# MiRaCLeXeoN/sduss

Hardware: AMD Instinct MI355X
Metric: images/sec (node), SDXL 1024^2 50-step, fixed prompt, CFG (higher is better)
Workload: dtype bf16; 1 GPU; SDXL-base-1.0 UNet 1024x1024 50-step Euler, CFG 5.0, 4 requests/step (denoiser batch 8) per GPU, is_sliced=False, random-init weights of the real architecture (2.57 B params), one data-parallel replica per GPU, no collective; resolution=1024, steps_per_image=50

## Files before the change

### include/mxdenoise.h

```cpp
#ifndef MXDENOISE_H
#define MXDENOISE_H

#include <stddef.h>
#include <stdint.h>

#ifdef __cplusplus
extern "C" {
#endif

enum { MX_F32 = 0, MX_F16 = 1, MX_BF16 = 2 };

const char* mx_last_error(void);
int mx_version(void);
#define MX_PROF_KINDS 12
int mx_profile_enable(int on);
int mx_profile_collect(double* out);
int mx_profile_records(double* out, int max_records);

size_t mx_groupnorm_halo_workspace_bytes(int N, int C, int cpg);
int mx_groupnorm_halo(void* stream, const void* x, const void* gamma, const void* beta, void* y,
                      int N, int C, int H, int W, int cpg, double eps, int padding,
                      const int32_t* latent_offset, int n_latents, const int32_t* patch_map,
                      const int32_t* padding_idx, int dtype, void* workspace);
int mx_halo_only(void* stream, const void* x, void* y, int N, int C, int H, int W,
                 const int32_t* padding_idx, int dtype);


enum {
  MX_EPI_SILU     = 1 << 0,
  MX_EPI_GEGLU    = 1 << 1,
  MX_EPI_OUT_F32  = 1 << 2,
  MX_EPI_QKV      = 1 << 3,
  MX_EPI_GELU_TANH = 1 << 4,
  MX_EPI_RES_BCAST = 1 << 5,
  MX_EPI_RMSNORM  = 1 << 6,
  MX_EPI_GELU     = 1 << 7,
  MX_EPI_QUICK_GELU = 1 << 8,
  MX_EPI_GEGLU_TANH = 1 << 9
};

#define MX_MAX_SEGS 4
typedef struct mx_gemm_seg {
  const void* a;
  const void* a2;
  void* c;
  const void* residual;
  void* vt;
  const float* rowbias;
  const float* gate;
  const float* ln_stats;
  float* stats_out;
  int M;
  int rows_per_batch;
  int ldvt;
  int B, Hin, Win, Hout, Wout;
  int a_batch_rows, a_row_off, c_batch_rows, c_row_off;
} mx_gemm_seg;

typedef struct mx_gemm_desc {
  const void* a;
  const void* w;
  void* c;
  const float* bias;
  const float* rowbias;
  const void* residual;
  void* vt;
  int M, N, K;
  int lda, ldc, ldr, ldrb;
  int rows_per_batch;
  int flags;
  int seg, period, ldvt;
  int B, Hin, Win, Cin;
  int Hout, Wout;
  int stride;
  int up;
  int corner_patch;
  int a_batch_rows, a_row_off, c_batch_rows, c_row_off;
  const float* gate;
  int ldg;
  float out_scale;
  const float* rms_wq;
  const float* rms_wk;
  float rms_eps;
  int vhalo;
  const void* a2;
  int lda2, k_split;
  const float* ln_stats;
  const float* ln_colsum;
  int ln_slabs;
  float ln_eps;
  float* stats_out;
  const mx_gemm_seg* segs;
  int n_segs;
  int splitk;
  const float* ln_final;
  float* ln_final_out;
  unsigned* ln_final_cnt;
  float* gn_part_out;
  int cin_valid;
} mx_gemm_desc;

int mx_gemm(void* stream, const mx_gemm_desc* d);
int mx_gemm_launches(const mx_gemm_desc* d);
int mx_gemm_stats_slabs(const mx_gemm_desc* d);
int mx_gemm_ln_prefers_pass(const mx_gemm_desc* d);
int mx_gemm_ln_final_supported(const mx_gemm_desc* d);
int mx_gemm_gn_partials_supported(const mx_gemm_desc* d, int conv);
enum { MX_FORM_TILE_GENERIC = 0, MX_FORM_TILE_256 = 1, MX_FORM_TILE_128 = 2, MX_FORM_PERSISTENT_256 = 3, MX_FORM_SMALL_M = 4, MX_FORM_CONV_SMALL_N = 5, MX_FORM_CONV_SMALL_CIN = 6 };
int mx_gemm_form(const mx_gemm_desc* d, int conv);
int mx_gemm_kernel_name(const mx_gemm_desc* d, int conv, int launch, char* buf, int cap);
int mx_gemm_kernel_names(char* buf, int cap);
int mx_attention_kernel_name(int B, int H, int Lq, int Lk, int ldo, int prescaled, int causal, int bias, int key_chunk, int force_cross, char* buf, int cap);
int mx_attention_kernel_names(char* buf, int cap);
#define MX_STATS_PITCH(slabs) (((slabs) + 3) & ~3)
int mx_row_stats(void* stream, const void* x, int ldx, float* stats, int M, int C);
int mx_conv3x3(void* stream, const mx_gemm_desc* d);
int mx_gemm_splitk(const mx_gemm_desc* d, int conv);
void mx_gemm_release_scratch(void* stream, int all);

typedef struct mx_attn_tail_desc {
  mx_gemm_desc out1, to_q, out2;
  const void* k; int ldk;
  const void* vt; int ldvt; int64_t vt_batch_stride;
  int B, heads, L, ctx_len;
  unsigned* sync;
} mx_attn_tail_desc;
size_t mx_attn_tail_sync_bytes(int M);
int mx_attn_tail_supported(const mx_attn_tail_desc* d);
int mx_attn_tail_preferred(void);
int mx_attn_tail(void* stream, const mx_attn_tail_desc* d);
int mx_attn_tail_status(void* stream, const unsigned* sync, unsigned* word);

#define MX_VT_POS(key) (((key) & ~12) | (((key) & 4) << 1) | (((key) & 8) >> 1))
#define MX_VT_LD(Lk) (((Lk) + 15) / 16 * 16)

int mx_attention(void* stream, const void* q, int ldq, const void* k, int ldk, const void* vt, int ldvt,
                 int64_t vt_batch_stride, void* o, int ldo, int B, int H, int Lq, int Lk, float scale);
#define MX_ATTN_QSCALE(scale) ((scale) * 1.4426950408889634f)
int mx_attention_prescaled(void* stream, const void* q, int ldq, const void* k, int ldk, const void* vt, int ldvt,
                           int64_t vt_batch_stride, void* o, int ldo, int B, int H, int Lq, int Lk);
int mx_attention_cross_prescaled(void* stream, const void* q, int ldq, const void* k, int ldk, const void* vt, int ldvt,
                                 int64_t vt_batch_stride, void* o, int ldo, int B, int H, int Lq, int Lk);
typedef struct mx_attn_problem {
  const void* q; const void* k; const void* vt; void* o;
  int64_t vt_batch_stride;
  int B, Lq, Lk, ldvt;
} mx_attn_problem;
int mx_attention_prescaled_grouped(void* stream, const mx_attn_problem* probs, int n, int ldq, int ldk, int ldo, int H);
int mx_attention_prescaled_bias(void* stream, const void* q, int ldq, const void* k, int ldk, const void* vt, int ldvt,
                                int64_t vt_batch_stride, void* o, int ldo, int B, int H, int Lq, int Lk, const float* bias, int ldb);
int mx_attention_prescaled_causal(void* stream, const void* q, int ldq, const void* k, int ldk, const void* vt, int ldvt,
                                  int64_t vt_batch_stride, void* o, int ldo, int B, int H, int L);

int mx_layernorm(void* stream, const void* x, void* y, const float* gamma, const float* beta,
                 int M, int C, float eps);

int mx_rmsnorm(void* stream, const void* x, void* y, const float* w, int M, int C, float eps);

int mx_layernorm_mod(void* stream, const void* x, void* y, void* y2, const float* scale, const float* shift,
                     const float* scale2, const float* shift2, int ldmod, int M, int C, int rows_per_batch, float eps);
int mx_layernorm_mod_grouped(void* stream, const void* x, void* y, void* y2, const float* scale, const float* shift, const float* scale2,
                             const float* shift2, int ldmod, int C, float eps, const int* batches, const int* rows_per_batch, int n);
int mx_rmsnorm_heads(void* stream, void* x, int ld, int nbatch, int rows_per_batch, int batch_rows, int row_off,
                     int heads_total, int heads_q, const float* wq, const float* wk, float eps, float q_scale);

size_t mx_groupnorm_nhwc_workspace_bytes(int B, int H, int W, int C);
int mx_groupnorm_nhwc(void* stream, const void* x, void* y, const float* gamma, const float* beta,
                      int B, int H, int W, int C, int groups, float eps, int silu, int patch,
                      void* workspace);

int mx_groupnorm_nhwc_cat(void* stream, const void* x, int C1, const void* x2, void* y, const float* gamma, const float* beta,
                          int B, int H, int W, int C, int groups, float eps, int silu, int patch, void* workspace);
int mx_groupnorm_nhwc_from_partials(void* stream, const void* x, void* y, const float* gamma, const float* beta, int B, int H, int W, int C, int groups, float eps,
                                    int silu, const float* part, int chunk, const float* add_bias, const float* add_rowbias, int ldrb, void* workspace);

typedef struct mx_gn_problem { const void* x; const void* x2; void* y; int B, H, W; } mx_gn_problem;
size_t mx_groupnorm_nhwc_grouped_workspace_bytes(const mx_gn_problem* probs, int n, int C);
int mx_groupnorm_nhwc_grouped(void* stream, const mx_gn_problem* probs, int n, int C1, const float* gamma, const float* beta, int C, int groups,
                              float eps, int silu, int patch, void* workspace);

typedef struct mx_unet_config {
  int in_channels, out_channels;
// ... 199 lines not shown
```

### sduss_amd/csrc/gemm_args.h

```cpp
#pragma once
#include "common.h"
#include "../../include/mxdenoise.h"

namespace mx {

constexpr int kMaxSegs = MX_MAX_SEGS;
struct GemmSeg {
  const bf16_t* a; const bf16_t* a2; void* c; const bf16_t* residual; bf16_t* vt; const float* rowbias; const float* gate;
  const float* ln_stats; float* stats_out;
  int M, tile0, rows_per_batch, ldvt;
  int B, Hin, Win, Hout, Wout;
  int a_batch_rows, a_row_off, c_batch_rows, c_row_off;
};

struct GemmArgs {
  const bf16_t* a;
  const bf16_t* w;
  void* c;
  const float* bias;
  const float* rowbias;
  const bf16_t* residual;
  bf16_t* vt;
  int M, N, K;
  int lda, ldc, ldr, ldrb;
  int rows_per_batch;
  int flags;
  int seg, period, ldvt;
  int B, Hin, Win, Cin, Hout, Wout, stride, up, corner_patch;
  int a_batch_rows, a_row_off, c_batch_rows, c_row_off;
  const float* gate;
  int ldg;
  int xcd_map;
  float out_scale;
  const float* rms_wq;
  const float* rms_wk;
  float rms_eps;
  int stagger_ticks;
  int vhalo;
  const bf16_t* a2;
  int lda2, k_split;
  const float* ln_stats;
  const float* ln_colsum;
  int ln_slabs;
  float ln_eps;
  float* stats_out;
  const float* ln_final;
  float* ln_final_out;
  unsigned* ln_final_cnt;
  int ln_final_slabs;
  float* gn_part;
  int splitk;
  float* sk_ws;
  unsigned* sk_cnt;
  int nseg, mt_total;
  GemmSeg prob[kMaxSegs];
};

__device__ __forceinline__ int gemm_select_seg(GemmArgs& q, const GemmArgs& p, int& tm) {
  if (p.nseg <= 0) return 0;
  int s = 0;
#pragma unroll
  for (int i = 1; i < kMaxSegs; ++i) if (i < p.nseg && tm >= p.prob[i].tile0) s = i;
  const GemmSeg& g = p.prob[s];
  tm -= g.tile0;
  q.a = g.a; q.a2 = g.a2; q.c = g.c; q.residual = g.residual; q.vt = g.vt; q.rowbias = g.rowbias; q.gate = g.gate;
  q.ln_stats = g.ln_stats; q.stats_out = g.stats_out;
  q.M = g.M; q.rows_per_batch = g.rows_per_batch; q.ldvt = g.ldvt;
  q.B = g.B; q.Hin = g.Hin; q.Win = g.Win; q.Hout = g.Hout; q.Wout = g.Wout;
  q.a_batch_rows = g.a_batch_rows; q.a_row_off = g.a_row_off; q.c_batch_rows = g.c_batch_rows; q.c_row_off = g.c_row_off;
  return s;
}
__device__ __forceinline__ int gemm_m_tiles(const GemmArgs& p, int rows) { return p.nseg > 0 ? p.mt_total : (p.M + rows - 1) / rows; }

__device__ __forceinline__ f32x4 fma4(const f32x4 a, const float s, const f32x4 c) {
  return f32x4{fmaf(a[0], s, c[0]), fmaf(a[1], s, c[1]), fmaf(a[2], s, c[2]), fmaf(a[3], s, c[3])};
}

__device__ __forceinline__ float sum_over_fq(float x) {
  float a = x, b = x;
  asm volatile("s_nop 1\n\tv_permlane16_swap_b32 %0, %1" : "+v"(a), "+v"(b));
  a += b; b = a;
  asm volatile("s_nop 1\n\tv_permlane32_swap_b32 %0, %1" : "+v"(a), "+v"(b));
  return a + b;
}

template <int NI, int MI>
__device__ __forceinline__ void gemm_ln_init(const GemmArgs& p, f32x4 (&acc)[NI][MI], const int m_wave0, const int wave_n0, const int fr,
                                             const int fq, float (&rstd)[MI]) {
#pragma clang fp contract(off)
  const int slabs = p.ln_slabs;
  const int pitch = (slabs + 3) & ~3;
  float s1[MI], s2[MI];
#pragma unroll
  for (int j = 0; j < MI; ++j) { s1[j] = 0.f; s2[j] = 0.f; }
  for (int g = 4 * fq; g < slabs; g += 16) {
    constexpr int JC = MI > 4 ? 4 : MI;
#pragma unroll
    for (int j0 = 0; j0 < MI; j0 += JC) {
      f32x4 va[JC], vb[JC];
#pragma unroll
      for (int j = 0; j < JC; ++j) {
        const int m = m_wave0 + (j0 + j) * 16 + fr;
        const float* src = p.ln_stats + ((long)(m < p.M ? m : p.M - 1) * pitch + g) * 2;
        va[j] = *reinterpret_cast<const f32x4*>(src);
        vb[j] = *reinterpret_cast<const f32x4*>(src + 4);
      }
#pragma unroll
      for (int j = 0; j < JC; ++j) {
        s1[j0 + j] += va[j][0] + (g + 1 < slabs ? va[j][2] : 0.f) + (g + 2 < slabs ? vb[j][0] : 0.f) + (g + 3 < slabs ? vb[j][2] : 0.f);
        s2[j0 + j] += va[j][1] + (g + 1 < slabs ? va[j][3] : 0.f) + (g + 2 < slabs ? vb[j][1] : 0.f) + (g + 3 < slabs ? vb[j][3] : 0.f);
      }
    }
  }
  const float inv = 1.0f / (float)p.K;
  float nmean[MI];
#pragma unroll
  for (int j = 0; j < MI; ++j) {
    const float a = sum_over_fq(s1[j]), b = sum_over_fq(s2[j]);
    const float mean = a * inv;
    const float var = fmaxf(fmaf(-mean, mean, b * inv), 0.f);
    rstd[j] = rsqrtf(var + p.ln_eps);
    nmean[j] = -mean;
  }
#pragma unroll
  for (int i = 0; i < NI; ++i) {
    const int n = wave_n0 + i * 16 + fq * 4;
    const f32x4 cs = n < p.N ? *reinterpret_cast<const f32x4*>(p.ln_colsum + n) : f32x4{0.f, 0.f, 0.f, 0.f};
#pragma unroll
    for (int j = 0; j < MI; ++j) acc[i][j] = cs * nmean[j];
  }
}

__device__ __forceinline__ void gemm_ln_row(const GemmArgs& p, const int m, const int fq, float& rstd, float& rm) {
#pragma clang fp contract(off)
  const int mc = m < p.M ? m : p.M - 1;
  const int pitch = (p.ln_slabs + 3) & ~3;
  float s1 = 0.f, s2 = 0.f;
  for (int s = fq; s < p.ln_slabs; s += 4) {
    const f32x2 v = *reinterpret_cast<const f32x2*>(p.ln_stats + ((long)mc * pitch + s) * 2);
    s1 += v[0]; s2 += v[1];
  }
  s1 = sum_over_fq(s1); s2 = sum_over_fq(s2);
  const float inv = 1.0f / (float)p.K;
  const float mean = s1 * inv;
  const float var = fmaxf(fmaf(-mean, mean, s2 * inv), 0.f);
  rstd = rsqrtf(var + p.ln_eps);
  rm = rstd * mean;
}

__device__ __forceinline__ float row16_sum(float x) {
  x += __builtin_bit_cast(float, __builtin_amdgcn_update_dpp(0, __builtin_bit_cast(int, x), 0xB1, 0xF, 0xF, true));
  x += __builtin_bit_cast(float, __builtin_amdgcn_update_dpp(0, __builtin_bit_cast(int, x), 0x4E, 0xF, 0xF, true));
  x += __builtin_bit_cast(float, __builtin_amdgcn_update_dpp(0, __builtin_bit_cast(int, x), 0x141, 0xF, 0xF, true));
  x += __builtin_bit_cast(float, __builtin_amdgcn_update_dpp(0, __builtin_bit_cast(int, x), 0x140, 0xF, 0xF, true));
  return x;
// ... 39 lines not shown
      a += __uint_as_float((unsigned)v); q += __uint_as_float((unsigned)(v >> 32));
    }
  }
  const float a2 = __shfl_xor(a, 1, 64), q2 = __shfl_xor(q, 1, 64);
  if (!(tid & 1) && m < p.M) {
    const float inv = 1.0f / (float)p.N;
    const float mean = (a + a2) * inv;
    const float var = fmaxf(fmaf(-mean, mean, (q + q2) * inv), 0.f);
    *reinterpret_cast<f32x2*>(p.ln_final_out + (long)m * 2) = f32x2{mean, rsqrtf(var + p.ln_eps)};
  }
}

template <int NI, int MI, bool KEEP>
__device__ __forceinline__ void gemm_ln_init_final(const GemmArgs& p, f32x4 (&acc)[NI][MI], const int m_wave0, const int wave_n0, const int fr,
                                                   const int fq, float (&rstd)[MI]) {
#pragma clang fp contract(off)
  f32x2 st[MI];
#pragma unroll
  for (int j = 0; j < MI; ++j) {
    const int m = m_wave0 + j * 16 + fr;
    st[j] = *reinterpret_cast<const f32x2*>(p.ln_final + (long)(m < p.M ? m : p.M - 1) * 2);
  }
  f32x4 cs[NI];
#pragma unroll
  for (int i = 0; i < NI; ++i) cs[i] = *reinterpret_cast<const f32x4*>(p.ln_colsum + wave_n0 + i * 16 + fq * 4);
  if constexpr (KEEP) {
#pragma unroll
    for (int j = 0; j < MI; ++j) rstd[j] = st[j][1];
  }
#pragma unroll
  for (int i = 0; i < NI; ++i)
#pragma unroll
    for (int j = 0; j < MI; ++j) acc[i][j] = cs[i] * (-st[j][0]);
}

typedef unsigned int u32x4_sk __attribute__((ext_vector_type(4)));
template <int NI, int MI>
__device__ __forceinline__ bool splitk_combine(const GemmArgs& p, f32x4 (&acc)[NI][MI], const int tile, const int slice, const int tile_elems,
                                               volatile int* ticket_word) {
  const int tid = threadIdx.x;
  const auto rsrc = __builtin_amdgcn_make_buffer_rsrc(p.sk_ws + (long)tile * p.splitk * tile_elems, 0, p.splitk * tile_elems * 4, 0x00020000);
  const int lane_off = tid * 16;
#pragma unroll
  for (int i = 0; i < NI; ++i)
#pragma unroll
    for (int j = 0; j < MI; ++j)
      __builtin_amdgcn_raw_buffer_store_b128(__builtin_bit_cast(u32x4_sk, acc[i][j]), rsrc, (slice * tile_elems + (i * MI + j) * 2048) * 4 + lane_off, 0, 16);
  asm volatile("s_waitcnt vmcnt(0)" ::: "memory");
  __syncthreads();
  if (tid == 0) *ticket_word = (int)__hip_atomic_fetch_add(p.sk_cnt + tile, 1u, __ATOMIC_RELAXED, __HIP_MEMORY_SCOPE_AGENT);
  __syncthreads();
  const int ticket = *ticket_word;
  if (ticket != p.splitk - 1) return false;
  if (tid == 0) __hip_atomic_store(p.sk_cnt + tile, 0u, __ATOMIC_RELAXED, __HIP_MEMORY_SCOPE_AGENT);
#pragma unroll
  for (int i = 0; i < NI; ++i)
#pragma unroll
    for (int j = 0; j < MI; ++j) acc[i][j] = f32x4{0.f, 0.f, 0.f, 0.f};
  for (int s = 0; s < p.splitk; ++s) {
    f32x4 v[NI][MI];
#pragma unroll
    for (int i = 0; i < NI; ++i)
#pragma unroll
      for (int j = 0; j < MI; ++j)
        v[i][j] = __builtin_bit_cast(f32x4, __builtin_amdgcn_raw_buffer_load_b128(rsrc, (s * tile_elems + (i * MI + j) * 2048) * 4 + lane_off, 0, 16));
#pragma unroll
    for (int i = 0; i < NI; ++i)
#pragma unroll
      for (int j = 0; j < MI; ++j) acc[i][j] += v[i][j];
  }
  return true;
}

__device__ __forceinline__ long gemm_in_row(const GemmArgs& p, int m) {
  if (p.a_batch_rows <= 0) return m;
  const int b = m / p.rows_per_batch;
  return (long)b * p.a_batch_rows + p.a_row_off + (m - b * p.rows_per_batch);
}
__device__ __forceinline__ long gemm_out_row(const GemmArgs& p, int m, int bidx) {
  if (p.c_batch_rows <= 0) return m;
  return (long)bidx * p.c_batch_rows + p.c_row_off + (m - bidx * p.rows_per_batch);
}

template <int NI, int MI, int BN>
__device__ __forceinline__ void gemm_epilogue(const GemmArgs& p, f32x4 (&acc)[NI][MI], const int m_wave0,
                                              const int wave_n0, const int fr, const int fq) {
  const int flags = p.flags;
  const bool geglu = (flags & MX_EPI_GEGLU) != 0;
  const bool qkv = (flags & MX_EPI_QKV) != 0;
  int seg_idx = 0, seg_grp = 0, seg_pos = 0;
  bool to_vt = false;
  if (qkv) {
    seg_idx = wave_n0 / p.seg;
    seg_grp = seg_idx / p.period;
    seg_pos = seg_idx - seg_grp * p.period;
    to_vt = (seg_pos == p.period - 1);
  }

  const bool rms = qkv && (flags & MX_EPI_RMSNORM) && !to_vt;
  const bool ln = p.ln_stats != nullptr;
#pragma unroll
  for (int j = 0; j < MI; ++j) {
    const int m = m_wave0 + j * 16 + fr;
    float rms_mul = 1.0f;
    float ln_rstd = 1.0f, ln_rm = 0.f;
    if (ln) gemm_ln_row(p, m, fq, ln_rstd, ln_rm);
    if (rms) {
      float ss = 0.f;
#pragma unroll
      for (int i = 0; i < NI; ++i) {
        const int n = wave_n0 + i * 16 + fq * 4;
#pragma unroll
        for (int q = 0; q < 4; ++q) { const float t = acc[i][j][q] + (p.bias ? p.bias[n + q] : 0.f); ss += t * t; }
      }
      ss = sum_over_fq(ss);
      rms_mul = rsqrtf(ss * (1.0f / 64.0f) + p.rms_eps) * ((seg_pos == 0 && p.out_scale != 0.f) ? p.out_scale : 1.0f);
    }
    if (m >= p.M) continue;
    const int bidx = (p.rows_per_batch > 0) ? (m / p.rows_per_batch) : 0;
    const long orow = gemm_out_row(p, m, bidx);
    const long rrow = (flags & MX_EPI_RES_BCAST) ? (long)(m - bidx * p.rows_per_batch) : orow;
#pragma unroll
    for (int i = 0; i < (NI); ++i) {
      if (geglu && i >= NI / 2) continue;
      const int n = wave_n0 + i * 16 + fq * 4;
      if (n >= p.N) continue;
      float v[4];
#pragma unroll
      for (int q = 0; q < 4; ++q) v[q] = acc[i][j][q];
      if (ln) {
        const f32x4 c4 = *reinterpret_cast<const f32x4*>(p.ln_colsum + n);
#pragma unroll
        for (int q = 0; q < 4; ++q) v[q] = v[q] * ln_rstd - ln_rm * c4[q];
      }
      if (p.bias) {
        const f32x4 b4 = *reinterpret_cast<const f32x4*>(p.bias + n);
#pragma unroll
        for (int q = 0; q < 4; ++q) v[q] += b4[q];
      }
      if (rms) {
        const float* w = (seg_pos == 0 ? p.rms_wq : p.rms_wk) + ((n - seg_idx * p.seg) & 63);
#pragma unroll
        for (int q = 0; q < 4; ++q) v[q] *= rms_mul * w[q];
      } else if (p.out_scale != 0.f && (!qkv || seg_pos == 0)) {
#pragma unroll
        for (int q = 0; q < 4; ++q) v[q] *= p.out_scale;
      }
      if (geglu) {
        float g[4];
        const int ng = n + (NI / 2) * 16;
#pragma unroll
        for (int q = 0; q < 4; ++q) g[q] = acc[i + NI / 2][j][q];
        if (ln) {
          const f32x4 c4 = *reinterpret_cast<const f32x4*>(p.ln_colsum + ng);
#pragma unroll
          for (int q = 0; q < 4; ++q) g[q] = g[q] * ln_rstd - ln_rm * c4[q];
        }
        if (p.bias) {
          const f32x4 b4 = *reinterpret_cast<const f32x4*>(p.bias + ng);
#pragma unroll
          for (int q = 0; q < 4; ++q) g[q] += b4[q];
        }
#pragma unroll
        for (int q = 0; q < 4; ++q) v[q] = v[q] * ((flags & MX_EPI_GEGLU_TANH) ? gelu_tanh_f(g[q]) : gelu_fast(g[q]));
        const int nout = wave_n0 / 2 + i * 16 + fq * 4;
        u32x2 o = {pack_bf16x2(v[0], v[1]), pack_bf16x2(v[2], v[3])};
        *reinterpret_cast<u32x2*>(reinterpret_cast<bf16_t*>(p.c) + (long)m * p.ldc + nout) = o;
        continue;
      }
      if (p.rowbias) {
        const f32x4 b4 = *reinterpret_cast<const f32x4*>(p.rowbias + (long)bidx * p.ldrb + n);
#pragma unroll
        for (int q = 0; q < 4; ++q) v[q] += b4[q];
      }
      if (p.gate) {
        const f32x4 g4 = *reinterpret_cast<const f32x4*>(p.gate + (long)bidx * p.ldg + n);
#pragma unroll
        for (int q = 0; q < 4; ++q) v[q] *= g4[q];
      }
      if (p.residual) {
        const u32x2 r = *reinterpret_cast<const u32x2*>(p.residual + rrow * p.ldr + n);
        v[0] += bf16lo_to_f32(r[0]); v[1] += bf16hi_to_f32(r[0]);
        v[2] += bf16lo_to_f32(r[1]); v[3] += bf16hi_to_f32(r[1]);
      }
      if (flags & MX_EPI_SILU) {
#pragma unroll
        for (int q = 0; q < 4; ++q) v[q] = silu_f(v[q]);
      }
      if (flags & MX_EPI_GELU_TANH) {
#pragma unroll
        for (int q = 0; q < 4; ++q) v[q] = gelu_tanh_f(v[q]);
      }
      if (flags & (MX_EPI_GELU | MX_EPI_QUICK_GELU)) {
#pragma unroll
        for (int q = 0; q < 4; ++q) v[q] = (flags & MX_EPI_GELU) ? gelu_fast(v[q]) : quick_gelu_f(v[q]);
      }
      if (qkv) {
        const int nin = n - seg_idx * p.seg;
        if (to_vt) {
          const int key0 = (p.c_batch_rows > 0 ? p.c_row_off : 0) + m - bidx * p.rows_per_batch;
          const int key = MX_VT_POS(key0);
          const int nv = p.N / p.period;
          bf16_t* dst = p.vt + ((long)bidx * nv + (long)seg_grp * p.seg + nin) * p.ldvt + key;
#pragma unroll
          for (int q = 0; q < 4; ++q) dst[(long)q * p.ldvt] = f32_to_bf16(v[q]);
        } else {
          const int ccol = seg_grp * (p.period - 1) * p.seg + seg_pos * p.seg + nin;
          u32x2 o = {pack_bf16x2(v[0], v[1]), pack_bf16x2(v[2], v[3])};
          *reinterpret_cast<u32x2*>(reinterpret_cast<bf16_t*>(p.c) + orow * p.ldc + ccol) = o;
        }
        continue;
      }
      if (flags & MX_EPI_OUT_F32) {
        f32x4 o = {v[0], v[1], v[2], v[3]};
        *reinterpret_cast<f32x4*>(reinterpret_cast<float*>(p.c) + orow * p.ldc + n) = o;
      } else {
        u32x2 o = {pack_bf16x2(v[0], v[1]), pack_bf16x2(v[2], v[3])};
        *reinterpret_cast<u32x2*>(reinterpret_cast<bf16_t*>(p.c) + orow * p.ldc + n) = o;
      }
    }
  }
}


__device__ __forceinline__ void gemm_tile_of_block(const int b, const int mt, const int nt, const int xcd_map, int& tm, int& tn) {
  constexpr int MB = 4;
  if (!xcd_map || (mt & 7) != 0) { tm = b % mt; tn = b / mt; return; }
  const int xcd = b & 7;
  const int local = b >> 3;
  const int mloc = mt >> 3;
  const int band_tiles = MB * nt;
  const int band = local / band_tiles;
  const int r = local - band * band_tiles;
  const int rows = (mloc - band * MB) < MB ? (mloc - band * MB) : MB;
  tn = r / rows;
  tm = ((band * MB + (r - tn * rows)) << 3) + xcd;
}

__device__ __forceinline__ void lane_exchange_pair(float (&a)[4], float (&b)[4]) {
#pragma unroll
  for (int d = 0; d < 4; ++d) {
    unsigned x = __float_as_uint(a[d]), y = __float_as_uint(b[d]);
    auto r = __builtin_amdgcn_permlane32_swap(x, y, false, false);
    auto t = __builtin_amdgcn_permlane16_swap(r[0], r[1], false, false);
    a[d] = __uint_as_float(t[0]);
    b[d] = __uint_as_float(t[1]);
  }
}

__device__ __forceinline__ u32x4 lane_xor1(const u32x4 x) {
  u32x4 r;
#pragma unroll
  for (int d = 0; d < 4; ++d) r[d] = (unsigned)__builtin_amdgcn_update_dpp(0, (int)x[d], 0xB1, 0xF, 0xF, true);
  return r;
}

constexpr int EPI_F_QKV = 1;
constexpr int EPI_F_ACT = 2;
constexpr int EPI_F_ALL = 3;
constexpr int EPI_F_TANH = 4;
__host__ __device__ inline int gemm_epi_features(int flags) {
  const int acts = flags & (MX_EPI_SILU | MX_EPI_GELU | MX_EPI_GELU_TANH | MX_EPI_QUICK_GELU | MX_EPI_GEGLU_TANH);
  return ((flags & MX_EPI_QKV) ? EPI_F_QKV : 0) | (acts == 0 ? 0 : acts == MX_EPI_GELU_TANH ? EPI_F_TANH : EPI_F_ACT);
}
template <int NI, int MI, bool GEGLU, bool VEC = true, bool VPF = true, bool STATS = true, int FEAT = EPI_F_ALL, bool EMIT = STATS, bool RSTD_LOAD = false, bool WT = false>
__device__ __forceinline__ void gemm_epilogue_regs(const GemmArgs& p, f32x4 (&acc)[NI][MI], const int m_wave0, const int wave_n0,
                                                   const int fr, const int fq, const float (&ln_rstd_a)[MI]) {
#pragma clang fp contract(off)
  constexpr int NIO = GEGLU ? NI / 2 : NI;
  constexpr int NP = NIO / 2;
  constexpr bool ODD = (NIO & 1) != 0;
  constexpr int DEPTH = MI <= 4 ? MI : 2;
  static_assert(!GEGLU || NI % 4 == 0, "GEGLU: hidden and gate halves must be whole pairs");
  const int flags = p.flags;
  constexpr bool ACT = (FEAT & EPI_F_ACT) != 0;
  constexpr bool TANH = (FEAT & (EPI_F_ACT | EPI_F_TANH)) != 0;
  const bool qkv = (FEAT & EPI_F_QKV) != 0 && (flags & MX_EPI_QKV) != 0;
  int seg_idx = 0, seg_grp = 0, seg_pos = 0;
  bool to_vt = false;
  if (qkv) {
    seg_idx = wave_n0 / p.seg;
    seg_grp = seg_idx / p.period;
    seg_pos = seg_idx - seg_grp * p.period;
    to_vt = seg_pos == p.period - 1;
  }
  const bool rms = qkv && (flags & MX_EPI_RMSNORM) && !to_vt;
  const float w_scale = (!rms && p.out_scale != 0.f && (!qkv || seg_pos == 0)) ? p.out_scale : 1.0f;
  const int col0 = GEGLU ? wave_n0 / 2 : qkv ? seg_grp * (p.period - 1) * p.seg + seg_pos * p.seg + (wave_n0 - seg_idx * p.seg) : wave_n0;
  const bool has_res = !GEGLU && p.residual != nullptr;
  const bool has_rb = VEC && !GEGLU && p.rowbias != nullptr, has_gate = VEC && !GEGLU && p.gate != nullptr;

  f32x4 bias_r[NI];
#pragma unroll
  for (int i = 0; i < NI; ++i) {
    bias_r[i] = f32x4{0.f, 0.f, 0.f, 0.f};
    if (p.bias && (GEGLU || i < NIO)) bias_r[i] = *reinterpret_cast<const f32x4*>(p.bias + wave_n0 + i * 16 + fq * 4);
  }
  f32x4 rmsw_r[NI];
  if (rms) {
    const float* w = seg_pos == 0 ? p.rms_wq : p.rms_wk;
#pragma unroll
    for (int i = 0; i < NI; ++i) rmsw_r[i] = *reinterpret_cast<const f32x4*>(w + ((wave_n0 - seg_idx * p.seg + i * 16 + fq * 4) & 63));
  }
  const bool stats = EMIT && !GEGLU && !qkv && p.stats_out != nullptr;

  if constexpr ((FEAT & EPI_F_QKV) != 0) {
    if (qkv && to_vt) {
      const int rpb_v = p.rows_per_batch > 0 ? p.rows_per_batch : 0x7fffffff;
      const int m_first = m_wave0 + fr;
      int bv = p.rows_per_batch > 0 ? m_first / p.rows_per_batch : 0;
      int rv = m_first - bv * (p.rows_per_batch > 0 ? p.rows_per_batch : 0);
      const int key_off = p.c_batch_rows > 0 ? p.c_row_off : 0;
      const int nv = p.N / p.period;
      const long feat0 = (long)seg_grp * p.seg + (wave_n0 - seg_idx * p.seg) + fq * 4;
      auto rstd_at = [&](int j) __attribute__((always_inline)) -> float {
        const int m = m_first + 16 * j;
        return p.ln_final[(long)(m < p.M ? m : p.M - 1) * 2 + 1];
      };
      float rs_next = RSTD_LOAD ? rstd_at(0) : 1.0f;
#pragma unroll
      for (int j = 0; j < MI; ++j) {
        const float rs_cur = rs_next;
        if (RSTD_LOAD && j + 1 < MI) rs_next = rstd_at(j + 1);
        if (m_first + 16 * j < p.M) {
          const int key = MX_VT_POS(key_off + rv);
          bf16_t* dst = p.vt + ((long)bv * nv + feat0) * p.ldvt + key;
          const float rs = RSTD_LOAD ? rs_cur : STATS ? ln_rstd_a[j] : 1.0f;
#pragma unroll
          for (int i = 0; i < NIO; ++i) {
            const f32x4 t = STATS ? fma4(acc[i][j], rs, bias_r[i]) : acc[i][j] + bias_r[i];
#pragma unroll
            for (int q = 0; q < 4; ++q) dst[(long)(i * 16 + q) * p.ldvt] = f32_to_bf16(t[q]);
          }
        }
        rv += 16;
        if (rv >= rpb_v) { rv -= rpb_v; ++bv; }
      }
      return;
    }
  }
  const bool odd_lane = (fr & 1) != 0;
  const int rpb = p.rows_per_batch > 0 ? p.rows_per_batch : 0x7fffffff;
  const int cbr = p.c_batch_rows > 0 ? p.c_batch_rows : (p.rows_per_batch > 0 ? p.rows_per_batch : 0);
  const int cro = p.c_batch_rows > 0 ? p.c_row_off : 0;
  const int b_last = p.rows_per_batch > 0 ? (p.M - 1) / p.rows_per_batch : 0;
  const int r_last = p.M - 1 - b_last * (p.rows_per_batch > 0 ? p.rows_per_batch : 0);
  const int row_last = b_last * cbr + cro + r_last;
  const int mA0 = (m_wave0 + fr) & ~1;
  int row_a[MI], row_b[MI];
  int bo_walk = 0, ro_walk = 0;
  {
    int bA = p.rows_per_batch > 0 ? mA0 / p.rows_per_batch : 0;
    int rA = mA0 - bA * (p.rows_per_batch > 0 ? p.rows_per_batch : 0);
#pragma unroll
    for (int j = 0; j < MI; ++j) {
      int bB = bA, rB = rA + 1;
      if (rB >= rpb) { rB = 0; ++bB; }
      const int mA = mA0 + 16 * j;
      row_a[j] = mA < p.M ? bA * cbr + cro + rA : row_last;
      row_b[j] = mA + 1 < p.M ? bB * cbr + cro + rB : row_last;
      if constexpr (VEC) { if (j == 0) { bo_walk = odd_lane ? bB : bA; ro_walk = odd_lane ? rB : rA; } }
      rA += 16;
      if (rA >= rpb) { rA -= rpb; ++bA; }
    }
  }
  auto token = [&](int j) __attribute__((always_inline)) { return m_wave0 + j * 16 + fr; };
  auto row_own = [&](int j) __attribute__((always_inline)) { return odd_lane ? row_b[j] : row_a[j]; };
  const char* const res_base = reinterpret_cast<const char*>(p.residual);
  char* const c_base = reinterpret_cast<char*>(p.c);
  const unsigned ldr_b = (unsigned)p.ldr * 2u, ldc_b = (unsigned)p.ldc * 2u;
  auto res_at = [&](int row, int col) __attribute__((always_inline)) { return res_base + (unsigned long long)(unsigned)row * ldr_b + (unsigned)(col * 2); };
  auto c_at = [&](int row, int col) __attribute__((always_inline)) { return c_base + (unsigned long long)(unsigned)row * ldc_b + (unsigned)(col * 2); };
  const auto c_rsrc = __builtin_amdgcn_make_buffer_rsrc(p.c, 0, WT ? (int)((unsigned)p.M * ldc_b) : 0, 0x00020000);
  auto store_c16 = [&](int row, int col, const u32x4 v) __attribute__((always_inline)) {
    if constexpr (WT) __builtin_amdgcn_raw_buffer_store_b128(v, c_rsrc, (int)((unsigned)row * ldc_b + (unsigned)(col * 2)), 0, 16);
    else *reinterpret_cast<u32x4*>(c_at(row, col)) = v;
  };
  auto store_c8 = [&](int row, int col, const u32x2 v) __attribute__((always_inline)) {
    if constexpr (WT) __builtin_amdgcn_raw_buffer_store_b64(v, c_rsrc, (int)((unsigned)row * ldc_b + (unsigned)(col * 2)), 0, 16);
    else *reinterpret_cast<u32x2*>(c_at(row, col)) = v;
  };

  auto load_res = [&](int j, int pr) __attribute__((always_inline)) -> u32x4 {
    if (!has_res) return u32x4{0u, 0u, 0u, 0u};
    return *reinterpret_cast<const u32x4*>(res_at(row_own(j), col0 + pr * 32 + fq * 8));
  };
  auto load_res_odd = [&](int j) __attribute__((always_inline)) -> u32x2 {
    if (!has_res) return u32x2{0u, 0u};
    return *reinterpret_cast<const u32x2*>(res_at(row_own(j), col0 + NP * 32 + fq * 4));
  };
  f32x4 rb_r[VEC ? NIO : 1], gate_r[VEC ? NIO : 1];
  auto load_batch_vectors = [&](int j) __attribute__((always_inline)) {
    if constexpr (VEC) {
      (void)j;
      const int bidx = bo_walk < b_last ? bo_walk : b_last;
      ro_walk += 16;
      if (ro_walk >= rpb) { ro_walk -= rpb; ++bo_walk; }
#pragma unroll
      for (int i = 0; i < NIO; ++i) {
        const int n = wave_n0 + i * 16 + fq * 4;
        if (has_rb) rb_r[i] = *reinterpret_cast<const f32x4*>(p.rowbias + (long)bidx * p.ldrb + n);
        if (has_gate) gate_r[i] = *reinterpret_cast<const f32x4*>(p.gate + (long)bidx * p.ldg + n);
      }
    }
  };
  if constexpr (VPF) { if (has_rb || has_gate) load_batch_vectors(0); }
  constexpr int NG = NP / 2;
  constexpr bool fullmode = NG > 0;
  const int col_full = col0 + (odd_lane ? 32 : 0) + fq * 8;
  auto load_res_full = [&](int j, int g, int which) __attribute__((always_inline)) -> u32x4 {
    if (!has_res) return u32x4{0u, 0u, 0u, 0u};
    return *reinterpret_cast<const u32x4*>(res_at(which ? row_b[j] : row_a[j], col_full + 64 * g));
  };
  auto load_res_any = [&](int j, int pr) __attribute__((always_inline)) -> u32x4 {
    if (pr < 2 * NG) return load_res_full(j, pr >> 1, pr & 1);
    return load_res(j, pr);
  };
  u32x4 res_r[DEPTH][NP > 0 ? NP : 1];
  u32x2 res_o[DEPTH];
  {
#pragma unroll
    for (int d = 0; d < DEPTH && d < MI; ++d) {
#pragma unroll
      for (int pr = 0; pr < NP; ++pr) res_r[d][pr] = load_res_any(d, pr);
      if constexpr (ODD) res_o[d] = load_res_odd(d);
    }
  }

  auto rstd_at = [&](int j) __attribute__((always_inline)) -> float {
    const int m = token(j);
    return p.ln_final[(long)(m < p.M ? m : p.M - 1) * 2 + 1];
  };
  float rstd_next = RSTD_LOAD ? rstd_at(0) : 1.0f;
#pragma unroll
// ... 153 lines not shown
```

### sduss_amd/csrc/gemm_bf16.hip

```cpp
#include <algorithm>
#include <cstdlib>

#include <mutex>
#include <unordered_map>

#include "common.h"
#include "../../include/mxdenoise.h"
#include "gemm_args.h"
#include "gemm_forms.h"

namespace mx {

constexpr int BM = 128;
constexpr int BK = 64;

__device__ __forceinline__ int swz(int row, int chunk) { return chunk ^ ((row >> 1) & 7); }

template <int BN, bool CONV>
__global__ __launch_bounds__(256, 2) void gemm_kernel(const GemmArgs pk) {
  constexpr int NI = BN / 32;
  constexpr int MI = 4;
  constexpr int WROWS = BN / 32;
  __shared__ __attribute__((aligned(16))) bf16_t sX[2][BM * BK];
  __shared__ __attribute__((aligned(16))) bf16_t sW[2][BN * BK];

  const int tid = threadIdx.x;
  const int lane = tid & 63;
  const int wave = tid >> 6;
  const int wm = wave >> 1;
  const int wn = wave & 1;
  GemmArgs p = pk;
  int tm = blockIdx.x;
  gemm_select_seg(p, pk, tm);
  const int m0 = tm * BM;
  const int n0 = blockIdx.y * BN;
  const int nk = p.K / BK;

  const int srow = tid >> 3;
  const int sch = tid & 7;

  int xoff[4];
  int xoff2[4];
  int cb[4], cy[4], cx[4];
#pragma unroll
  for (int i = 0; i < 4; ++i) {
    const int m = m0 + srow + 32 * i;
    if constexpr (!CONV) {
      xoff[i] = (m < p.M) ? (int)(gemm_in_row(p, m) * p.lda) + sch * 8 : -1;
      xoff2[i] = (p.a2 != nullptr && m < p.M) ? m * p.lda2 + sch * 8 : 0;
    } else {
      if (m < p.M) {
        const int hw = p.Hout * p.Wout;
        const int b = m / hw;
        const int r = m - b * hw;
        const int oy = r / p.Wout;
        cb[i] = b;
        cy[i] = oy * p.stride;
        cx[i] = (r - oy * p.Wout) * p.stride;
      } else {
        cb[i] = -1; cy[i] = 0; cx[i] = 0;
      }
    }
  }
  int woff[WROWS];
#pragma unroll
  for (int i = 0; i < WROWS; ++i) {
    const int n = n0 + srow + 32 * i;
    woff[i] = (n < p.N) ? n * p.K + sch * 8 : -1;
  }

  u32x4 rx[4], rw[WROWS];
  const u32x4 zero4 = {0u, 0u, 0u, 0u};

  auto load_tile = [&](int kt) {
    const int k0 = kt * BK;
    if constexpr (!CONV) {
#pragma unroll
      for (int i = 0; i < 4; ++i) {
        if (p.a2 != nullptr && k0 >= p.k_split) rx[i] = (xoff[i] >= 0) ? *reinterpret_cast<const u32x4*>(p.a2 + xoff2[i] + (k0 - p.k_split)) : zero4;
        else rx[i] = (xoff[i] >= 0) ? *reinterpret_cast<const u32x4*>(p.a + xoff[i] + k0) : zero4;
      }
    } else {
      const int tap = k0 / p.Cin;
      const int c0 = k0 - tap * p.Cin;
      const int dy = tap / 3 - 1;
      const int dx = tap - (tap / 3) * 3 - 1;
      const int Hv = p.Hin << p.up, Wv = p.Win << p.up;
      const int P = p.corner_patch;
#pragma unroll
      for (int i = 0; i < 4; ++i) {
        int iy = cy[i] + dy;
        const int ix = cx[i] + dx;
        if (P > 0 && dy != 0 && dx != 0) {
          const bool cross_r = ((iy + P) / P) != ((cy[i] + P) / P);
          const bool cross_c = ((ix + P) / P) != ((cx[i] + P) / P);
          if (cross_r && cross_c) iy = cy[i];
        }
        const bool ok = (cb[i] >= 0) && (iy >= -p.vhalo) && (iy < Hv + p.vhalo) && (ix >= 0) && (ix < Wv);
        if (ok) {
          const long src = (((long)cb[i] * (p.Hin + 2 * p.vhalo) + (iy >> p.up) + p.vhalo) * p.Win + (ix >> p.up)) * p.Cin + c0 + sch * 8;
          rx[i] = *reinterpret_cast<const u32x4*>(p.a + src);
        } else {
          rx[i] = zero4;
        }
      }
    }
#pragma unroll
    for (int i = 0; i < WROWS; ++i)
      rw[i] = (woff[i] >= 0) ? *reinterpret_cast<const u32x4*>(p.w + woff[i] + k0) : zero4;
  };
  auto store_tile = [&](int buf) {
#pragma unroll
    for (int i = 0; i < 4; ++i) {
      const int row = srow + 32 * i;
      *reinterpret_cast<u32x4*>(&sX[buf][row * BK + swz(row, sch) * 8]) = rx[i];
    }
#pragma unroll
    for (int i = 0; i < WROWS; ++i) {
      const int row = srow + 32 * i;
      *reinterpret_cast<u32x4*>(&sW[buf][row * BK + swz(row, sch) * 8]) = rw[i];
    }
  };

  f32x4 acc[NI][MI];
#pragma unroll
  for (int i = 0; i < NI; ++i)
#pragma unroll
    for (int j = 0; j < MI; ++j) acc[i][j] = f32x4{0.f, 0.f, 0.f, 0.f};

  const int fr = lane & 15;
  const int fq = lane >> 4;

  load_tile(0);
  store_tile(0);
  __syncthreads();

  for (int kt = 0; kt < nk; ++kt) {
    const int buf = kt & 1;
    if (kt + 1 < nk) load_tile(kt + 1);
#pragma unroll
    for (int ks = 0; ks < 2; ++ks) {
      bf16x8 wf[NI], xf[MI];
#pragma unroll
      for (int i = 0; i < NI; ++i) {
        const int row = wn * (BN / 2) + i * 16 + fr;
        wf[i] = *reinterpret_cast<const bf16x8*>(&sW[buf][row * BK + swz(row, ks * 4 + fq) * 8]);
      }
#pragma unroll
      for (int j = 0; j < MI; ++j) {
        const int row = wm * 64 + j * 16 + fr;
        xf[j] = *reinterpret_cast<const bf16x8*>(&sX[buf][row * BK + swz(row, ks * 4 + fq) * 8]);
      }
#pragma unroll
      for (int i = 0; i < NI; ++i)
#pragma unroll
        for (int j = 0; j < MI; ++j)
          acc[i][j] = __builtin_amdgcn_mfma_f32_16x16x32_bf16(wf[i], xf[j], acc[i][j], 0, 0, 0);
    }
    if (kt + 1 < nk) store_tile(buf ^ 1);
    __syncthreads();
  }

  gemm_epilogue<NI, MI, BN>(p, acc, m0 + wm * 64, n0 + wn * (BN / 2), fr, fq);
}

int launch_v2(hipStream_t s, const GemmArgs& a, int bn, int form);
int launch_v5(hipStream_t s, const GemmArgs& a, int bn, int rows, int form);
int launch_v4(hipStream_t s, const GemmArgs& a, int form);
bool small_m_serves(const mx_gemm_desc* d, bool conv);
int small_m_form(long N, long K, int flags);
int launch_small_m(hipStream_t s, const GemmArgs& a, int form);
bool conv_small_n_serves(const mx_gemm_desc* d);
int launch_conv_small_n(hipStream_t s, const GemmArgs& a);
bool conv_small_cin_serves(const mx_gemm_desc* d);
int launch_conv_small_cin(hipStream_t s, const GemmArgs& a);

constexpr size_t kSplitKWsBytes = 96u << 20;
constexpr size_t kSplitKCntBytes = 64u << 10;
struct TileChoice { int bn; int rows; int splitk = 1; };
static long m_tiles_of(const mx_gemm_desc* d, int rows) {
  if (d->n_segs <= 0) return cdiv(d->M, rows);
  long t = 0;
  for (int i = 0; i < d->n_segs; ++i) t += cdiv(d->segs[i].M, rows);
  return t;
}
static long rows_of(const mx_gemm_desc* d) {
  if (d->n_segs <= 0) return d->M;
  long m = 0;
  for (int i = 0; i < d->n_segs; ++i) m += d->segs[i].M;
  return m;
}
static TileChoice pick_tile(const mx_gemm_desc* d, bool conv) {
  constexpr double v3_discount = 0.87;
  const TileChoice none = {0, 0};
  const long Mtot = rows_of(d);
  if (Mtot < 128 || d->K < 128) return none;
  if (d->flags & (MX_EPI_OUT_F32 | MX_EPI_RES_BCAST)) return none;
  if (d->n_segs <= 0) { if (d->rows_per_batch > 0 && d->rows_per_batch < 16) return none; }
  else for (int i = 0; i < d->n_segs; ++i) if (d->segs[i].rows_per_batch > 0 && d->segs[i].rows_per_batch < 16) return none;
  if (d->ldc % 8 != 0 || ((uintptr_t)d->c & 15) != 0) return none;
  if (d->residual && (d->ldr % 8 != 0 || ((uintptr_t)d->residual & 15) != 0)) return none;
  const bool geglu = (d->flags & MX_EPI_GEGLU) != 0, qkv = (d->flags & MX_EPI_QKV) != 0;
  bool fits32 = (long)d->N * d->K * 2 < (1L << 32);
  if (d->n_segs <= 0) {
    const long in_rows = d->a_batch_rows > 0 ? (long)(d->M / d->rows_per_batch + 1) * d->a_batch_rows : d->M;
    fits32 = fits32 && in_rows * d->lda * 2 < (1L << 32);
  } else {
    uintptr_t lo = (uintptr_t)d->segs[0].a;
    for (int i = 1; i < d->n_segs; ++i) lo = std::min(lo, (uintptr_t)d->segs[i].a);
    for (int i = 0; i < d->n_segs; ++i) {
      const mx_gemm_seg& g = d->segs[i];
      const long in_rows = g.a_batch_rows > 0 ? (long)(g.M / std::max(g.rows_per_batch, 1) + 1) * g.a_batch_rows : g.M;
      fits32 = fits32 && (long)((uintptr_t)g.a - lo) + in_rows * d->lda * 2 < (1L << 32);
    }
  }
  TileChoice best = none;
  double best_cost = 0;
  const TileChoice cands[5] = {{256, 256}, {160, 256}, {128, 256}, {160, 128}, {128, 128}};
  for (int c = 0; c < 5; ++c) {
    const int bn = cands[c].bn, rows = cands[c].rows;
    if (d->N % bn != 0 || Mtot < rows) continue;
    if (bn == 256 && (conv || !fits32 || d->a2 || d->ln_stats || d->stats_out)) continue;
    if (d->ln_final && bn != 256) continue;
    if (geglu && bn == 160) continue;
    if (qkv && d->seg % 64 != 0) continue;
    if ((d->flags & MX_EPI_RMSNORM) && bn == 160) continue;
    if (qkv && bn != 256 && d->seg % (bn / 2) != 0) continue;
    const long tiles = m_tiles_of(d, rows) * (d->N / bn);
    const int ncu = cu_count();
    const double cost = (double)((tiles + ncu - 1) / ncu) * (rows + bn) * (bn == 256 ? v3_discount : 1.0);
    if (best.rows == 0 || cost < best_cost) { best = cands[c]; best_cost = cost; }
  }
  if (d->splitk != 1 && best.rows == 128 && !d->a2 && d->K / 64 >= 16) {
    const int ncu = cu_count();
    const int nk = d->K / 64;
    double best_t = 0, unsplit_t = 0;
    TileChoice pick = best;
    const double mtot = (double)Mtot;
    for (int c = 3; c < 5; ++c) {
      const int bn = cands[c].bn;
      if (d->N % bn != 0 || (geglu && bn == 160) || (qkv && (d->seg % 64 != 0 || d->seg % (bn / 2) != 0)) || ((d->flags & MX_EPI_RMSNORM) && bn == 160)) continue;
      const long tiles = m_tiles_of(d, 128) * (d->N / bn);
      for (int sk = 1; sk <= 4; ++sk) {
        if (d->splitk > 1 && sk != 1 && sk != d->splitk) continue;
        if (nk / sk < 8 || (sk > 1 && tiles * sk > 2L * ncu)) continue;
        if (sk > 1 && (tiles * sk * 128L * bn * 4 > (long)kSplitKWsBytes || tiles * 4 > (long)kSplitKCntBytes)) continue;
        const double combine = sk > 1 ? 2.0 + (double)sk * mtot * d->N * 8.0 / 4.0e6 : 0.0;
        const double t = (double)((tiles * sk + ncu - 1) / ncu) * ((double)(nk / sk) * 0.57 * (128 + bn) / 256.0 + 5.0) + combine;
        if (sk == 1 && bn == best.bn) unsplit_t = t;
        if (best_t == 0 || t < best_t - 1e-9) { best_t = t; pick = TileChoice{bn, 128, sk}; }
      }
    }
    if (pick.splitk > 1 && unsplit_t > 0 && best_t <= 0.75 * unsplit_t) best = pick;
    if (d->splitk > 1) {
      double ft = 0;
      for (int c = 3; c < 5; ++c) {
        const int bn = cands[c].bn, sk = d->splitk;
        if (d->N % bn != 0 || (geglu && bn == 160) || (qkv && (d->seg % 64 != 0 || d->seg % (bn / 2) != 0)) || ((d->flags & MX_EPI_RMSNORM) && bn == 160)) continue;
        const long tiles = m_tiles_of(d, 128) * (d->N / bn);
        if (sk > 4 || nk / sk < 8 || tiles * sk * 128L * bn * 4 > (long)kSplitKWsBytes || tiles * 4 > (long)kSplitKCntBytes) continue;
        const double t = (double)((tiles * sk + ncu - 1) / ncu) * ((double)(nk / sk) * 0.57 * (128 + bn) / 256.0 + 5.0);
        if (ft == 0 || t < ft) { ft = t; best = TileChoice{bn, 128, sk}; }
      }
    }
  }
  return best;
}

struct SplitKScratch { float* ws = nullptr; unsigned* cnt = nullptr; };
struct SplitKPool {
  std::mutex mu;
  std::unordered_map<hipStream_t, SplitKScratch> per_stream;
  static void drop(SplitKScratch& b) { if (b.ws) (void)hipFree(b.ws); if (b.cnt) (void)hipFree(b.cnt); b = SplitKScratch{}; }
  ~SplitKPool() { for (auto& kv : per_stream) drop(kv.second); }
};
static SplitKPool& splitk_pool() { static SplitKPool p; return p; }
static bool splitk_scratch(hipStream_t s, SplitKScratch& out) {
  SplitKPool& pool = splitk_pool();
  std::lock_guard<std::mutex> lock(pool.mu);
  auto it = pool.per_stream.find(s);
  if (it != pool.per_stream.end()) { out = it->second; return out.ws != nullptr; }
  hipStreamCaptureMode mode = hipStreamCaptureModeRelaxed;
  (void)hipThreadExchangeStreamCaptureMode(&mode);
  SplitKScratch b;
  hipStream_t z = nullptr;
  bool ok = hipMalloc(&b.ws, kSplitKWsBytes) == hipSuccess && hipMalloc(&b.cnt, kSplitKCntBytes) == hipSuccess &&
            hipStreamCreateWithFlags(&z, hipStreamNonBlocking) == hipSuccess && hipMemsetAsync(b.cnt, 0, kSplitKCntBytes, z) == hipSuccess &&
            hipStreamSynchronize(z) == hipSuccess;
  if (z) (void)hipStreamDestroy(z);
  (void)hipThreadExchangeStreamCaptureMode(&mode);
  if (!ok) { (void)hipGetLastError(); SplitKPool::drop(b); return false; }
  pool.per_stream[s] = b;
  out = b;
  return true;
}
static void splitk_release(hipStream_t s, bool all) {
  SplitKPool& pool = splitk_pool();
  std::lock_guard<std::mutex> lock(pool.mu);
  if (all) { for (auto& kv : pool.per_stream) { (void)hipStreamSynchronize(kv.first); SplitKPool::drop(kv.second); } pool.per_stream.clear(); return; }
  auto it = pool.per_stream.find(s);
  if (it == pool.per_stream.end()) return;
  (void)hipStreamSynchronize(s);
  SplitKPool::drop(it->second);
  pool.per_stream.erase(it);
}

static int stats_slabs_of(const mx_gemm_desc* d, bool conv, const TileChoice& tc) {
  if (conv || tc.bn == 0 || tc.bn == 256) return 0;
  if (d->flags & (MX_EPI_GEGLU | MX_EPI_QKV | MX_EPI_OUT_F32)) return 0;
  if (d->a_batch_rows > 0 || d->c_batch_rows > 0) return 0;
  for (int i = 0; i < d->n_segs; ++i) if (d->segs[i].a_batch_rows > 0 || d->segs[i].c_batch_rows > 0) return 0;
  const int panel = tc.bn / 2;
  return d->N / panel;
}

static bool is_small_m_form(int form) {
  switch (form) {
#define MX_SM(id, k, targs) case id: return true;
    MX_GEMM_SMALL_M_FORMS(MX_SM)
#undef MX_SM
    default: return false;
  }
}

static int gemm_kernel_of(const mx_gemm_desc* d, bool conv, const TileChoice& tc) {
  if (d->ln_final && tc.bn != 256) return -1;
  if (small_m_serves(d, conv)) return small_m_form(d->N, d->K, d->flags);
  if (conv && conv_small_n_serves(d)) return GK_CONV_SMALL_N;
  if (conv && conv_small_cin_serves(d)) return GK_CONV_SMALL_CIN;
  const int feat = gemm_epi_features(d->flags);
  const bool geglu = (d->flags & MX_EPI_GEGLU) != 0;
  const bool vec = d->rowbias || d->gate;
  if (tc.bn == 256) {
    if (d->ln_final) {
      if (geglu) return (feat & EPI_F_ACT) ? -1 : GK_V4_GEGLU_LN;
      return feat == EPI_F_QKV ? GK_V4_QKV_LN : feat == 0 ? GK_V4_LN : -1;
    }
    if (geglu) return (feat & EPI_F_ACT) ? GK_V4_GEGLU_ACT : GK_V4_GEGLU;
    if (!vec) return feat == 0 ? GK_V4 : feat == EPI_F_QKV ? GK_V4_QKV : feat == EPI_F_TANH ? GK_V4_TANH : GK_V4_VEC_ALL;
    return feat == 0 ? GK_V4_VEC : GK_V4_VEC_ALL;
  }
  if (tc.bn != 0 && tc.rows == 256) {
    const bool b160 = tc.bn == 160;
    if (geglu) return (feat & EPI_F_ACT) ? GK_V5_128_GEGLU_ACT : GK_V5_128_GEGLU;
    if (conv) {
      if (feat == 0 && !vec) return b160 ? GK_V5_160_CONV : GK_V5_128_CONV;
      if (feat == 0) return b160 ? GK_V5_160_CONV_VEC : GK_V5_128_CONV_VEC;
      return b160 ? GK_V5_160_CONV_ALL : GK_V5_128_CONV_ALL;
    }
    if (feat == 0 && !vec) return b160 ? GK_V5_160 : GK_V5_128;
    if (feat == EPI_F_QKV && !vec) return b160 ? GK_V5_160_QKV : GK_V5_128_QKV;
    return b160 ? GK_V5_160_ALL : GK_V5_128_ALL;
  }
  if (tc.bn != 0) {
    const bool b160 = tc.bn == 160;
    if (geglu) return (feat & EPI_F_ACT) ? GK_V2_128_GEGLU_ACT : GK_V2_128_GEGLU;
    if (conv) return feat == 0 ? (b160 ? GK_V2_160_CONV : GK_V2_128_CONV) : (b160 ? GK_V2_160_CONV_ALL : GK_V2_128_CONV_ALL);
    if (feat == 0) return b160 ? GK_V2_160 : GK_V2_128;
    if (feat == EPI_F_QKV) return b160 ? GK_V2_160_QKV : GK_V2_128_QKV;
    return b160 ? GK_V2_160_ALL : GK_V2_128_ALL;
  }
  if (d->N % 128 == 0) return conv ? GK_GEN128_CONV : GK_GEN128;
  return conv ? GK_GEN64_CONV : GK_GEN64;
}

static int prepare(void* stream, const mx_gemm_desc* d, bool conv, GemmArgs& a, TileChoice& tc_out) {
  MX_CHECK(d != nullptr, "gemm: null descriptor");
  MX_CHECK(d->a && d->w && (d->c || (d->flags & MX_EPI_QKV)), "gemm: null operand");
  MX_CHECK(d->n_segs >= 0 && d->n_segs <= MX_MAX_SEGS && (d->n_segs == 0 || d->segs != nullptr), "gemm: bad n_segs / segs");
  MX_CHECK((d->n_segs > 0 || d->M > 0) && d->N > 0 && d->K > 0, "gemm: empty problem");
  for (int i = 0; i < d->n_segs; ++i) {
    const mx_gemm_seg& g = d->segs[i];
    MX_CHECK(g.M > 0 && g.a && (g.c != nullptr) == (d->c != nullptr), "gemm: grouped launch: empty problem or missing a / c");
    MX_CHECK((g.a2 != nullptr) == (d->a2 != nullptr && !conv) && (g.residual != nullptr) == (d->residual != nullptr) && (g.vt != nullptr) == (d->vt != nullptr) &&
             (g.rowbias != nullptr) == (d->rowbias != nullptr) && (g.gate != nullptr) == (d->gate != nullptr) &&
             (g.ln_stats != nullptr) == (d->ln_stats != nullptr) && (g.stats_out != nullptr) == (d->stats_out != nullptr),
             "gemm: grouped launch: a problem's optional operands must match the descriptor's");
    const void* ptrs[] = {g.a, g.a2, g.c, g.residual, g.vt, g.rowbias, g.gate, g.ln_stats, g.stats_out};
    for (const void* q : ptrs) MX_CHECK(((uintptr_t)q & 15) == 0, "gemm: grouped launch: operand pointers must be 16-byte aligned");
    if (d->rowbias || d->gate || g.a_batch_rows > 0 || g.c_batch_rows > 0 || (d->flags & (MX_EPI_QKV | MX_EPI_RES_BCAST)))
      MX_CHECK(g.rows_per_batch > 0, "gemm: grouped launch: rows_per_batch required");
    if (g.a_batch_rows > 0) MX_CHECK(!conv && g.a_row_off >= 0 && g.a_row_off + g.rows_per_batch <= g.a_batch_rows, "gemm: grouped launch: bad input row remap");
    if (g.c_batch_rows > 0) MX_CHECK(g.c_row_off >= 0 && g.c_row_off + g.rows_per_batch <= g.c_batch_rows, "gemm: grouped launch: bad output row remap");
    if (d->ln_stats || d->stats_out)
      MX_CHECK(g.a_batch_rows <= 0 && g.c_batch_rows <= 0, "gemm: grouped launch: the folded LayerNorm / stats_out exclude a problem's row remaps");
    if (d->flags & MX_EPI_QKV)
      MX_CHECK(g.M % g.rows_per_batch == 0 && g.ldvt >= MX_VT_LD(g.c_batch_rows > 0 ? g.c_batch_rows : g.rows_per_batch) && g.ldvt % 8 == 0,
               "gemm: grouped launch: QKV needs whole batches and ldvt >= MX_VT_LD(keys per batch)");
    if (conv) {
      const int Hv = g.Hin << d->up, Wv = g.Win << d->up;
      MX_CHECK(g.Hout == (Hv + d->stride - 1) / d->stride && g.Wout == (Wv + d->stride - 1) / d->stride && (long)g.B * g.Hout * g.Wout == g.M,
               "conv3x3: grouped launch: a problem's output grid does not match its input grid / stride / rows");
    }
    MX_CHECK((long)g.M * (conv ? 1 : d->lda) < 2147483647L, "gemm: grouped launch: operand exceeds 32-bit indexing");
  }
  MX_CHECK(d->K % BK == 0, "gemm: K must be a multiple of 64");
  MX_CHECK(d->N % 4 == 0, "gemm: N must be a multiple of 4");
  a.stagger_ticks = 0;
  a.vhalo = conv ? d->vhalo : 0;
  a.a2 = conv ? nullptr : (const bf16_t*)d->a2; a.lda2 = d->lda2; a.k_split = d->k_split;
  a.a = (const bf16_t*)d->a; a.w = (const bf16_t*)d->w; a.c = d->c;
  a.bias = d->bias; a.rowbias = d->rowbias; a.residual = (const bf16_t*)d->residual; a.vt = (bf16_t*)d->vt;
  a.M = d->M; a.N = d->N; a.K = d->K; a.lda = d->lda; a.ldc = d->ldc; a.ldr = d->ldr; a.ldrb = d->ldrb;
  a.rows_per_batch = d->rows_per_batch; a.flags = d->flags; a.seg = d->seg; a.period = d->period; a.ldvt = d->ldvt;
  a.B = d->B; a.Hin = d->Hin; a.Win = d->Win; a.Cin = d->Cin; a.Hout = d->Hout; a.Wout = d->Wout;
  a.stride = d->stride; a.up = d->up; a.corner_patch = d->corner_patch;
  a.a_batch_rows = d->a_batch_rows; a.a_row_off = d->a_row_off; a.c_batch_rows = d->c_batch_rows; a.c_row_off = d->c_row_off;
  a.gate = d->gate; a.ldg = d->ldg; a.out_scale = d->out_scale;
  a.rms_wq = d->rms_wq; a.rms_wk = d->rms_wk; a.rms_eps = d->rms_eps;
  a.ln_stats = d->ln_stats; a.ln_colsum = d->ln_colsum; a.ln_slabs = d->ln_slabs; a.ln_eps = d->ln_eps; a.stats_out = nullptr;
  a.ln_final = nullptr; a.ln_final_out = nullptr; a.ln_final_cnt = nullptr; a.ln_final_slabs = 0;
  if (d->ln_final) {
    MX_CHECK(!conv && !d->ln_stats && d->ln_colsum && d->n_segs == 0, "gemm: ln_final needs ln_colsum, excludes ln_stats and grouped launches (mx_gemm only)");
    MX_CHECK(!(d->flags & MX_EPI_RMSNORM) && d->a_batch_rows <= 0 && d->c_batch_rows <= 0 && !d->a2 && !d->rowbias && !d->gate && !d->stats_out,
             "gemm: ln_final excludes RMSNORM, the row remaps, the split A operand, per-sample vectors and stats_out");
    MX_CHECK((((uintptr_t)d->ln_final & 15) | ((uintptr_t)d->ln_colsum & 15)) == 0, "gemm: ln_final / ln_colsum must be 16-byte aligned");
    a.ln_final = d->ln_final;
  }
  a.nseg = d->n_segs; a.mt_total = 0;
  const bool grouped = d->n_segs > 0;
  if (d->ln_stats) {
    MX_CHECK(!conv && d->ln_colsum && d->ln_slabs > 0, "gemm: folded LayerNorm needs ln_colsum and ln_slabs > 0 (mx_gemm only)");
    MX_CHECK(!(d->flags & MX_EPI_RMSNORM) && d->a_batch_rows <= 0 && d->c_batch_rows <= 0 && !d->a2, "gemm: folded LayerNorm excludes RMSNORM, the row remaps and the split A operand");
    MX_CHECK((((uintptr_t)d->ln_stats & 15) | ((uintptr_t)d->ln_colsum & 15)) == 0, "gemm: ln_stats / ln_colsum must be 16-byte aligned");
  }
  a.xcd_map = 1;

  if (!conv && d->a2) {
    MX_CHECK(d->k_split > 0 && d->k_split < d->K && d->k_split % BK == 0, "gemm: k_split must be a multiple of 64 inside (0, K)");
    MX_CHECK(d->lda >= d->k_split && d->lda % 8 == 0 && d->lda2 >= d->K - d->k_split && d->lda2 % 8 == 0, "gemm: bad lda / lda2 for the split A operand");
    MX_CHECK(d->a_batch_rows <= 0 && ((uintptr_t)d->a2 & 15) == 0 && rows_of(d) * d->lda2 < 2147483647L, "gemm: split A operand excludes the row remap and needs 16-byte alignment");
  } else if (!conv) {
    MX_CHECK(d->lda >= d->K && d->lda % 8 == 0, "gemm: lda must be >= K and a multiple of 8");
  } else {
    MX_CHECK(d->Cin % BK == 0 && d->K == 9 * d->Cin, "conv3x3: Cin must be a multiple of 64 and K = 9*Cin");
    MX_CHECK(d->stride == 1 || d->stride == 2, "conv3x3: stride must be 1 or 2");
    MX_CHECK(d->up == 0 || d->up == 1, "conv3x3: up must be 0 or 1");
    MX_CHECK(!(d->up && d->stride != 1), "conv3x3: upsample only with stride 1");
    if (!grouped) {
      const int Hv = d->Hin << d->up, Wv = d->Win << d->up;
      MX_CHECK(d->Hout == (Hv + d->stride - 1) / d->stride && d->Wout == (Wv + d->stride - 1) / d->stride,
               "conv3x3: output grid does not match input grid / stride");
      MX_CHECK((long)d->B * d->Hout * d->Wout == d->M, "conv3x3: M != B*Hout*Wout");
    }
    MX_CHECK(2 * d->Cin <= 16384, "conv3x3: Cin > 8192 (the pipelined loader walks a 16 KB zero page for padding taps)");
    MX_CHECK(!(d->flags & MX_EPI_GEGLU), "conv3x3: no GEGLU epilogue");
    MX_CHECK(d->vhalo == 0 || (d->vhalo == 1 && d->corner_patch == 0), "conv3x3: vhalo must be 0 or 1 and excludes the sliced corner rule");
  }
  {
    const void* ptrs[] = {d->a, d->w, d->c, d->bias, d->rowbias, d->residual, d->gate, d->rms_wq, d->rms_wk};
    for (const void* q : ptrs) MX_CHECK(((uintptr_t)q & 15) == 0, "gemm: operand pointers must be 16-byte aligned");
  }
  if (!grouped && (d->rowbias || d->gate || d->a_batch_rows > 0 || d->c_batch_rows > 0 || (d->flags & (MX_EPI_QKV | MX_EPI_RES_BCAST))))
    MX_CHECK(d->rows_per_batch > 0, "gemm: rows_per_batch required");
  if (d->gate) MX_CHECK(d->ldg >= d->N && d->ldg % 4 == 0, "gemm: bad ldg");
  if (!grouped && d->a_batch_rows > 0) MX_CHECK(!conv && d->a_row_off >= 0 && d->a_row_off + d->rows_per_batch <= d->a_batch_rows, "gemm: bad input row remap");
  if (!grouped && d->c_batch_rows > 0) MX_CHECK(d->c_row_off >= 0 && d->c_row_off + d->rows_per_batch <= d->c_batch_rows, "gemm: bad output row remap");
  if (d->rowbias) MX_CHECK(d->ldrb >= d->N && d->ldrb % 4 == 0, "gemm: bad ldrb");
  if (!grouped) {
    const long in_rows = (!conv && d->a_batch_rows > 0) ? (long)(d->M / d->rows_per_batch + 1) * d->a_batch_rows : d->M;
    MX_CHECK(in_rows * (conv ? 1 : d->lda) < 2147483647L, "gemm: operand exceeds 32-bit indexing");
  }
  MX_CHECK((long)d->N * d->K < 2147483647L, "gemm: operand exceeds 32-bit indexing");
  if (d->residual) MX_CHECK(d->ldr >= d->N && d->ldr % 4 == 0, "gemm: bad ldr");
  const bool use128 = (d->N % 128 == 0);
  const TileChoice tc = pick_tile(d, conv);
  tc_out = tc;
  a.splitk = 0; a.sk_ws = nullptr; a.sk_cnt = nullptr;
  if (tc.splitk > 1) {
    SplitKScratch sk;
    MX_CHECK(splitk_scratch((hipStream_t)stream, sk), "gemm: the split-K scratch (96 MB per stream) could not be allocated; set mx_gemm_desc.splitk = 1 to run unsplit");
    a.splitk = tc.splitk; a.sk_ws = sk.ws; a.sk_cnt = sk.cnt;
  }
  if (d->stats_out) {
    MX_CHECK(stats_slabs_of(d, conv, tc) > 0, "gemm: stats_out is not supported for this shape / epilogue (see mx_gemm_stats_slabs)");
    MX_CHECK(((uintptr_t)d->stats_out & 15) == 0, "gemm: stats_out must be 16-byte aligned");
    a.stats_out = d->stats_out;
  }
  a.gn_part = nullptr;
  if (d->gn_part_out) {
    MX_CHECK(!grouped && tc.rows == 256 && tc.bn != 256 && tc.bn != 0 && tc.splitk <= 1, "gemm: gn_part_out needs an ungrouped launch on a 256-row tile (mx_gemm_gn_partials_supported)");
    MX_CHECK(d->flags == 0 && !d->residual && !d->gate && d->out_scale == 0.f && !d->ln_stats && !d->ln_final && d->a_batch_rows <= 0 && d->c_batch_rows <= 0,
             "gemm: gn_part_out needs an epilogue of bias (+ row bias) only");
    MX_CHECK(d->M % 64 == 0 && (!d->rowbias || d->rows_per_batch % 64 == 0) && ((uintptr_t)d->gn_part_out & 15) == 0, "gemm: gn_part_out needs M % 64 == 0, rows_per_batch % 64 == 0 and 16-byte alignment");
    a.gn_part = d->gn_part_out;
  }
  if (d->ln_final_out) {
    MX_CHECK(d->stats_out && d->ln_final_cnt && !grouped && tc.rows == 256 && tc.bn != 256 && tc.bn != 0,
             "gemm: ln_final_out needs stats_out, ln_final_cnt and an ungrouped launch on a 256-row tile (mx_gemm_ln_final_supported)");
    MX_CHECK((((uintptr_t)d->ln_final_out & 15) | ((uintptr_t)d->ln_final_cnt & 3)) == 0, "gemm: ln_final_out must be 16-byte aligned");
    a.ln_final_out = d->ln_final_out; a.ln_final_cnt = d->ln_final_cnt; a.ln_final_slabs = stats_slabs_of(d, conv, tc);
  }
  if (grouped) {
    const int rows = tc.rows > 0 ? tc.rows : BM;
    uintptr_t lo = (uintptr_t)d->segs[0].a;
    int t0 = 0;
    for (int i = 0; i < d->n_segs; ++i) {
      const mx_gemm_seg& g = d->segs[i];
      GemmSeg& o = a.prob[i];
      o.a = (const bf16_t*)g.a; o.a2 = conv ? nullptr : (const bf16_t*)g.a2; o.c = g.c; o.residual = (const bf16_t*)g.residual; o.vt = (bf16_t*)g.vt;
      o.rowbias = g.rowbias; o.gate = g.gate; o.ln_stats = g.ln_stats; o.stats_out = d->stats_out ? g.stats_out : nullptr;
      o.M = g.M; o.tile0 = t0; o.rows_per_batch = g.rows_per_batch; o.ldvt = g.ldvt;
      o.B = g.B; o.Hin = g.Hin; o.Win = g.Win; o.Hout = g.Hout; o.Wout = g.Wout;
      o.a_batch_rows = g.a_batch_rows; o.a_row_off = g.a_row_off; o.c_batch_rows = g.c_batch_rows; o.c_row_off = g.c_row_off;
      t0 += cdiv(g.M, rows);
      lo = std::min(lo, (uintptr_t)g.a);
    }
    a.mt_total = t0;
    a.a = (const bf16_t*)lo;
    a.M = (int)rows_of(d);
  }
  if (d->flags & MX_EPI_GEGLU) {
    MX_CHECK(use128, "gemm: GEGLU needs N % 128 == 0");
    MX_CHECK(!(d->flags & (MX_EPI_QKV | MX_EPI_OUT_F32)) && !d->residual && !d->rowbias && d->out_scale == 0.f, "gemm: GEGLU excludes other epilogues");
    MX_CHECK(d->ldc >= d->N / 2 && d->ldc % 4 == 0, "gemm: bad ldc for GEGLU");
  } else if (d->flags & MX_EPI_QKV) {
    MX_CHECK(d->seg > 0 && d->seg % 64 == 0 && d->period >= 2 && d->N % (d->seg * d->period) == 0, "gemm: bad QKV segments");
    MX_CHECK(d->vt != nullptr, "gemm: QKV needs vt");
    if (!grouped) {
      MX_CHECK(d->ldvt >= MX_VT_LD(d->c_batch_rows > 0 ? d->c_batch_rows : d->rows_per_batch), "gemm: QKV needs ldvt >= MX_VT_LD(keys per batch)");
      MX_CHECK(d->M % d->rows_per_batch == 0, "gemm: QKV needs M % rows_per_batch == 0");
    }
    MX_CHECK(d->ldc >= d->N / d->period * (d->period - 1) && d->ldc % 4 == 0, "gemm: bad ldc for QKV");
    MX_CHECK(!(d->flags & MX_EPI_OUT_F32), "gemm: QKV output is bf16");
    MX_CHECK(!d->rowbias && !d->gate && !d->residual, "gemm: QKV excludes the per-sample vectors and the residual (its V^T segment takes none of them)");
    if (d->flags & MX_EPI_RMSNORM)
      MX_CHECK(d->rms_wq && d->rms_wk && d->period == 3 && d->N % 128 == 0 && !conv, "gemm: RMSNORM needs rms_wq/rms_wk, period 3, N % 128 == 0");
  } else {
    MX_CHECK(d->ldc >= d->N && d->ldc % 4 == 0, "gemm: bad ldc");
  }
  return 0;
}

int gemm_prepare_for_chain(void* stream, const mx_gemm_desc* d, GemmArgs& a, int& bn, int& rows, int& splitk) {
  TileChoice tc;
  if (int rc = prepare(stream, d, false, a, tc)) return rc;
  bn = tc.bn; rows = tc.rows; splitk = tc.splitk;
  return 0;
}

static int launch(void* stream, const mx_gemm_desc* d, bool conv) {
  GemmArgs a;
  TileChoice tc;
  if (int rc = prepare(stream, d, conv, a, tc)) return rc;
  const bool grouped = d->n_segs > 0;
  const bool use128 = (d->N % 128 == 0);
  const int v2bn = tc.bn;
  dim3 block(256);
  hipStream_t s = (hipStream_t)stream;
  if (prof_enabled()) {
    const double kk = conv ? 9.0 * d->Cin : (double)d->K;
    const double Mt = (double)rows_of(d);
    double in_elems = conv ? (double)d->B * d->Hin * d->Win * d->Cin : Mt * d->K;
    if (conv && grouped) { in_elems = 0; for (int i = 0; i < d->n_segs; ++i) in_elems += (double)d->segs[i].B * d->segs[i].Hin * d->segs[i].Win * d->Cin; }
    const double flops = 2.0 * Mt * (double)d->N * kk;
    const double bytes = 2.0 * (in_elems + (double)d->N * d->K + Mt * d->N);
    const int kind = v2bn == 256 ? PROF_GEMM_V3_256 : v2bn ? (conv ? PROF_CONV_V2_160 : PROF_GEMM_V2_160) + (v2bn == 160 ? 0 : 2) : (conv ? PROF_CONV128 : PROF_GEMM128) + (use128 ? 0 : 1);
    prof_begin(s, kind, flops, bytes, (int)Mt, d->N, (int)kk);
  }
  const int mt128 = grouped ? a.mt_total : cdiv(d->M, BM);
  if (d->ln_final) MX_CHECK(v2bn == 256, "gemm: ln_final is the 256 x 256 kernel's form of the folded LayerNorm; this shape does not run there (use ln_stats)");
  const int form = gemm_kernel_of(d, conv, tc);
  MX_CHECK(form >= 0, v2bn == 256 ? "gemm: no 256 x 256 instantiation serves ln_final with this epilogue (GEGLU, QKV or plain bias only)"
                                   : "gemm: no kernel instantiation serves this descriptor");
  if (is_small_m_form(form)) {
    MX_CHECK(launch_small_m(s, a, form) == 0, "gemm: the small-M launcher was handed a form outside its list");
  } else if (form == GK_CONV_SMALL_N) {
    launch_conv_small_n(s, a);
  } else if (form == GK_CONV_SMALL_CIN) {
    launch_conv_small_cin(s, a);
  } else if (v2bn == 256) {
    MX_CHECK(launch_v4(s, a, form) == 0, "gemm: no 256 x 256 instantiation serves ln_final with this epilogue (GEGLU, QKV or plain bias only)");
  } else if (v2bn) {
    if (tc.rows == 256) MX_CHECK(launch_v5(s, a, v2bn, tc.rows, form) == 0, "gemm: the 256-row launcher was handed a form outside its list");
    else MX_CHECK(launch_v2(s, a, v2bn, form) == 0, "gemm: the 128-row launcher was handed a form outside its list");
  } else {
    const dim3 grid(mt128, use128 ? d->N / 128 : cdiv(d->N, 64));
    switch (form) {
#define MX_GEN(id, k, targs) case id: hipLaunchKernelGGL((k<MX_FORM_UNPAREN targs>), grid, block, 0, s, a); break;
      MX_GEMM_GENERIC_FORMS(MX_GEN)
#undef MX_GEN
      default: MX_CHECK(false, "gemm: the generic launcher was handed a form outside its list");
    }
  }
  prof_end(s);
  MX_LAUNCH_CHECK();
  return 0;
}

}

namespace mx {
static bool tail_split(const mx_gemm_desc* d, mx_gemm_desc& d1, mx_gemm_desc& d2) {
  if (d->n_segs != 0 || d->M <= 0 || d->N <= 0 || d->K <= 0 || d->N % 256 != 0) return false;
  if (d->flags & (MX_EPI_QKV | MX_EPI_OUT_F32 | MX_EPI_RES_BCAST | MX_EPI_RMSNORM)) return false;
  if (d->stats_out || d->ln_stats || d->ln_final || d->ln_final_out || d->a_batch_rows > 0 || d->c_batch_rows > 0 || d->splitk > 1) return false;
  if (pick_tile(d, false).bn != 256) return false;
  const int ncu = cu_count();
  if (ncu <= 0) return false;
  const long mt = cdiv(d->M, 256), nt = d->N / 256, tiles = mt * nt;
  const long full = tiles / ncu, rem = tiles % ncu;
  if (full < 1 || rem == 0 || rem * 2 > ncu || (full * ncu) % mt != 0) return false;
  const long nt1 = full * ncu / mt;
  if (nt1 <= 0 || nt1 >= nt) return false;
  const int N1 = (int)nt1 * 256, N2 = d->N - N1;
  const bool geglu = (d->flags & MX_EPI_GEGLU) != 0;
  const long cofs = geglu ? N1 / 2 : N1;
  d1 = *d; d2 = *d;
  d1.N = N1; d2.N = N2;
  d1.splitk = 1; d2.splitk = 1;
  d2.w = (const char*)d->w + (size_t)N1 * d->K * 2;
  if (d->bias) d2.bias = d->bias + N1;
  d2.c = (char*)d->c + (size_t)cofs * 2;
  if (geglu && d->residual) return false;
  if (d->residual) d2.residual = (const char*)d->residual + (size_t)N1 * 2;
  if (d->rowbias) d2.rowbias = d->rowbias + N1;
  if (d->gate) d2.gate = d->gate + N1;
  const TileChoice t2 = pick_tile(&d2, false);
  if (t2.bn == 0 || t2.bn == 256 || t2.rows + t2.bn > 384) return false;
  if (m_tiles_of(&d2, t2.rows) * (N2 / t2.bn) > ncu) return false;
  return pick_tile(&d1, false).bn == 256;
}
}

extern "C" int mx_gemm(void* stream, const mx_gemm_desc* d) {
  mx_gemm_desc d1, d2;
  if (d != nullptr && mx::tail_split(d, d1, d2)) { if (int rc = mx::launch(stream, &d1, false)) return rc; return mx::launch(stream, &d2, false); }
  return mx::launch(stream, d, false);
}
extern "C" int mx_gemm_launches(const mx_gemm_desc* d) { mx_gemm_desc d1, d2; return d != nullptr && mx::tail_split(d, d1, d2) ? 2 : 1; }
extern "C" int mx_gemm_form(const mx_gemm_desc* d, int conv) {
  if (!d || mx::rows_of(d) <= 0 || d->N <= 0 || d->K <= 0) return MX_FORM_TILE_GENERIC;
  if (mx::small_m_serves(d, conv != 0)) return MX_FORM_SMALL_M;
  if (conv && mx::conv_small_n_serves(d)) return MX_FORM_CONV_SMALL_N;
  if (conv && mx::conv_small_cin_serves(d)) return MX_FORM_CONV_SMALL_CIN;
  const mx::TileChoice tc = mx::pick_tile(d, conv != 0);
  return tc.bn == 256 ? MX_FORM_PERSISTENT_256 : tc.bn == 0 ? MX_FORM_TILE_GENERIC : tc.rows == 256 ? MX_FORM_TILE_256 : MX_FORM_TILE_128;
}
extern "C" int mx_gemm_stats_slabs(const mx_gemm_desc* d) {
  if (!d || mx::rows_of(d) <= 0 || d->N <= 0 || d->K <= 0) return 0;
  mx_gemm_desc q = *d;
  if (!q.stats_out) q.stats_out = reinterpret_cast<float*>(16);
  return mx::stats_slabs_of(&q, false, mx::pick_tile(&q, false));
}
extern "C" int mx_gemm_ln_prefers_pass(const mx_gemm_desc* d) {
  if (!d || mx::rows_of(d) <= 0 || d->N <= 0 || d->K <= 0) return 0;
  mx_gemm_desc plain = *d;
  plain.ln_stats = nullptr; plain.stats_out = nullptr;
  return mx::pick_tile(&plain, false).bn == 256;
}
extern "C" int mx_gemm_gn_partials_supported(const mx_gemm_desc* d, int conv) {
  if (!d || d->n_segs > 0 || d->M <= 0 || d->N <= 0 || d->K <= 0 || d->M % 64 != 0) return 0;
  if (d->flags != 0 || d->residual || d->gate || d->out_scale != 0.f || d->ln_stats || d->ln_final || d->a_batch_rows > 0 || d->c_batch_rows > 0) return 0;
  if (d->rowbias && (d->rows_per_batch <= 0 || d->rows_per_batch % 64 != 0)) return 0;
  const mx::TileChoice tc = mx::pick_tile(d, conv != 0);
  return tc.rows == 256 && tc.bn != 256 && tc.bn != 0 && tc.splitk <= 1;
}
extern "C" int mx_gemm_ln_final_supported(const mx_gemm_desc* d) {
  if (!d || d->n_segs > 0 || d->M <= 0 || d->N <= 0 || d->K <= 0) return 0;
  mx_gemm_desc q = *d;
  if (!q.stats_out) q.stats_out = reinterpret_cast<float*>(16);
  const mx::TileChoice tc = mx::pick_tile(&q, false);
  return tc.rows == 256 && tc.bn != 256 && tc.bn != 0 && mx::stats_slabs_of(&q, false, tc) > 0;
}
extern "C" int mx_conv3x3(void* stream, const mx_gemm_desc* d) { return mx::launch(stream, d, true); }
extern "C" void mx_gemm_release_scratch(void* stream, int all) { mx::splitk_release((hipStream_t)stream, all != 0); }
extern "C" int mx_gemm_splitk(const mx_gemm_desc* d, int conv) {
  if (!d || mx::rows_of(d) <= 0 || d->N <= 0 || d->K <= 0) return 0;
  return mx::pick_tile(d, conv != 0).splitk;
}

namespace mx {
static const char* const kGemmKernelNames[GK_COUNT] = {
  MX_GEMM_GENERIC_FORMS(MX_FORM_NAME_T) MX_GEMM_V2_FORMS(MX_FORM_NAME_T) MX_GEMM_V5_FORMS(MX_FORM_NAME_T) MX_GEMM_V4_FORMS(MX_FORM_NAME_T)
  MX_GEMM_SMALL_M_FORMS(MX_FORM_NAME_T) MX_GEMM_CONV_SMALL_FORMS(MX_FORM_NAME_P)
};
}
extern "C" int mx_gemm_kernel_name(const mx_gemm_desc* d, int conv, int launch, char* buf, int cap) {
  if (!d || mx::rows_of(d) <= 0 || d->N <= 0 || d->K <= 0 || launch < 0) return -1;
  mx_gemm_desc d1, d2;
  const mx_gemm_desc* q = d;
  if (!conv && mx::tail_split(d, d1, d2)) { if (launch > 1) return 0; q = launch == 0 ? &d1 : &d2; }
  else if (launch > 0) return 0;
  const int form = mx::gemm_kernel_of(q, conv != 0, mx::pick_tile(q, conv != 0));
  if (form < 0) return -1;
  return mx::copy_name(mx::kGemmKernelNames[form], buf, cap);
}
extern "C" int mx_gemm_kernel_names(char* buf, int cap) { return mx::join_names(mx::kGemmKernelNames, mx::GK_COUNT, buf, cap); }
```

### sduss_amd/csrc/gemm_bf16_v2.hip

```cpp
#include <cstdlib>

#include "common.h"
#include "../../include/mxdenoise.h"
#include "gemm_args.h"
#include "gemm_forms.h"
#include "gemm_dma_loader.h"

namespace mx {

template <int BN, int MI> struct RingDepth { static constexpr int value = MI == 4 ? 3 : (BN == 160 ? 4 : 5); };

template <int BN, int MI, bool CONV, int FEAT, bool GEGLU>
__global__ __launch_bounds__(512, 2) void gemm_v2_kernel(const GemmArgs pk) {
  constexpr int BM2 = 64 * MI;
  constexpr int NI = BN / 32;
  constexpr int LOADS = DmaTile<BN, MI>::LOADS;
  constexpr int NSTAGE = RingDepth<BN, MI>::value;
  __shared__ __attribute__((aligned(16))) bf16_t smem[NSTAGE * DmaTile<BN, MI>::STAGE_ELEMS];

  const int tid = threadIdx.x;
  const int lane = tid & 63;
  const int wave = __builtin_amdgcn_readfirstlane(tid >> 6);
  const int wm = wave >> 1;
  const int wn = wave & 1;
  GemmArgs p = pk;
  int tm, tn;
  const int n_tiles = gemm_m_tiles(pk, BM2) * (pk.N / BN);
  const int slice = pk.splitk > 1 ? (int)blockIdx.x / n_tiles : 0;
  const int tile_id = (int)blockIdx.x - slice * n_tiles;
  gemm_tile_of_block(tile_id, gemm_m_tiles(pk, BM2), pk.N / BN, pk.xcd_map, tm, tn);
  gemm_select_seg(p, pk, tm);
  const int nk_all = p.K / DMA_BK;
  const int k_first = pk.splitk > 1 ? (int)((long)nk_all * slice / pk.splitk) : 0;
  const int nk = pk.splitk > 1 ? (int)((long)nk_all * (slice + 1) / pk.splitk) - k_first : nk_all;
  constexpr bool SPLIT_K = true;
#include "gemm_dma_loader.inc"
  auto issue_next = [&](int stage) __attribute__((always_inline)) { issue_group(stage); advance_cursor(); };

  const int fr = lane & 15;
  const int fq = lane >> 4;

  auto load_frags = [&](int stage, int ks, bf16x8 (&wf)[NI], bf16x8 (&xf)[MI]) {
    const bf16_t* sx = smem + stage * STAGE_ELEMS;
    const bf16_t* sw = sx + BM2 * DMA_BK;
#pragma unroll
    for (int i = 0; i < NI; ++i) {
      const int row = wn * (BN / 2) + i * 16 + fr;
      wf[i] = *reinterpret_cast<const bf16x8*>(&sw[row * DMA_BK + swz(row, ks * 4 + fq) * 8]);
    }
#pragma unroll
    for (int j = 0; j < MI; ++j) {
      const int row = wm * 16 * MI + j * 16 + fr;
      xf[j] = *reinterpret_cast<const bf16x8*>(&sx[row * DMA_BK + swz(row, ks * 4 + fq) * 8]);
    }
  };
  constexpr int NM = NI * MI;
  constexpr int NF = NI + MI;

  setup_tile();
#pragma unroll
  for (int st = 0; st < NSTAGE - 1; ++st) issue_next(st);

  int stage = 0;
  {
    f32x4 acc[NI][MI];
#pragma unroll
    for (int i = 0; i < NI; ++i)
#pragma unroll
      for (int j = 0; j < MI; ++j) acc[i][j] = f32x4{0.f, 0.f, 0.f, 0.f};
    float ln_rstd[MI];
#pragma unroll
    for (int j = 0; j < MI; ++j) ln_rstd[j] = 1.0f;
    if constexpr (!CONV) {
      if (p.ln_stats != nullptr) {
        gemm_ln_init<NI, MI>(p, acc, tm * BM2 + wm * 16 * MI, tn * BN + wn * (BN / 2), fr, fq, ln_rstd);
        if (slice != 0) {
#pragma unroll
          for (int i = 0; i < NI; ++i)
#pragma unroll
            for (int j = 0; j < MI; ++j) acc[i][j] = f32x4{0.f, 0.f, 0.f, 0.f};
        }
      }
    }

    for (int kt = 0; kt < nk; ++kt) {
      constexpr int INFLIGHT = LOADS * (NSTAGE - 2);
      wait_vmcnt<INFLIGHT>();
      __builtin_amdgcn_s_barrier();
      bf16x8 wf0[NI], xf0[MI], wf1[NI], xf1[MI];
      load_frags(stage, 0, wf0, xf0);
      const int st2 = stage >= 1 ? stage - 1 : NSTAGE - 1;
      issue_group(st2);
      load_frags(stage, 1, wf1, xf1);
#pragma unroll
      for (int i = 0; i < NI; ++i)
#pragma unroll
        for (int j = 0; j < MI; ++j)
          acc[i][j] = __builtin_amdgcn_mfma_f32_16x16x32_bf16(wf0[i], xf0[j], acc[i][j], 0, 0, 0);
#pragma unroll
      for (int i = 0; i < NI; ++i)
#pragma unroll
        for (int j = 0; j < MI; ++j)
          acc[i][j] = __builtin_amdgcn_mfma_f32_16x16x32_bf16(wf1[i], xf1[j], acc[i][j], 0, 0, 0);
      __builtin_amdgcn_sched_group_barrier(0x100, NF, 0);
#pragma unroll
      for (int s = 0; s < LOADS; ++s) {
        __builtin_amdgcn_sched_group_barrier(0x008, 1, 0);
        __builtin_amdgcn_sched_group_barrier(0x020, 1, 0);
      }
#pragma unroll
      for (int s = 0; s < (NF + 1) / 2; ++s) {
        __builtin_amdgcn_sched_group_barrier(0x008, 1, 0);
        __builtin_amdgcn_sched_group_barrier(0x100, 2, 0);
      }
      __builtin_amdgcn_sched_group_barrier(0x008, 2 * NM - LOADS - (NF + 1) / 2, 0);
      advance_cursor();
      stage = stage == NSTAGE - 1 ? 0 : stage + 1;
    }

    const int m0 = tm * BM2, n0 = tn * BN;
    if (pk.splitk > 1) {
      if (!splitk_combine<NI, MI>(pk, acc, tile_id, slice, BM2 * BN, reinterpret_cast<volatile int*>(smem))) return;
    }
    static_assert(!GEGLU || (NI % 4 == 0 && !CONV), "the gated epilogue pairs whole 32-feature halves");
    gemm_epilogue_regs<NI, MI, GEGLU, true, true, true, FEAT>(p, acc, m0 + wm * 16 * MI, n0 + wn * (BN / 2), fr, fq, ln_rstd);
    wait_vmcnt<0>();
  }
}

int launch_v2(hipStream_t s, const GemmArgs& a, int bn, int form) {
  const int tiles = (a.nseg > 0 ? a.mt_total : cdiv(a.M, 128)) * (a.N / bn) * (a.splitk > 1 ? a.splitk : 1);
  dim3 grid(tiles), block(512);
  switch (form) {
#define MX_V2(id, k, targs) case id: hipLaunchKernelGGL((k<MX_FORM_UNPAREN targs>), grid, block, 0, s, a); return 0;
    MX_GEMM_V2_FORMS(MX_V2)
#undef MX_V2
    default: return 1;
  }
}

}
```

### sduss_amd/csrc/gemm_bf16_v5.hip

```cpp
#include <cstdlib>

#include "common.h"
#include "../../include/mxdenoise.h"
#include "gemm_args.h"
#include "gemm_forms.h"
#include "gemm_v5_body.h"

namespace mx {

template <int BN, int MI, bool CONV, int FEAT, bool GEGLU, bool VEC>
__global__ __launch_bounds__(512, 2) void gemm_v5_kernel(const GemmArgs pk) {
  constexpr int STAGE_ELEMS = (64 * MI + BN) * DMA_BK;
  __shared__ __attribute__((aligned(16))) bf16_t smem[NSTAGE5 * STAGE_ELEMS];
  int tm, tn;
  gemm_tile_of_block(blockIdx.x, gemm_m_tiles(pk, 64 * MI), pk.N / BN, pk.xcd_map, tm, tn);
  gemm_v5_tile<BN, MI, CONV, FEAT, GEGLU, VEC>(pk, tm, tn, smem);
}

int launch_v5(hipStream_t s, const GemmArgs& a, int bn, int rows, int form) {
  const int tiles = (a.nseg > 0 ? a.mt_total : cdiv(a.M, rows)) * (a.N / bn);
  dim3 grid(tiles), block(512);
  switch (form) {
#define MX_V5(id, k, targs) case id: hipLaunchKernelGGL((k<MX_FORM_UNPAREN targs>), grid, block, 0, s, a); return 0;
    MX_GEMM_V5_FORMS(MX_V5)
#undef MX_V5
    default: return 1;
  }
}

}

#if defined(MX_EXP) && MX_EXP == 8
extern "C" int mx_debug_v5_stamps(unsigned long long* out) { return (int)hipMemcpyFromSymbol(out, HIP_SYMBOL(mx::g_v5_stamps), sizeof(mx::g_v5_stamps)); }
#endif
```

### sduss_amd/csrc/gemm_dma_loader.inc

```
  constexpr int BM = DmaTile<BN, MI>::BM, WCH = DmaTile<BN, MI>::WCH, XI = DmaTile<BN, MI>::XI, WI = DmaTile<BN, MI>::WI, STAGE_ELEMS = DmaTile<BN, MI>::STAGE_ELEMS;
  const char* zero = reinterpret_cast<const char*>(g_zero_page);
  const int cs = tid & 7;
  const int tiles_per_tap = CONV ? p.Cin / DMA_BK : 1;

  bool parked = false;
  int is_kt = 0;
  const char* xsrc[XI];
  long xjump[XI];
  const char* wsrc[WI];
  int cb[XI], cy[XI], cx[XI];
  unsigned xchb[XI];
  int tap_next = 0, in_tap = 0;

  auto conv_set_tap = [&](int tap, int cbyte = 0) __attribute__((always_inline)) {
    const int dy = tap / 3 - 1;
    const int dx = tap - (tap / 3) * 3 - 1;
    const int Hv = p.Hin << p.up, Wv = p.Win << p.up;
    const int P = p.corner_patch;
#pragma unroll
    for (int i = 0; i < XI; ++i) {
      int iy = cy[i] + dy;
      const int ix = cx[i] + dx;
      if (P > 0 && dy != 0 && dx != 0) {
        const bool cross_r = ((iy + P) / P) != ((cy[i] + P) / P);
        const bool cross_c = ((ix + P) / P) != ((cx[i] + P) / P);
        if (cross_r && cross_c) iy = cy[i];
      }
      const bool ok = (cb[i] >= 0) && (iy >= -p.vhalo) && (iy < Hv + p.vhalo) && (ix >= 0) && (ix < Wv);
      const long off = ((((long)cb[i] * (p.Hin + 2 * p.vhalo) + (iy >> p.up) + p.vhalo) * p.Win + (ix >> p.up)) * p.Cin) * 2;
      xsrc[i] = (ok ? reinterpret_cast<const char*>(p.a) + off + cbyte : zero) + xchb[i];
    }
  };

  auto setup_tile = [&]() __attribute__((always_inline)) {
    const int m0 = tm * BM;
    const int n0 = tn * BN;
#pragma unroll
    for (int i = 0; i < XI; ++i) {
      const int row = (i * 512 + tid) >> 3;
      const int ch = swz(row, cs);
      const int m = m0 + row;
      if constexpr (!CONV) {
        const int mc = m < p.M ? m : p.M - 1;
        xsrc[i] = reinterpret_cast<const char*>(p.a) + (gemm_in_row(p, mc) * p.lda + ch * 8) * 2;
        xjump[i] = p.a2 != nullptr ? (reinterpret_cast<const char*>(p.a2) + ((long)mc * p.lda2 + ch * 8) * 2) - (xsrc[i] + (long)p.k_split * 2) : 0;
      } else {
        xchb[i] = ch * 16;
        if (m < p.M) {
          const int hw = p.Hout * p.Wout;
          const int b = m / hw;
          const int r = m - b * hw;
          const int oy = r / p.Wout;
          cb[i] = b; cy[i] = oy * p.stride; cx[i] = (r - oy * p.Wout) * p.stride;
        } else {
          cb[i] = -1; cy[i] = 0; cx[i] = 0;
        }
      }
    }
    if constexpr (SPLIT_K) { tap_next = CONV ? k_first / tiles_per_tap : 0; in_tap = CONV ? k_first - tap_next * tiles_per_tap : 0; }
    if constexpr (CONV) conv_set_tap(tap_next, in_tap * DMA_BK * 2);
    else if constexpr (SPLIT_K) {
#pragma unroll
      for (int i = 0; i < XI; ++i) xsrc[i] += (long)k_first * DMA_BK * 2;
    }
#pragma unroll
    for (int i = 0; i < WI; ++i) {
      int q = i * 512 + tid;
      if (q >= WCH) q -= WCH;
      const int row = q >> 3;
      wsrc[i] = reinterpret_cast<const char*>(p.w) + ((long)(n0 + row) * p.K + (long)k_first * DMA_BK + swz(row, cs) * 8) * 2;
    }
  };
  auto park_on_zero_page = [&]() __attribute__((always_inline)) {
#pragma unroll
    for (int i = 0; i < XI; ++i) xsrc[i] = zero + lane * 16;
#pragma unroll
    for (int i = 0; i < WI; ++i) wsrc[i] = zero + lane * 16;
  };

  auto issue_group = [&](int stage) __attribute__((always_inline)) {
    bf16_t* st = smem + stage * STAGE_ELEMS;
    bf16_t* sw = st + BM * DMA_BK;
#pragma unroll
    for (int i = 0; i < XI; ++i) glds16(xsrc[i], st + (i * 512 + wave * 64) * 8);
#pragma unroll
    for (int i = 0; i < WI; ++i) {
      const int qb = (i * 512 + wave * 64 >= WCH) ? i * 512 + wave * 64 - WCH : i * 512 + wave * 64;
      glds16(wsrc[i], sw + qb * 8);
    }
  };
  auto advance_cursor = [&]() __attribute__((always_inline)) {
    if (parked) return;
    if (++is_kt == nk) {
      is_kt = 0;
      parked = true;
      park_on_zero_page();
      return;
    }
#pragma unroll
    for (int i = 0; i < WI; ++i) wsrc[i] += DMA_BK * 2;
    if constexpr (!CONV) {
      const bool to_a2 = p.a2 != nullptr && is_kt * DMA_BK == p.k_split;
#pragma unroll
      for (int i = 0; i < XI; ++i) xsrc[i] += DMA_BK * 2 + (to_a2 ? xjump[i] : 0L);
    } else {
      if (++in_tap == tiles_per_tap) {
        in_tap = 0;
        conv_set_tap(++tap_next);
      } else {
#pragma unroll
        for (int i = 0; i < XI; ++i) xsrc[i] += DMA_BK * 2;
      }
// ... 3 lines not shown
```

### sduss_amd/csrc/gemm_v5_body.h

```cpp
#pragma once
#include "common.h"
#include "../../include/mxdenoise.h"
#include "gemm_args.h"
#include "gemm_dma_loader.h"

namespace mx {

constexpr int NSTAGE5 = 3;

#if defined(MX_EXP) && MX_EXP == 8
static __device__ unsigned long long g_v5_stamps[1024 * 2 * 4];
#define MX5_STAMP(slot) do { if (lane == 0 && (wave == 0 || wave == 7) && blockIdx.x < 1024) \
    g_v5_stamps[(blockIdx.x * 2 + (wave == 7)) * 4 + (slot)] = __builtin_amdgcn_s_memrealtime(); } while (0)
#else
#define MX5_STAMP(slot) do {} while (0)
#endif

template <int BN, int MI, bool CONV, int FEAT, bool GEGLU, bool VEC, bool WT = false>
__device__ __forceinline__ void gemm_v5_tile(const GemmArgs& pk, int tm, const int tn, bf16_t* const smem) {
  constexpr int BM5 = 64 * MI;
  constexpr int NI = BN / 32;
  constexpr int LOADS = DmaTile<BN, MI>::LOADS;

  const int tid = threadIdx.x;
  const int lane = tid & 63;
  const int wave = __builtin_amdgcn_readfirstlane(tid >> 6);
  const int wm = wave >> 1;
  const int wn = wave & 1;
  const bool group_b = wave >= 4;
  MX5_STAMP(0);
  GemmArgs p = pk;
  gemm_select_seg(p, pk, tm);
  const int nk = p.K / DMA_BK;
  constexpr bool SPLIT_K = false;
  constexpr int k_first = 0;
#include "gemm_dma_loader.inc"

  const int fr = lane & 15;
  const int fq = lane >> 4;
  unsigned wrd[2], xrd[2];
#pragma unroll
  for (int ks = 0; ks < 2; ++ks) {
    const int wrow = wn * (BN / 2) + fr, xrow = wm * 16 * MI + fr;
    wrd[ks] = (unsigned)(((BM5 * DMA_BK) + wrow * DMA_BK + swz(wrow, ks * 4 + fq) * 8) * 2);
    xrd[ks] = (unsigned)((xrow * DMA_BK + swz(xrow, ks * 4 + fq) * 8) * 2);
  }

  setup_tile();
  issue_group(0); advance_cursor();
  issue_group(1); advance_cursor();
  wait_vmcnt<LOADS>();

  f32x4 acc[NI][MI];
#pragma unroll
  for (int i = 0; i < NI; ++i)
#pragma unroll
    for (int j = 0; j < MI; ++j) acc[i][j] = f32x4{0.f, 0.f, 0.f, 0.f};
  float ln_rstd[MI];
#pragma unroll
  for (int j = 0; j < MI; ++j) ln_rstd[j] = 1.0f;
  if constexpr (!CONV) {
    if (p.ln_stats != nullptr) gemm_ln_init<NI, MI>(p, acc, tm * BM5 + wm * 16 * MI, tn * BN + wn * (BN / 2), fr, fq, ln_rstd);
  }
  MX_BAR();
  if (group_b) MX_BAR();
  MX5_STAMP(1);

  int stage = 0;
  for (int kt = 0; kt < nk; ++kt) {
    const char* sb = reinterpret_cast<const char*>(smem) + stage * (STAGE_ELEMS * 2);
    bf16x8 wf[2][NI], xf[2][MI];
#pragma unroll
    for (int ks = 0; ks < 2; ++ks) {
#pragma unroll
      for (int i = 0; i < NI; ++i) wf[ks][i] = *reinterpret_cast<const bf16x8*>(sb + wrd[ks] + i * (16 * DMA_BK * 2));
#pragma unroll
      for (int j = 0; j < MI; ++j) xf[ks][j] = *reinterpret_cast<const bf16x8*>(sb + xrd[ks] + j * (16 * DMA_BK * 2));
    }
    const int st2 = stage >= 1 ? stage - 1 : NSTAGE5 - 1;
    issue_group(st2);
    advance_cursor();
    wait_vmcnt<LOADS>();
    asm volatile("s_waitcnt lgkmcnt(0)" ::: "memory");
    __builtin_amdgcn_sched_barrier(0);
    MX_BAR();
    __builtin_amdgcn_s_setprio(1);
#pragma unroll
    for (int ks = 0; ks < 2; ++ks)
#pragma unroll
      for (int i = 0; i < NI; ++i)
#pragma unroll
        for (int j = 0; j < MI; ++j) acc[i][j] = __builtin_amdgcn_mfma_f32_16x16x32_bf16(wf[ks][i], xf[ks][j], acc[i][j], 0, 0, 0);
    __builtin_amdgcn_s_setprio(0);
    MX_BAR();
    stage = stage == NSTAGE5 - 1 ? 0 : stage + 1;
  }
  MX5_STAMP(2);
  if (!group_b) MX_BAR();

  const int m0 = tm * BM5, n0 = tn * BN;
  static_assert(!GEGLU || (NI % 4 == 0 && !CONV), "the gated epilogue pairs whole 32-feature halves");
  gemm_epilogue_regs<NI, MI, GEGLU, VEC, true, true, FEAT, true, false, WT>(p, acc, m0 + wm * 16 * MI, n0 + wn * (BN / 2), fr, fq, ln_rstd);
  if constexpr (!GEGLU && FEAT == 0 && MI == 4) {
    if (pk.gn_part != nullptr) gemm_gn_partials<NI, MI>(p, acc, m0 + wm * 16 * MI, n0 + wn * (BN / 2), fr, fq);
  }
  MX5_STAMP(3);
  wait_vmcnt<0>();
  if constexpr (!CONV && !GEGLU && BM5 == 256) {
    if (pk.ln_final_out != nullptr) gemm_ln_finalize(p, tm, pk.N / BN, reinterpret_cast<volatile int*>(smem));
  }
}


}
```

### sduss_amd/csrc/plan_base.h

```cpp
#pragma once
#include <hip/hip_runtime.h>

#include <cstring>
#include <map>
#include <string>
#include <unordered_map>
#include <vector>

#include "../../include/mxdenoise.h"
#include "common.h"
#include "graph_cache.h"
#include "pp_exchange.h"

namespace mx {
int launch_copy_rows(hipStream_t s, void* batch, void* slotted, size_t bytes_per_sample, int B, const int* slot, int scatter);

struct Arena {
  char* base = nullptr; size_t cap = 0; size_t top = 0; size_t peak = 0; bool dry = false;
  void reset(void* b, size_t c, bool d) { base = (char*)b; cap = c; top = 0; peak = 0; dry = d; }
  void* alloc(size_t bytes) {
    const size_t a = (top + 255) & ~(size_t)255;
    top = a + bytes;
    if (top > peak) peak = top;
    if (dry) return (void*)(uintptr_t)(0x1000 + a);
    return (top <= cap) ? base + a : nullptr;
  }
  size_t mark() const { return top; }
  void release(size_t m) { top = m; }
};

struct WeightTable {
  const char* blob = nullptr;
  uint64_t blob_bytes = 0;
  std::unordered_map<std::string, std::pair<uint64_t, uint64_t>> table;
  int set(const char* who, const void* b, uint64_t bytes, const mx_weight_entry* entries, int n) {
    const std::string p = std::string(who) + ": ";
    MX_CHECK(b && entries && n > 0, p + "bad arguments");
    table.clear();
    for (int i = 0; i < n; ++i) {
      MX_CHECK(entries[i].name != nullptr, p + "null name");
      MX_CHECK(entries[i].offset % 16 == 0, p + "tensor offsets must be 16-byte aligned");
      MX_CHECK(entries[i].offset + entries[i].bytes <= bytes, p + "entry exceeds blob");
      table[entries[i].name] = {entries[i].offset, entries[i].bytes};
    }
    blob = (const char*)b; blob_bytes = bytes;
    return 0;
  }
  const void* find(const std::string& name, size_t bytes, std::string& err) const {
    auto it = table.find(name);
    if (it == table.end()) { err = "missing weight '" + name + "'"; return nullptr; }
    if (it->second.second != bytes) { err = "weight '" + name + "' has " + std::to_string(it->second.second) + " bytes, expected " + std::to_string(bytes); return nullptr; }
    return blob + it->second.first;
  }
};

struct PlanBase {
  const WeightTable* weights = nullptr;
  hipStream_t stream = nullptr;
  Arena ar;
  bool dry = false;
  bool lookup = false;
  bool mute = false;
  std::string err;
  const char* stage = nullptr; void* stage_out = nullptr; size_t stage_bytes = 0; bool stage_hit = false;

  void begin(const WeightTable& wt, hipStream_t s, void* workspace, size_t workspace_bytes) { weights = &wt; stream = s; dry = false; ar.reset(workspace, workspace_bytes, false); }
  void begin_dry(const WeightTable& wt) { weights = &wt; dry = true; ar.reset(nullptr, 0, true); }
  bool ok() const { return err.empty(); }
  bool fail(const std::string& m) { if (err.empty()) err = m; return false; }
  bool quiet() const { return dry || mute; }

  const void* w(const std::string& name, size_t bytes) {
    if (dry && !lookup) return (const void*)(uintptr_t)0x1000;
    std::string e;
    const void* p = weights->find(name, bytes, e);
    if (!p) fail(e);
    return p;
  }
  const bf16_t* wb(const std::string& name, size_t elems) { return (const bf16_t*)w(name, elems * 2); }
  const float* wf(const std::string& name, size_t elems) { return (const float*)w(name, elems * 4); }
  template <typename T> T* alloc(size_t elems) {
    T* p = (T*)ar.alloc(elems * sizeof(T));
    if (!p) fail("workspace too small");
    return p;
  }
  bool gemm(mx_gemm_desc& d, bool conv = false) {
    if (!ok()) return false;
    if (quiet()) return true;
    if (conv ? mx_conv3x3(stream, &d) : mx_gemm(stream, &d)) return fail(std::string("gemm/conv: ") + mx_last_error());
    return true;
  }
  void dump(const std::string& name, const bf16_t* t, size_t elems) {
    if (!stage || quiet() || !ok() || stage_hit) return;
    if (name != stage) return;
    if (elems * 2 > stage_bytes) { fail("stage buffer too small for '" + name + "'"); return; }
    if (hipMemcpyAsync(stage_out, t, elems * 2, hipMemcpyDeviceToDevice, stream) != hipSuccess) fail("stage copy failed");
    stage_hit = true;
  }
  int finish(bool okr, size_t* peak) {
    if (peak) *peak = ar.peak;
    if (!okr) { set_error(err); return 1; }
    return 0;
  }
};

struct Groups {
  int ng = 1, B = 0, H = 0, W = 0;
  int gB[MX_MAX_SEGS], gH[MX_MAX_SEGS], gW[MX_MAX_SEGS], gb0[MX_MAX_SEGS];
  const void* g_lat[MX_MAX_SEGS]; void* g_out[MX_MAX_SEGS];
  void set_single(int batch, int h, int w, const void* lat, void* out) { const mx_unet_group g{lat, out, batch, h, w}; set_groups(&g, 1); }
  void set_groups(const mx_unet_group* groups, int n) {
    ng = n; B = 0; H = groups[0].H; W = groups[0].W;
    for (int g = 0; g < n; ++g) {
      gB[g] = groups[g].batch; gH[g] = groups[g].H; gW[g] = groups[g].W; gb0[g] = B; g_lat[g] = groups[g].latents; g_out[g] = groups[g].out;
      B += groups[g].batch;
    }
  }
};

struct DenoiserPlan : PlanBase, Groups {
  PPExchange px;
  mx_block_cache* bc = nullptr;
  int bc_rows = 0;
  const int* bc_dslot = nullptr;
  std::vector<unsigned char> bc_valid;
  bool bc_all_valid = false, bc_any_valid = false;
  bool bc_keyed = false;
  std::vector<float> h_timesteps;
  static size_t bc_head_bytes(int part_rows, int tables, int rows) {
    return (((size_t)part_rows * rows * 64 * sizeof(double) + (size_t)tables * rows * sizeof(int)) + 255) & ~(size_t)255;
  }
  int* bc_table(int part_rows, int k) const { return (int*)((char*)bc->state + (size_t)part_rows * bc_rows * 64 * sizeof(double)) + (size_t)k * bc_rows; }

  void bc_fold() {
    bc_all_valid = true; bc_any_valid = false;
    for (unsigned char v : bc_valid) { bc_all_valid = bc_all_valid && v; bc_any_valid = bc_any_valid || v; }
  }
  int bc_begin_slots(const std::string& who, mx_block_cache* cache, int batch) {
    bc = cache;
    MX_CHECK(cache->slots && cache->slot_valid && cache->n_slots >= batch, who + ": slots need slot_valid and n_slots >= batch");
    bc_valid.assign(batch, 0);
    std::vector<char> seen(cache->n_slots, 0);
    for (int b = 0; b < batch; ++b) {
      MX_CHECK(cache->slots[b] >= 0 && cache->slots[b] < cache->n_slots && !seen[cache->slots[b]], who + ": slots must be distinct and inside [0, n_slots)");
      seen[cache->slots[b]] = 1;
      bc_valid[b] = cache->slot_valid[b] ? 1 : 0;
    }
    bc_fold();
    return 0;
  }
  int bc_begin(const std::string& who, mx_block_cache* cache, int batch, int h, int w) {
    bc_keyed = true;
    bc_rows = cache->slots ? cache->n_slots : batch;
    if (cache->slots) return bc_begin_slots(who, cache, batch);
    bc = cache;
    cache->cached_valid = cache->cached_valid && cache->cached_key == cache->batch_key && cache->cached_batch == batch && cache->cached_h == h && cache->cached_w == w;
    bc_valid.assign(batch, cache->cached_valid ? 1 : 0);
    bc_fold();
    return 0;
  }
  int bc_send_slots(const std::string& who, int part_rows, int tables, int batch) {
    if (!bc->slots) return 0;
    MX_CHECK(bc_head_bytes(part_rows, tables, bc_rows) <= bc->state_bytes, who + ": state buffer too small");
// ... 129 lines not shown
```

### sduss_amd/csrc/unet_sdxl.cpp

```cpp
#include <hip/hip_runtime.h>

#include <algorithm>
#include <cstring>
#include <functional>
#include <map>
#include <string>
#include <vector>

#include "../../include/mxdenoise.h"
#include "common.h"
#include "graph_cache.h"
#include "patch_cache.h"
#include "plan_base.h"

namespace mx {
int launch_prep_latent(hipStream_t s, const void* in, int dtype, void* out, int B, int Cin, int HW, int CP);
int launch_nhwc_to_nchw(hipStream_t s, const void* in, void* out, int dtype, int B, int C, int HW, int ld);
int launch_time_embed(hipStream_t s, const float* timesteps, const void* text_embeds, const float* time_ids,
                      void* tsin, void* addin, int B, int d0, int text_dim, int da);
int launch_concat(hipStream_t s, const void* a, const void* b, void* out, long M, int C1, int C2);
size_t gn_workspace_exact(int B, int H, int W, int C, int patch);
int launch_sq_diff_partial(hipStream_t s, const void* a, const void* b, long elems_per_sample, int B, double* partial, const int* slot = nullptr);
int launch_gn_pp_partial(hipStream_t s, const void* x, int C1, const void* x2, int B, int H, int W, int C, int groups, void* workspace, double* sums);
int launch_gn_pp_finish(hipStream_t s, const void* x, int C1, const void* x2, void* y, long y_img_elems, const float* gamma, const float* beta, const double* all_sums,
// ... 203 lines not shown
    if (!dry) {
      char* Pc = (char*)P;
      bool e = hipMemcpy2DAsync(send, row, Pc + row, pimg, row, B, hipMemcpyDeviceToDevice, stream) != hipSuccess;
      e |= hipMemcpy2DAsync(send + B * row, row, Pc + (size_t)h * row, pimg, row, B, hipMemcpyDeviceToDevice, stream) != hipSuccess;
      if (e) return fail("halo pack failed");
      if (!all_gather(send, recv, 2 * B * row)) return false;
      if (pp_rank > 0) e |= hipMemcpy2DAsync(Pc, pimg, recv + ((size_t)(pp_rank - 1) * 2 + 1) * B * row, row, row, B, hipMemcpyDeviceToDevice, stream) != hipSuccess;
      else e |= hipMemset2DAsync(Pc, pimg, 0, row, B, stream) != hipSuccess;
      if (pp_rank < pp_world - 1) e |= hipMemcpy2DAsync(Pc + (size_t)(h + 1) * row, pimg, recv + ((size_t)(pp_rank + 1) * 2) * B * row, row, row, B, hipMemcpyDeviceToDevice, stream) != hipSuccess;
      else e |= hipMemset2DAsync(Pc + (size_t)(h + 1) * row, pimg, 0, row, B, stream) != hipSuccess;
      if (e) return fail("halo unpack failed");
    }
    ar.release(m);
    return true;
  }
  bool groupnorm_pp(const bf16_t* x, bf16_t* y, long y_img, const std::string& prefix, int h, int wd, int C, float eps, bool silu, int level,
                    const bf16_t* x2 = nullptr, int C1 = 0) {
    if (!ok()) return false;
    const size_t m = ar.mark();
    const int G = u->cfg.norm_num_groups;
    void* ws = ar.alloc(mx::gn_workspace_exact(B, h, wd, C, 0));
    double* sums = (double*)ar.alloc((size_t)B * G * 2 * sizeof(double));
    double* all = (double*)ar.alloc((size_t)pp_world * B * G * 2 * sizeof(double));
    if (!ws || !sums || !all) return fail("workspace too small");
    const float* g = wf(prefix + ".weight", C); const float* b = wf(prefix + ".bias", C);
    if (ok() && dry) all_gather(sums, all, (size_t)B * G * 2 * sizeof(double));
    if (ok() && !dry) {
      if (mx::launch_gn_pp_partial(stream, x, C1, x2, B, h, wd, C, G, ws, sums)) return fail(std::string("groupnorm: ") + mx_last_error());
      const bool corrected = px.mode == MX_PP_STALE && px.corrected_gn;
      if (!all_gather(sums, all, (size_t)B * G * 2 * sizeof(double), corrected)) return false;
      if (mx::launch_gn_pp_finish(stream, x, C1, x2, y, y_img, g, b, all, pp_world, B, h, wd, C, G, Htot >> level, eps, silu ? 1 : 0, ws,
                                  corrected ? sums : nullptr, pp_rank))
        return fail(std::string("groupnorm: ") + mx_last_error());
    }
    ar.release(m);
    return ok();
  }

  struct RowStats { float* buf = nullptr; int slabs = 0; float* fin = nullptr; unsigned* cnt = nullptr; };
  unsigned* ln_cnt = nullptr;
  static constexpr int kLnCnt = 4096;
  unsigned* tail_sync = nullptr;
  long tail_rows = 0;
  bool gemm_with_stats(mx_gemm_desc& d, RowStats& st, bool finalise = false) {
    if (!ok()) return false;
    const int slabs = mx_gemm_stats_slabs(&d);
    if (finalise) {
      if (slabs <= 0 || !mx_gemm_ln_final_supported(&d) || (d.M + 255) / 256 > kLnCnt) return fail("finalised row statistics: the producing launch cannot write them");
      d.ln_final_out = st.fin; d.ln_final_cnt = st.cnt; d.ln_eps = u->cfg.layer_norm_eps;
    }
    if (slabs > 0) { d.stats_out = st.buf; st.slabs = slabs; return gemm(d, false); }
    st.slabs = 1;
    if (!gemm(d, false)) return false;
    if (!quiet() && mx_row_stats(stream, d.c, d.ldc, st.buf, d.M, d.N)) return fail(std::string("row_stats: ") + mx_last_error());
    return true;
  }
  void use_ln(mx_gemm_desc& d, const RowStats& st, const std::string& csname, bool final = false) {
    if (final) d.ln_final = st.fin; else { d.ln_stats = st.buf; d.ln_slabs = st.slabs; }
    d.ln_colsum = wf(csname, d.N); d.ln_eps = u->cfg.layer_norm_eps;
  }
  bool linear(const bf16_t* a, int lda, const std::string& wname, const std::string& bname, void* c, int ldc, int M, int N,
              int K, const void* residual = nullptr, int ldr = 0, int flags = 0, float out_scale = 0.f, const bf16_t* a2 = nullptr, int lda2 = 0,
              const RowStats* ln = nullptr, RowStats* stats_out = nullptr, bool ln_final = false, bool finalise = false) {
    mx_gemm_desc d; std::memset(&d, 0, sizeof(d));
    d.out_scale = out_scale;
    if (a2) { d.a2 = a2; d.lda2 = lda2; d.k_split = lda; }
    d.a = a; d.lda = lda; d.w = wb(wname, (size_t)N * K); d.bias = bname.empty() ? nullptr : wf(bname, N);
    d.c = c; d.ldc = ldc; d.M = M; d.N = N; d.K = K; d.residual = residual; d.ldr = ldr; d.flags = flags;
    if (ln) use_ln(d, *ln, wname.substr(0, wname.size() - 6) + "colsum", ln_final);
    if (stats_out) return gemm_with_stats(d, *stats_out, finalise);
    return gemm(d, false);
  }
  int conv_cin_valid = 0;
  bool conv(const bf16_t* x, int Hin, int Win, int Cin, const std::string& prefix, bf16_t* out, int Cout, int stride, int up,
            int corner_patch, const float* rowbias = nullptr, int ldrb = 0, const void* residual = nullptr, int vhalo = 0, float* gn_part = nullptr,
            bool* gn_done = nullptr) {
    mx_gemm_desc d; std::memset(&d, 0, sizeof(d));
    d.vhalo = vhalo;
    const int Hv = Hin << up, Wv = Win << up;
    d.a = x; d.w = wb(prefix + ".weight", (size_t)Cout * 9 * Cin); d.bias = wf(prefix + ".bias", Cout);
    d.c = out; d.ldc = Cout; d.B = gB[0]; d.Hin = Hin; d.Win = Win; d.Cin = Cin;
    d.Hout = (Hv + stride - 1) / stride; d.Wout = (Wv + stride - 1) / stride; d.stride = stride; d.up = up;
    d.corner_patch = corner_patch;
    d.M = gB[0] * d.Hout * d.Wout; d.N = Cout; d.K = 9 * Cin;
    d.rowbias = rowbias; d.ldrb = ldrb; d.rows_per_batch = d.Hout * d.Wout;
    d.residual = residual; d.ldr = Cout;
    mx_gemm_seg sg[MX_MAX_SEGS];
    if (ng > 1) {
      std::memset(sg, 0, sizeof(sg));
      long in0 = 0, out0 = 0;
      for (int g = 0; g < ng; ++g) {
        mx_gemm_seg& q = sg[g];
        q.B = gB[g]; q.Hin = ch[g]; q.Win = cw[g];
        q.Hout = ((ch[g] << up) + stride - 1) / stride; q.Wout = ((cw[g] << up) + stride - 1) / stride;
        q.M = gB[g] * q.Hout * q.Wout; q.rows_per_batch = q.Hout * q.Wout;
        q.a = x + in0 * Cin; q.c = out + out0 * Cout;
        q.residual = residual ? (const bf16_t*)residual + out0 * Cout : nullptr;
        q.rowbias = rowbias ? rowbias + (long)gb0[g] * ldrb : nullptr;
        in0 += (long)gB[g] * ch[g] * cw[g]; out0 += q.M;
      }
      d.segs = sg; d.n_segs = ng;
    }
    if (gn_part && gn_done && ng == 1 && mx_gemm_gn_partials_supported(&d, 1)) { d.gn_part_out = gn_part; *gn_done = true; }
    d.cin_valid = conv_cin_valid;
    return gemm(d, true);
  }
  bool groupnorm(const bf16_t* x, bf16_t* y, const std::string& prefix, int h, int wd, int C, float eps, bool silu, int patch,
                 const bf16_t* x2 = nullptr, int C1 = 0) {
    if (!ok()) return false;
    const size_t m = ar.mark();
    mx_gn_problem pr[MX_MAX_SEGS];
    long r0 = 0;
    for (int k = 0; k < ng; ++k) {
      pr[k].x = x + r0 * (x2 ? C1 : C); pr[k].x2 = x2 ? x2 + r0 * (C - C1) : nullptr; pr[k].y = y + r0 * C;
      pr[k].B = gB[k]; pr[k].H = ch[k]; pr[k].W = cw[k];
      r0 += (long)gB[k] * ch[k] * cw[k];
    }
    const size_t need = ng > 1 ? mx_groupnorm_nhwc_grouped_workspace_bytes(pr, ng, C) : mx::gn_workspace_exact(gB[0], h, wd, C, patch);
    void* ws = ar.alloc(need);
    if (!ws) return fail("workspace too small");
    const float* g = wf(prefix + ".weight", C); const float* b = wf(prefix + ".bias", C);
    if (ok() && !quiet()) {
      if (mx_groupnorm_nhwc_grouped(stream, pr, ng, x2 ? C1 : C, g, b, C, u->cfg.norm_num_groups, eps, silu ? 1 : 0, patch, ws))
        fail(std::string("groupnorm: ") + mx_last_error());
    }
    ar.release(m);
    return ok();
  }
  bool groupnorm_from_partials(const bf16_t* x, bf16_t* y, const std::string& prefix, int h, int wd, int C, float eps, bool silu, const float* part,
                               const float* add_bias, const float* add_rowbias, int ldrb) {
    if (!ok()) return false;
    const size_t m = ar.mark();
    void* ws = ar.alloc(mx::gn_workspace_exact(gB[0], h, wd, C, 0));
    if (!ws) return fail("workspace too small");
    const float* g = wf(prefix + ".weight", C); const float* b = wf(prefix + ".bias", C);
    if (ok() && !quiet()) {
      if (mx_groupnorm_nhwc_from_partials(stream, x, y, g, b, gB[0], h, wd, C, u->cfg.norm_num_groups, eps, silu ? 1 : 0, part, 64, add_bias, add_rowbias, ldrb, ws))
        fail(std::string("groupnorm: ") + mx_last_error());
    }
    ar.release(m);
    return ok();
  }
  bool attention(const bf16_t* q, int ldq, const bf16_t* k, int ldk, const bf16_t* vt, int ldvt, long vt_bstride, bf16_t* o,
                 int ldo, int heads, int Lq, int Lk) {
    if (!ok()) return false;
    if (quiet()) return true;
    if (mx_attention_prescaled(stream, q, ldq, k, ldk, vt, ldvt, vt_bstride, o, ldo, B, heads, Lq, Lk))
      return fail(std::string("attention: ") + mx_last_error());
    return true;
  }
  bool attention_grouped(const mx_attn_problem* pr, int ldq, int ldk, int ldo, int heads) {
    if (!ok()) return false;
    if (quiet()) return true;
    if (mx_attention_prescaled_grouped(stream, pr, ng, ldq, ldk, ldo, heads)) return fail(std::string("attention: ") + mx_last_error());
    return true;
  }
  int level_patch(int level) const { return gn_patch > 0 ? std::max(gn_patch >> level, 1) : 0; }

  bf16_t* resnet(const std::string& p, const bf16_t* x, int h, int wd, int Cin, int Cout, int level, const bf16_t* x2 = nullptr, int C2 = 0) {
    const int M = (int)rows();
    const int C1 = Cin - C2;
    bf16_t* out = alloc<bf16_t>((size_t)M * Cout);
    const size_t m = ar.mark();
    const int patch = level_patch(level);
    if (is_pp()) {
      bf16_t* n1p = alloc_padded(h, wd, Cin);
// ... 1112 lines not shown
```

### sduss_amd/lib.py

```python
from __future__ import annotations

import ctypes as C
import os
from typing import Optional

_HERE = os.path.dirname(os.path.abspath(__file__))
LIB_PATH = os.path.join(_HERE, "libmxdenoise.so")

MX_F32, MX_F16, MX_BF16 = 0, 1, 2
EPI_SILU, EPI_GEGLU, EPI_OUT_F32, EPI_QKV, EPI_GELU_TANH, EPI_RES_BCAST, EPI_RMSNORM, EPI_GELU, EPI_QUICK_GELU, EPI_GEGLU_TANH = 1, 2, 4, 8, 16, 32, 64, 128, 256, 512


class MxError(RuntimeError):
    """Raised for every non-zero status of the C ABI (the reference's launcher only printed
    cudaGetLastError and went on -- norm_silu_concat.cu:434-437; SURVEY.md section 8b asks to raise)."""


MAX_SEGS = 4


class GemmSeg(C.Structure):
    _fields_ = [
        ("a", C.c_void_p), ("a2", C.c_void_p), ("c", C.c_void_p), ("residual", C.c_void_p), ("vt", C.c_void_p), ("rowbias", C.c_void_p),
        ("gate", C.c_void_p), ("ln_stats", C.c_void_p), ("stats_out", C.c_void_p),
        ("M", C.c_int), ("rows_per_batch", C.c_int), ("ldvt", C.c_int),
        ("B", C.c_int), ("Hin", C.c_int), ("Win", C.c_int), ("Hout", C.c_int), ("Wout", C.c_int),
        ("a_batch_rows", C.c_int), ("a_row_off", C.c_int), ("c_batch_rows", C.c_int), ("c_row_off", C.c_int),
    ]


class GemmDesc(C.Structure):
    _fields_ = [
        ("a", C.c_void_p), ("w", C.c_void_p), ("c", C.c_void_p), ("bias", C.c_void_p), ("rowbias", C.c_void_p),
        ("residual", C.c_void_p), ("vt", C.c_void_p),
        ("M", C.c_int), ("N", C.c_int), ("K", C.c_int),
        ("lda", C.c_int), ("ldc", C.c_int), ("ldr", C.c_int), ("ldrb", C.c_int),
        ("rows_per_batch", C.c_int), ("flags", C.c_int),
        ("seg", C.c_int), ("period", C.c_int), ("ldvt", C.c_int),
        ("B", C.c_int), ("Hin", C.c_int), ("Win", C.c_int), ("Cin", C.c_int),
        ("Hout", C.c_int), ("Wout", C.c_int), ("stride", C.c_int), ("up", C.c_int), ("corner_patch", C.c_int),
        ("a_batch_rows", C.c_int), ("a_row_off", C.c_int), ("c_batch_rows", C.c_int), ("c_row_off", C.c_int),
        ("gate", C.c_void_p), ("ldg", C.c_int), ("out_scale", C.c_float), ("rms_wq", C.c_void_p), ("rms_wk", C.c_void_p), ("rms_eps", C.c_float), ("vhalo", C.c_int), ("a2", C.c_void_p), ("lda2", C.c_int), ("k_split", C.c_int),
        ("ln_stats", C.c_void_p), ("ln_colsum", C.c_void_p), ("ln_slabs", C.c_int), ("ln_eps", C.c_float), ("stats_out", C.c_void_p),
        ("segs", C.POINTER(GemmSeg)), ("n_segs", C.c_int), ("splitk", C.c_int),
        ("ln_final", C.c_void_p), ("ln_final_out", C.c_void_p), ("ln_final_cnt", C.c_void_p), ("gn_part_out", C.c_void_p), ("cin_valid", C.c_int),
    ]


class AttnTailDesc(C.Structure):
    _fields_ = [("out1", GemmDesc), ("to_q", GemmDesc), ("out2", GemmDesc),
                ("k", C.c_void_p), ("ldk", C.c_int), ("vt", C.c_void_p), ("ldvt", C.c_int), ("vt_batch_stride", C.c_int64),
                ("B", C.c_int), ("heads", C.c_int), ("L", C.c_int), ("ctx_len", C.c_int), ("sync", C.c_void_p)]


class AttnProblem(C.Structure):
    _fields_ = [("q", C.c_void_p), ("k", C.c_void_p), ("vt", C.c_void_p), ("o", C.c_void_p), ("vt_batch_stride", C.c_int64),
                ("B", C.c_int), ("Lq", C.c_int), ("Lk", C.c_int), ("ldvt", C.c_int)]


class GnProblem(C.Structure):
    _fields_ = [("x", C.c_void_p), ("x2", C.c_void_p), ("y", C.c_void_p), ("B", C.c_int), ("H", C.c_int), ("W", C.c_int)]


class UNetGroup(C.Structure):
    _fields_ = [("latents", C.c_void_p), ("out", C.c_void_p), ("batch", C.c_int), ("H", C.c_int), ("W", C.c_int)]


class UNetConfigC(C.Structure):
    _fields_ = [
        ("in_channels", C.c_int), ("out_channels", C.c_int), ("n_levels", C.c_int),
        ("block_out_channels", C.c_int * 4), ("layers_per_block", C.c_int),
        ("down_has_attn", C.c_int * 4), ("transformer_layers", C.c_int * 4), ("num_heads", C.c_int * 4),
        ("cross_attention_dim", C.c_int), ("addition_time_embed_dim", C.c_int),
        ("projection_class_embeddings_input_dim", C.c_int), ("norm_num_groups", C.c_int),
        ("norm_eps", C.c_float), ("transformer_norm_eps", C.c_float), ("layer_norm_eps", C.c_float),
    ]


class MMDiTConfigC(C.Structure):
    _fields_ = [
        ("patch_size", C.c_int), ("in_channels", C.c_int), ("out_channels", C.c_int), ("num_layers", C.c_int),
        ("num_attention_heads", C.c_int), ("joint_attention_dim", C.c_int), ("pooled_projection_dim", C.c_int),
        ("pos_embed_max_size", C.c_int), ("dual_attention", C.c_int * 64), ("norm_eps", C.c_float),
    ]


ALLGATHER_FN = C.CFUNCTYPE(C.c_int, C.c_void_p, C.c_void_p, C.c_void_p, C.c_void_p, C.c_size_t)


class PPComm(C.Structure):
    _fields_ = [("rank", C.c_int), ("world", C.c_int), ("all_gather", ALLGATHER_FN), ("ctx", C.c_void_p)]


ALLGATHER_INPLACE_FN = C.CFUNCTYPE(C.c_int, C.c_void_p, C.c_void_p, C.c_void_p, C.c_size_t)
PP_SYNC, PP_WARMUP, PP_STALE = 0, 1, 2


class PPStale(C.Structure):
    _fields_ = [("state", C.c_void_p), ("state_bytes", C.c_size_t), ("mode", C.c_int), ("corrected_gn", C.c_int),
                ("all_gather_async", ALLGATHER_INPLACE_FN)]


SKIP_PREDICT_FN = C.CFUNCTYPE(C.c_int, C.c_void_p, C.c_int, C.c_int, C.c_int, C.c_int, C.POINTER(C.c_float), C.POINTER(C.c_float),
                              C.POINTER(C.c_ubyte))
MSE_UNCACHED = 9.2233720368547758e18


SKIP_OBSERVE_FN = C.CFUNCTYPE(None, C.c_void_p, C.c_int, C.c_int, C.POINTER(C.c_float))


class BlockCacheC(C.Structure):
    _fields_ = [("predict", SKIP_PREDICT_FN), ("ctx", C.c_void_p), ("state", C.c_void_p), ("state_bytes", C.c_size_t),
                ("batch_key", C.c_uint64), ("cached_key", C.c_uint64), ("cached_valid", C.c_int), ("cached_batch", C.c_int),
                ("cached_h", C.c_int), ("cached_w", C.c_int), ("blocks_run", C.c_uint), ("blocks_run_hi", C.c_uint), ("observe", SKIP_OBSERVE_FN),
                ("slots", C.POINTER(C.c_int32)), ("slot_valid", C.POINTER(C.c_ubyte)), ("n_slots", C.c_int),
                ("max_h", C.c_int), ("max_w", C.c_int), ("patches_asked", C.c_ulonglong), ("patches_total", C.c_ulonglong)]


class CLIPConfigC(C.Structure):
    _fields_ = [("vocab_size", C.c_int), ("hidden_size", C.c_int), ("intermediate_size", C.c_int), ("num_hidden_layers", C.c_int),
                ("num_attention_heads", C.c_int), ("max_position_embeddings", C.c_int), ("hidden_act", C.c_int), ("projection_dim", C.c_int),
                ("eos_token_id", C.c_int), ("hidden_layer", C.c_int), ("layer_norm_eps", C.c_float)]


class T5ConfigC(C.Structure):
    _fields_ = [("vocab_size", C.c_int), ("d_model", C.c_int), ("d_ff", C.c_int), ("num_layers", C.c_int), ("num_heads", C.c_int),
                ("layer_norm_epsilon", C.c_float)]

# ... 199 lines not shown
```

### sduss_amd/ops.py

```python
from __future__ import annotations

import ctypes as C
from typing import Optional

import torch

from . import lib as _lib


def _p(t: Optional[torch.Tensor]):
    return None if t is None else t.data_ptr()


def _bf16(t):
    assert t.is_cuda and t.dtype == torch.bfloat16 and t.is_contiguous(), "expected a contiguous CUDA bf16 tensor"
    return t


def gemm(a: torch.Tensor, w: torch.Tensor, bias: Optional[torch.Tensor] = None, residual: Optional[torch.Tensor] = None,
         rowbias: Optional[torch.Tensor] = None, rows_per_batch: int = 0, silu: bool = False, geglu: bool = False,
         out_f32: bool = False, out_scale: float = 0.0, ln_stats: Optional[torch.Tensor] = None, ln_colsum: Optional[torch.Tensor] = None,
         ln_eps: float = 1e-5, want_stats: bool = False, splitk: int = 0, ln_final: Optional[torch.Tensor] = None, want_final: bool = False,
         final_buffers=None):
    l = _lib.load()
# ... 24 lines not shown
        slabs = l.mx_gemm_stats_slabs(C.byref(d))
        stats = torch.full((m, stats_pitch(max(slabs, 1)), 2), float("nan"), dtype=torch.float32, device=a.device)
        if slabs > 0:
            d.stats_out = stats.data_ptr()
            if want_final and l.mx_gemm_ln_final_supported(C.byref(d)):
                if final_buffers is not None:
                    final, cnt = final_buffers
                else:
                    final = torch.full((m, 2), float("nan"), dtype=torch.float32, device=a.device)
                    cnt = torch.zeros((m + 255) // 256, dtype=torch.int32, device=a.device)
                d.ln_final_out, d.ln_final_cnt, d.ln_eps = final.data_ptr(), cnt.data_ptr(), ln_eps
    _lib.check(l.mx_gemm(_lib.current_stream(), C.byref(d)), "mx_gemm")
    if want_stats:
        if not d.stats_out:
            _lib.check(l.mx_row_stats(_lib.current_stream(), c.data_ptr(), nout, stats.data_ptr(), m, nout), "mx_row_stats")
        if want_final:
            if final is not None and final_buffers is None:
                assert int(cnt.abs().sum()) == 0, "ln_final_cnt must be zero again after the launch"
            return c, (stats, max(slabs, 1)), final
        return c, (stats, max(slabs, 1))
    return c


def stats_pitch(slabs: int) -> int:
    return (slabs + 3) & ~3


def row_stats(x: torch.Tensor) -> torch.Tensor:
    l = _lib.load()
    _bf16(x)
    m, c = x.shape
    st = torch.full((m, 4, 2), float("nan"), dtype=torch.float32, device=x.device)
    _lib.check(l.mx_row_stats(_lib.current_stream(), x.data_ptr(), c, st.data_ptr(), m, c), "mx_row_stats")
    return st, 1


def vt_ld(lk: int) -> int:
    return (lk + 15) // 16 * 16


def vt_pos(lk: int) -> torch.Tensor:
    k = torch.arange(lk)
    return (k & ~12) | ((k & 4) << 1) | ((k & 8) >> 1)


def pack_vt(v: torch.Tensor, pad: float = 0.0) -> torch.Tensor:
    b, lk, c = v.shape
    vt = torch.full((b, c, vt_ld(lk)), pad, dtype=v.dtype, device=v.device)
    vt[:, :, vt_pos(lk).to(v.device)] = v.permute(0, 2, 1)
    return vt


def unpack_vt(vt: torch.Tensor, lk: int) -> torch.Tensor:
    return vt[:, :, vt_pos(lk).to(vt.device)].permute(0, 2, 1)


def gemm_qkv(a: torch.Tensor, w: torch.Tensor, seg: int, period: int, rows_per_batch: int, q_scale: float = 0.0,
             ln_stats: Optional[torch.Tensor] = None, ln_colsum: Optional[torch.Tensor] = None, ln_eps: float = 1e-5,
             bias: Optional[torch.Tensor] = None, ln_final: Optional[torch.Tensor] = None):
    l = _lib.load()
    _bf16(a); _bf16(w)
    m, k = a.shape
    n = w.shape[0]
    nb = m // rows_per_batch
    ldvt = vt_ld(rows_per_batch)
    c = torch.empty((m, n // period * (period - 1)), dtype=torch.bfloat16, device=a.device)
    vt = torch.zeros((nb, n // period, ldvt), dtype=torch.bfloat16, device=a.device)
    d = _lib.GemmDesc()
    d.a, d.w, d.c, d.vt = a.data_ptr(), w.data_ptr(), c.data_ptr(), vt.data_ptr()
    d.M, d.N, d.K, d.lda, d.ldc = m, n, k, k, c.shape[1]
    d.rows_per_batch, d.flags, d.seg, d.period, d.ldvt = rows_per_batch, _lib.EPI_QKV, seg, period, ldvt
    d.out_scale = q_scale
    d.bias = _p(bias)
    if ln_stats is not None:
        d.ln_stats, d.ln_colsum, d.ln_slabs, d.ln_eps = ln_stats[0].data_ptr(), ln_colsum.data_ptr(), ln_stats[1], ln_eps
    if ln_final is not None:
        d.ln_final, d.ln_colsum, d.ln_eps = ln_final.data_ptr(), ln_colsum.data_ptr(), ln_eps
    _lib.check(l.mx_gemm(_lib.current_stream(), C.byref(d)), "mx_gemm(qkv)")
    return c, vt


def conv3x3(x: torch.Tensor, w: torch.Tensor, bias: Optional[torch.Tensor], stride: int = 1, up: int = 0,
            corner_patch: int = 0, rowbias: Optional[torch.Tensor] = None, residual: Optional[torch.Tensor] = None, splitk: int = 0, want_gn_partials: bool = False,
            cin_valid: int = 0):
    l = _lib.load()
    _bf16(x); _bf16(w)
    b, h, wd, cin = x.shape
    cout = w.shape[0]
    hv, wv = h << up, wd << up
    ho, wo = (hv + stride - 1) // stride, (wv + stride - 1) // stride
    c = torch.empty((b, ho, wo, cout), dtype=torch.bfloat16, device=x.device)
    d = _lib.GemmDesc()
    d.a, d.w, d.c, d.bias, d.rowbias, d.residual = x.data_ptr(), w.data_ptr(), c.data_ptr(), _p(bias), _p(rowbias), _p(residual)
    d.M, d.N, d.K, d.ldc, d.ldr = b * ho * wo, cout, 9 * cin, cout, cout
    d.ldrb = rowbias.shape[1] if rowbias is not None else 0
    d.rows_per_batch = ho * wo
    d.B, d.Hin, d.Win, d.Cin, d.Hout, d.Wout, d.stride, d.up, d.corner_patch = b, h, wd, cin, ho, wo, stride, up, corner_patch
    d.splitk = splitk
    d.cin_valid = cin_valid
    part = None
    if want_gn_partials and l.mx_gemm_gn_partials_supported(C.byref(d), 1):
        part = torch.full((b * ho * wo // 64, cout, 2), float("nan"), dtype=torch.float32, device=x.device)
        d.gn_part_out = part.data_ptr()
    _lib.check(l.mx_conv3x3(_lib.current_stream(), C.byref(d)), "mx_conv3x3")
    if want_gn_partials:
        return c, part
    return c


ATTN_QSCALE = 0.125 * 1.4426950408889634


def attention(q: torch.Tensor, k: torch.Tensor, vt: torch.Tensor, heads: int, lq: int, lk: int, prescaled: bool = False) -> torch.Tensor:
    l = _lib.load()
    _bf16(q); _bf16(k); _bf16(vt)
    b = vt.shape[0]
    o = torch.empty_like(q)
    if prescaled:
        _lib.check(l.mx_attention_prescaled(_lib.current_stream(), q.data_ptr(), q.shape[1], k.data_ptr(), k.shape[1], vt.data_ptr(),
                                            vt.shape[2], vt.shape[1] * vt.shape[2], o.data_ptr(), o.shape[1], b, heads, lq, lk),
                   "mx_attention_prescaled")
        return o
    _lib.check(l.mx_attention(_lib.current_stream(), q.data_ptr(), q.shape[1], k.data_ptr(), k.shape[1], vt.data_ptr(),
                              vt.shape[2], vt.shape[1] * vt.shape[2], o.data_ptr(), o.shape[1], b, heads, lq, lk,
                              0.125), "mx_attention")
    return o


def attn_tail(ao: torch.Tensor, y: torch.Tensor, w1: torch.Tensor, b1: torch.Tensor, wq: torch.Tensor, bq: torch.Tensor, colsum_q: torch.Tensor,
              k: torch.Tensor, vt: torch.Tensor, w2: torch.Tensor, b2: torch.Tensor, heads: int, L: int, ctx_len: int, ln_eps: float = 1e-5,
              chained: bool = True, finalise: bool = True, sync: Optional[torch.Tensor] = None):
    l = _lib.load()
    for t_ in (ao, y, w1, wq, w2, k, vt):
        _bf16(t_)
    m, c = y.shape
    b = m // L
    dev = y.device
    y = y.clone()
    q2 = torch.empty_like(y)
    ao2 = torch.empty_like(y)
    td = _lib.AttnTailDesc()

    def lin(d, a_, w_, bias, c_, res):
        d.a, d.w, d.c, d.bias = a_.data_ptr(), w_.data_ptr(), c_.data_ptr(), bias.data_ptr()
        d.M, d.N, d.K, d.lda, d.ldc = m, c, c, c, c
        if res is not None:
            d.residual, d.ldr = res.data_ptr(), c
    lin(td.out1, ao, w1, b1, y, y)
    lin(td.to_q, y, wq, bq, q2, None)
    lin(td.out2, ao2, w2, b2, y, y)
    td.out1.stats_out = 16
    slabs = l.mx_gemm_stats_slabs(C.byref(td.out1))
    assert slabs > 0, "out1 cannot write slab statistics at this shape"
    st1 = torch.full((m, stats_pitch(slabs), 2), float("nan"), dtype=torch.float32, device=dev)
    st2 = torch.full((m, stats_pitch(slabs), 2), float("nan"), dtype=torch.float32, device=dev)
    td.out1.stats_out = st1.data_ptr()
    td.to_q.ln_stats, td.to_q.ln_colsum, td.to_q.ln_slabs, td.to_q.ln_eps = st1.data_ptr(), colsum_q.data_ptr(), slabs, ln_eps
    td.to_q.out_scale = ATTN_QSCALE
    td.out2.stats_out = st2.data_ptr()
    final = cnt = None
    if finalise:
        final = torch.full((m, 2), float("nan"), dtype=torch.float32, device=dev)
        cnt = torch.zeros((m + 255) // 256, dtype=torch.int32, device=dev)
        td.out2.ln_final_out, td.out2.ln_final_cnt, td.out2.ln_eps = final.data_ptr(), cnt.data_ptr(), ln_eps
    td.k, td.ldk, td.vt, td.ldvt, td.vt_batch_stride = k.data_ptr(), k.shape[1], vt.data_ptr(), vt.shape[2], vt.shape[1] * vt.shape[2]
    td.B, td.heads, td.L, td.ctx_len = b, heads, L, ctx_len
    stream = _lib.current_stream()
    if chained:
        if sync is None:
            sync = torch.zeros(l.mx_attn_tail_sync_bytes(m) // 4, dtype=torch.int32, device=dev)
        td.sync = sync.data_ptr()
        assert l.mx_attn_tail_supported(C.byref(td)), "mx_attn_tail cannot serve this shape"
        _lib.check(l.mx_attn_tail(stream, C.byref(td)), "mx_attn_tail")
    else:
        _lib.check(l.mx_gemm(stream, C.byref(td.out1)), "mx_gemm")
        _lib.check(l.mx_gemm(stream, C.byref(td.to_q)), "mx_gemm")
        _lib.check(l.mx_attention_cross_prescaled(stream, q2.data_ptr(), c, k.data_ptr(), k.shape[1], vt.data_ptr(), vt.shape[2], vt.shape[1] * vt.shape[2],
                                                  ao2.data_ptr(), c, b, heads, L, ctx_len), "mx_attention_cross_prescaled")
        _lib.check(l.mx_gemm(stream, C.byref(td.out2)), "mx_gemm")
    return y, (st2, slabs), final, q2, ao2, sync


# ... 100 lines not shown
```

### sduss_amd/unet.py

```python
from __future__ import annotations

import ctypes as C
from typing import Dict, List, Optional

import torch

from . import lib as _lib
from .config import UNetConfig
from .weights import PackedWeights, pack


class _Config(dict):
    __getattr__ = dict.__getitem__


def _row_ids(ids, n_rows):
    return [f"{ids[i % len(ids)]}#{i // len(ids)}" for i in range(n_rows)]


class MxUNet:

    def __init__(self, cfg: UNetConfig, params: Dict[str, torch.Tensor], device="cuda:0"):
        self.cfg = cfg
        self.device = torch.device(device)
        self.dtype = torch.bfloat16
        self._lib = _lib.load()
        cc = _lib.UNetConfigC()
        cc.in_channels, cc.out_channels = cfg.in_channels, cfg.out_channels
        cc.n_levels = len(cfg.block_out_channels)
        for i, v in enumerate(cfg.block_out_channels):
            cc.block_out_channels[i] = v
            cc.down_has_attn[i] = int(cfg.down_has_attn[i])
            cc.transformer_layers[i] = cfg.transformer_layers_per_block[i]
            cc.num_heads[i] = cfg.num_heads[i]
        cc.layers_per_block = cfg.layers_per_block
        cc.cross_attention_dim = cfg.cross_attention_dim
        cc.addition_time_embed_dim = cfg.addition_time_embed_dim
        cc.projection_class_embeddings_input_dim = cfg.projection_class_embeddings_input_dim
        cc.norm_num_groups = cfg.norm_num_groups
        cc.norm_eps, cc.transformer_norm_eps, cc.layer_norm_eps = cfg.norm_eps, cfg.transformer_norm_eps, cfg.layer_norm_eps
        self._handle = self._lib.mx_unet_create(C.byref(cc))
        if not self._handle:
            raise _lib.MxError("mx_unet_create: " + self._lib.mx_last_error().decode())
        self.weights = PackedWeights(pack(cfg, params), self.device)
        _lib.check(self._lib.mx_unet_set_weights(self._handle, self.weights.blob.data_ptr(), self.weights.blob.numel(),
                                                 self.weights.table, len(self.weights.names)), "mx_unet_set_weights")
        self.mixed_one_sequence = True
        self.max_mixed_groups = _lib.MAX_SEGS
        self._ws_by_stream: Dict[int, Optional[torch.Tensor]] = {}
        self._ws_need = {}
        self._next_ctx_key = 0
        self.config = _Config(in_channels=cfg.in_channels, time_cond_proj_dim=None,
                              addition_time_embed_dim=cfg.addition_time_embed_dim,
                              projection_class_embeddings_input_dim=cfg.projection_class_embeddings_input_dim,
                              sample_size=128, center_input_sample=False)

    def __del__(self):
        h = getattr(self, "_handle", None)
        if h:
            self._lib.mx_unet_destroy(h)
            self._handle = None

    def to(self, *args, **kwargs):
        return self

    def set_context_key(self, key: int) -> None:
        self._next_ctx_key = int(key)

    def _apply_ctx_key(self) -> None:
        key, self._next_ctx_key = self._next_ctx_key, 0
        _lib.check(self._lib.mx_unet_set_context_key(self._handle, key), "mx_unet_set_context_key")

    def context_stats(self):
        h, m = C.c_long(0), C.c_long(0)
        _lib.check(self._lib.mx_unet_context_stats(self._handle, C.byref(h), C.byref(m)), "mx_unet_context_stats")
        return h.value, m.value

    def _workspace(self, batch: int, h: int, w: int, ctx_len: int, stream: int) -> torch.Tensor:
        key = (batch, h, w, ctx_len)
        need = self._ws_need.get(key)
        if need is None:
            need = self._ws_need[key] = self._lib.mx_unet_workspace_bytes(self._handle, batch, h, w, ctx_len)
        if need == 0:
            raise _lib.MxError("mx_unet_workspace_bytes: " + self._lib.mx_last_error().decode())
        ws = self._ws_by_stream.get(stream)
        if ws is None or ws.numel() < need:
            self._ws_by_stream[stream] = None
            ws = self._ws_by_stream[stream] = torch.empty(need, dtype=torch.uint8, device=self.device)
        return ws

    def forward_one(self, sample: torch.Tensor, timestep: torch.Tensor, encoder_hidden_states: torch.Tensor,
                    text_embeds: torch.Tensor, time_ids: torch.Tensor, gn_patch: int = 0,
                    stage: Optional[str] = None, stage_shape=None) -> torch.Tensor:
        assert sample.is_cuda and sample.ndim == 4
        sample = sample.contiguous()
        b, _c, h, w = sample.shape
        ctx_len = encoder_hidden_states.shape[1]
        ts = timestep.to(device=self.device, dtype=torch.float32).reshape(-1)
        if ts.numel() == 1:
            ts = ts.expand(b)
        ts = ts.contiguous()
        ehs = encoder_hidden_states.to(device=self.device, dtype=torch.bfloat16).contiguous()
        te = text_embeds.to(device=self.device, dtype=torch.bfloat16).contiguous()
        ti = time_ids.to(device=self.device, dtype=torch.float32).contiguous()
        assert ts.shape[0] == b and ehs.shape[0] == b and te.shape[0] == b and ti.shape == (b, 6)
        assert ehs.shape[2] == self.cfg.cross_attention_dim and te.shape[1] == self.cfg.text_embed_dim
        out = torch.empty((b, self.cfg.out_channels, h, w), dtype=sample.dtype, device=self.device)
        code = _lib.torch_dtype_code(sample.dtype)
        stream = _lib.current_stream()
        ws = self._workspace(b, h, w, ctx_len, int(stream or 0))
        if stage is None:
            self._apply_ctx_key()
            _lib.check(self._lib.mx_unet_forward(self._handle, stream, sample.data_ptr(), code, ts.data_ptr(), ehs.data_ptr(),
                                                 te.data_ptr(), ti.data_ptr(), out.data_ptr(), b, h, w, ctx_len, gn_patch,
                                                 ws.data_ptr(), ws.numel()), "mx_unet_forward")
            return out
        st = torch.empty(stage_shape, dtype=torch.bfloat16, device=self.device)
        _lib.check(self._lib.mx_unet_forward_trace(self._handle, stream, sample.data_ptr(), code, ts.data_ptr(), ehs.data_ptr(),
                                                   te.data_ptr(), ti.data_ptr(), out.data_ptr(), b, h, w, ctx_len, gn_patch,
                                                   ws.data_ptr(), ws.numel(), stage.encode(), st.data_ptr(),
                                                   st.numel() * 2), "mx_unet_forward_trace")
        return st

    def forward_mixed(self, samples: List[torch.Tensor], timestep: torch.Tensor, encoder_hidden_states: torch.Tensor,
                      text_embeds: torch.Tensor, time_ids: torch.Tensor, gn_patch: int = 0, stage: Optional[str] = None) -> List[torch.Tensor]:
        assert 1 <= len(samples) <= _lib.MAX_SEGS, f"a mixed batch holds up to {_lib.MAX_SEGS} resolutions"
        if not torch.is_tensor(timestep):
# ... 200 lines not shown
```

### sduss_amd/weights.py

```python
from __future__ import annotations

import ctypes as C
import os
from typing import Dict, List, Optional, Tuple

import torch

from . import lib as _lib
from .config import UNetConfig, param_shapes, resnet_names, transformer_names

_ALIGN = 256
CONV_IN_PAD = 64


def synthetic_params(cfg: UNetConfig, device="cpu", seed: int = 10086) -> Dict[str, torch.Tensor]:
    g = torch.Generator(device=device).manual_seed(seed)
    out = {}
    for name, shape in sorted(param_shapes(cfg).items()):
        if name.endswith(".weight") and len(shape) >= 2:
            fan_in = 1
            for d in shape[1:]:
                fan_in *= d
            t = torch.randn(shape, generator=g, device=device) * fan_in ** -0.5
        elif name.endswith(".weight"):
            t = 1.0 + 0.1 * torch.randn(shape, generator=g, device=device)
        else:
            t = 0.05 * torch.randn(shape, generator=g, device=device)
        out[name] = t.to(torch.bfloat16)
    return out


def load_safetensors_dir(unet_dir: str) -> Tuple[UNetConfig, Dict[str, torch.Tensor]]:
    from safetensors.torch import load_file
    cfg = UNetConfig.from_hf_json(os.path.join(unet_dir, "config.json"))
    params: Dict[str, torch.Tensor] = {}
    files = sorted(f for f in os.listdir(unet_dir) if f.endswith(".safetensors"))
    if not files:
        raise FileNotFoundError(f"no .safetensors under {unet_dir}")
    pick = [f for f in files if "fp16" not in f] or files
    for f in pick:
        params.update(load_file(os.path.join(unet_dir, f)))
    return cfg, params


def load_mmdit_safetensors_dir(transformer_dir: str):
    from safetensors.torch import load_file
    from .config import MMDiTConfig
    cfg = MMDiTConfig.from_hf_json(os.path.join(transformer_dir, "config.json"))
    files = sorted(f for f in os.listdir(transformer_dir) if f.endswith(".safetensors"))
    if not files:
        raise FileNotFoundError(f"no .safetensors under {transformer_dir}")
    params: Dict[str, torch.Tensor] = {}
    for f in [f for f in files if "fp16" not in f] or files:
        params.update(load_file(os.path.join(transformer_dir, f)))
    return cfg, params


def _conv_pack(w: torch.Tensor, pad_in: int = 0) -> torch.Tensor:
    o, i, kh, kw = w.shape
    w = w.permute(0, 2, 3, 1)
    if pad_in and pad_in > i:
        w = torch.nn.functional.pad(w, (0, pad_in - i))
    return w.reshape(o, -1).contiguous()


def fold_layernorm(w: torch.Tensor, bias: Optional[torch.Tensor], gamma: torch.Tensor, beta: torch.Tensor):
    w32 = w.to(torch.float32)
    wf = (w32 * gamma.to(torch.float32)[None, :]).to(torch.bfloat16)
    colsum = wf.to(torch.float32).sum(dim=1)
    b = w32 @ beta.to(torch.float32)
    if bias is not None:
        b = b + bias.to(torch.float32)
    return wf.contiguous(), colsum.contiguous(), b.contiguous()


def params_as_held(cfg: UNetConfig, P: Dict[str, torch.Tensor]) -> Dict[str, torch.Tensor]:
    out = dict(P)
    for p, _dim, _h, layers in transformer_names(cfg):
        for k in range(layers):
            b = f"{p}.transformer_blocks.{k}"
            for names, nn in (((f"{b}.attn1.to_q.weight", f"{b}.attn1.to_k.weight", f"{b}.attn1.to_v.weight"), "norm1"),
                              ((f"{b}.attn2.to_q.weight",), "norm2"), ((f"{b}.ff.net.0.proj.weight",), "norm3")):
                g = P[f"{b}.{nn}.weight"].to(torch.float32)
                safe = torch.where(g.abs() > 1e-6, g, torch.ones_like(g))
                for n in names:
                    w = P[n].to(torch.float32)
                    held = (w * g[None, :]).to(torch.bfloat16).to(torch.float32) / safe[None, :]
                    out[n] = torch.where(g.abs()[None, :] > 1e-6, held, w).to(P[n].dtype)
    return out


def _geglu_interleave(t: torch.Tensor) -> torch.Tensor:
    half = t.shape[0] // 2
    h = t[:half].reshape(half // 32, 32, *t.shape[1:])
    g = t[half:].reshape(half // 32, 32, *t.shape[1:])
    return torch.cat([h, g], dim=1).reshape(t.shape).contiguous()


def pack(cfg: UNetConfig, P: Dict[str, torch.Tensor]) -> List[Tuple[str, torch.Tensor]]:
    missing = [k for k in param_shapes(cfg) if k not in P]
    if missing:
        raise KeyError(f"state dict lacks {len(missing)} tensors, e.g. {missing[:3]}")
    bf, f32 = torch.bfloat16, torch.float32
    out: List[Tuple[str, torch.Tensor]] = []

    def mat(name, t):
        out.append((name, t.to(bf).contiguous()))

    def vec(name, t):
        out.append((name, t.to(f32).contiguous()))

    mat("conv_in.weight", _conv_pack(P["conv_in.weight"], CONV_IN_PAD))
    vec("conv_in.bias", P["conv_in.bias"])
    for nm in ("time_embedding", "add_embedding"):
        for l in ("linear_1", "linear_2"):
            mat(f"{nm}.{l}.weight", P[f"{nm}.{l}.weight"])
            vec(f"{nm}.{l}.bias", P[f"{nm}.{l}.bias"])
    res = resnet_names(cfg)
    mat("temb_proj_all.weight", torch.cat([P[f"{p}.time_emb_proj.weight"] for p, _, _ in res], dim=0))
    vec("temb_proj_all.bias", torch.cat([P[f"{p}.time_emb_proj.bias"] for p, _, _ in res], dim=0))
    for p, cin, cout in res:
        vec(f"{p}.norm1.weight", P[f"{p}.norm1.weight"]); vec(f"{p}.norm1.bias", P[f"{p}.norm1.bias"])
        mat(f"{p}.conv1.weight", _conv_pack(P[f"{p}.conv1.weight"])); vec(f"{p}.conv1.bias", P[f"{p}.conv1.bias"])
        vec(f"{p}.norm2.weight", P[f"{p}.norm2.weight"]); vec(f"{p}.norm2.bias", P[f"{p}.norm2.bias"])
        mat(f"{p}.conv2.weight", _conv_pack(P[f"{p}.conv2.weight"])); vec(f"{p}.conv2.bias", P[f"{p}.conv2.bias"])
        if cin != cout:
            mat(f"{p}.conv_shortcut.weight", P[f"{p}.conv_shortcut.weight"].reshape(cout, cin))
            vec(f"{p}.conv_shortcut.bias", P[f"{p}.conv_shortcut.bias"])
    kv_by_dim: Dict[int, List[torch.Tensor]] = {}
    for p, dim, _h, layers in transformer_names(cfg):
        vec(f"{p}.norm.weight", P[f"{p}.norm.weight"]); vec(f"{p}.norm.bias", P[f"{p}.norm.bias"])
        for l in ("proj_in", "proj_out"):
            mat(f"{p}.{l}.weight", P[f"{p}.{l}.weight"].reshape(dim, dim)); vec(f"{p}.{l}.bias", P[f"{p}.{l}.bias"])
        for k in range(layers):
            b = f"{p}.transformer_blocks.{k}"
            def folded(name, w, bias, nn):
                wf, cs, bf_ = fold_layernorm(w, bias, P[f"{b}.{nn}.weight"], P[f"{b}.{nn}.bias"])
                mat(f"{name}.weight", wf); vec(f"{name}.colsum", cs); vec(f"{name}.bias", bf_)
            folded(f"{b}.attn1.to_qkv", torch.cat([P[f"{b}.attn1.to_q.weight"], P[f"{b}.attn1.to_k.weight"], P[f"{b}.attn1.to_v.weight"]], dim=0),
                   None, "norm1")
            mat(f"{b}.attn1.to_out.0.weight", P[f"{b}.attn1.to_out.0.weight"]); vec(f"{b}.attn1.to_out.0.bias", P[f"{b}.attn1.to_out.0.bias"])
            folded(f"{b}.attn2.to_q", P[f"{b}.attn2.to_q.weight"], None, "norm2")
            kv_by_dim.setdefault(dim, []).append(torch.cat([P[f"{b}.attn2.to_k.weight"], P[f"{b}.attn2.to_v.weight"]], dim=0))
            mat(f"{b}.attn2.to_out.0.weight", P[f"{b}.attn2.to_out.0.weight"]); vec(f"{b}.attn2.to_out.0.bias", P[f"{b}.attn2.to_out.0.bias"])
            folded(f"{b}.ff.net.0.proj", _geglu_interleave(P[f"{b}.ff.net.0.proj.weight"]), _geglu_interleave(P[f"{b}.ff.net.0.proj.bias"]), "norm3")
            mat(f"{b}.ff.net.2.weight", P[f"{b}.ff.net.2.weight"]); vec(f"{b}.ff.net.2.bias", P[f"{b}.ff.net.2.bias"])
    for dim, lst in kv_by_dim.items():
        mat(f"attn2_kv_all.{dim}.weight", torch.cat(lst, dim=0))
    n = len(cfg.block_out_channels)
    for i in range(n - 1):
        for p in (f"down_blocks.{i}.downsamplers.0.conv", f"up_blocks.{i}.upsamplers.0.conv"):
            mat(f"{p}.weight", _conv_pack(P[f"{p}.weight"])); vec(f"{p}.bias", P[f"{p}.bias"])
    vec("conv_norm_out.weight", P["conv_norm_out.weight"]); vec("conv_norm_out.bias", P["conv_norm_out.bias"])
    co = P["conv_out.weight"].shape[0]
    pad = (-co) % 4
    w = _conv_pack(P["conv_out.weight"]); bias = P["conv_out.bias"]
    if pad:
        w = torch.nn.functional.pad(w, (0, 0, 0, pad)); bias = torch.nn.functional.pad(bias, (0, pad))
    mat("conv_out.weight", w); vec("conv_out.bias", bias)
    return out


class PackedWeights:

    def __init__(self, entries: List[Tuple[str, torch.Tensor]], device):
        total = 0
        offs = []
        for _n, t in entries:
            total = (total + _ALIGN - 1) // _ALIGN * _ALIGN
            offs.append(total)
            total += t.numel() * t.element_size()
        self.blob = torch.empty(total + _ALIGN, dtype=torch.uint8, device=device)
        self.names = []
        for (name, t), off in zip(entries, offs):
            nb = t.numel() * t.element_size()
            self.blob[off:off + nb].copy_(t.reshape(-1).view(torch.uint8).to(device), non_blocking=False)
            self.names.append((name, off, nb))
        self.nbytes = total
        self._keep = [n.encode() for n, _, _ in self.names]
        arr = (_lib.WeightEntry * len(self.names))()
        for i, (n, off, nb) in enumerate(self.names):
            arr[i].name = self._keep[i]
            arr[i].offset = off
            arr[i].bytes = nb
        self.table = arr


def synthetic_mmdit_params(cfg, device="cpu", seed: int = 10086) -> Dict[str, torch.Tensor]:
    from .config import mmdit_param_shapes
    g = torch.Generator(device=device).manual_seed(seed)
    out = {}
    for name, shape in sorted(mmdit_param_shapes(cfg).items()):
        if name == "pos_embed.pos_embed":
            t = 0.5 * torch.randn(shape, generator=g, device=device)
        elif name.endswith(("norm_q.weight", "norm_k.weight", "norm_added_q.weight", "norm_added_k.weight")):
            t = 1.0 + 0.1 * torch.randn(shape, generator=g, device=device)
        elif name.endswith(".weight"):
            fan_in = 1
            for d in shape[1:]:
                fan_in *= d
            gain = 0.3 if (".norm1" in name or "norm_out" in name) else 1.0
            t = torch.randn(shape, generator=g, device=device) * gain * fan_in ** -0.5
        else:
            t = 0.05 * torch.randn(shape, generator=g, device=device)
        out[name] = t.to(torch.bfloat16)
    return out


def pack_mmdit(cfg, P: Dict[str, torch.Tensor]) -> List[Tuple[str, torch.Tensor]]:
    from .config import mmdit_param_shapes
    missing = [k for k in mmdit_param_shapes(cfg) if k not in P]
    if missing:
        raise KeyError(f"state dict lacks {len(missing)} tensors, e.g. {missing[:3]}")
    bf, f32 = torch.bfloat16, torch.float32
    out: List[Tuple[str, torch.Tensor]] = []

    def mat(name, t):
        out.append((name, t.to(bf).contiguous()))

    def vec(name, t):
        out.append((name, t.to(f32).contiguous()))

    def lin(dst, src):
        mat(f"{dst}.weight", P[f"{src}.weight"]); vec(f"{dst}.bias", P[f"{src}.bias"])

    d = cfg.dim
    mat("pos_embed.table", P["pos_embed.pos_embed"].reshape(-1, d))
    mat("pos_embed.proj.weight", _conv_pack(P["pos_embed.proj.weight"]))
    vec("pos_embed.proj.bias", P["pos_embed.proj.bias"])
    for n in ("time_text_embed.timestep_embedder.linear_1", "time_text_embed.timestep_embedder.linear_2",
              "time_text_embed.text_embedder.linear_1", "time_text_embed.text_embedder.linear_2", "context_embedder"):
        lin(n, n)
    ada_w, ada_b = [], []
    for i in range(cfg.num_layers):
        b = f"transformer_blocks.{i}"
        for n in (f"{b}.norm1.linear", f"{b}.norm1_context.linear"):
            ada_w.append(P[f"{n}.weight"]); ada_b.append(P[f"{n}.bias"])
    ada_w.append(P["norm_out.linear.weight"]); ada_b.append(P["norm_out.linear.bias"])
    mat("adaln_all.weight", torch.cat(ada_w, dim=0)); vec("adaln_all.bias", torch.cat(ada_b, dim=0))
    for i in range(cfg.num_layers):
        b = f"transformer_blocks.{i}"
        last = i == cfg.num_layers - 1
# ... 22 lines not shown
```

Measured before the change: 1.435 images/s.

## Collapse nearest-upsample + 3x3 conv into four phase-wise 2x2 convs

Precomputes per-phase summed 2x2 kernels for the upsampler convolutions at weight-pack time. The GEMM kernels get a new view where each of the four output phases runs as an extra grid dimension over the low-resolution input with K=4*Cin instead of 9*Cin. This scatters results to the interleaved upsampled output rows. It cuts redundant multiply-adds that come from sampling duplicated upsampled pixels, at the cost of extra weight storage and bf16 rounding of the summed taps.

```diff
diff --git a/include/mxdenoise.h b/include/mxdenoise.h
--- a/include/mxdenoise.h
+++ b/include/mxdenoise.h
@@ -98,6 +98,7 @@
   unsigned* ln_final_cnt;
   float* gn_part_out;
   int cin_valid;
+  const void* w_up4;
 } mx_gemm_desc;
 
 int mx_gemm(void* stream, const mx_gemm_desc* d);
diff --git a/sduss_amd/csrc/gemm_args.h b/sduss_amd/csrc/gemm_args.h
--- a/sduss_amd/csrc/gemm_args.h
+++ b/sduss_amd/csrc/gemm_args.h
@@ -37,6 +37,7 @@
   float rms_eps;
   int stagger_ticks;
   int vhalo;
+  int phase;
   const bf16_t* a2;
   int lda2, k_split;
   const float* ln_stats;
@@ -71,6 +72,21 @@
   return s;
 }
 __device__ __forceinline__ int gemm_m_tiles(const GemmArgs& p, int rows) { return p.nseg > 0 ? p.mt_total : (p.M + rows - 1) / rows; }
+
+constexpr int MX_CONV_UP4_VIEW = 2;
+__host__ __device__ constexpr bool conv_up4_form(bool conv, int feat, bool geglu, bool vec) { return conv && feat == 0 && !geglu && !vec; }
+__device__ __forceinline__ void gemm_set_phase(GemmArgs& q, const GemmArgs& p, int phase) {
+  q.phase = phase;
+  q.w = p.w + (long)phase * p.N * p.K;
+}
+__device__ __forceinline__ int conv_up4_out_row(const GemmArgs& p, int m) {
+  const unsigned hw = (unsigned)(p.Hin * p.Win);
+  const unsigned b = (unsigned)m / hw;
+  const unsigned r = (unsigned)m - b * hw;
+  const unsigned y = r / (unsigned)p.Win;
+  const unsigned x = r - y * (unsigned)p.Win;
+  return (int)(((b * 2u * p.Hin + 2u * y + (unsigned)(p.phase >> 1)) * 2u * p.Win) + 2u * x + (unsigned)(p.phase & 1));
+}
 
 __device__ __forceinline__ f32x4 fma4(const f32x4 a, const float s, const f32x4 c) {
   return f32x4{fmaf(a[0], s, c[0]), fmaf(a[1], s, c[1]), fmaf(a[2], s, c[2]), fmaf(a[3], s, c[3])};
@@ -276,7 +292,7 @@
   return (long)bidx * p.c_batch_rows + p.c_row_off + (m - bidx * p.rows_per_batch);
 }
 
-template <int NI, int MI, int BN>
+template <int NI, int MI, int BN, bool CONV = false>
 __device__ __forceinline__ void gemm_epilogue(const GemmArgs& p, f32x4 (&acc)[NI][MI], const int m_wave0,
                                               const int wave_n0, const int fr, const int fq) {
   const int flags = p.flags;
@@ -312,7 +328,7 @@
     }
     if (m >= p.M) continue;
     const int bidx = (p.rows_per_batch > 0) ? (m / p.rows_per_batch) : 0;
-    const long orow = gemm_out_row(p, m, bidx);
+    const long orow = (CONV && p.up == MX_CONV_UP4_VIEW) ? (long)conv_up4_out_row(p, m) : gemm_out_row(p, m, bidx);
     const long rrow = (flags & MX_EPI_RES_BCAST) ? (long)(m - bidx * p.rows_per_batch) : orow;
 #pragma unroll
     for (int i = 0; i < (NI); ++i) {
@@ -457,7 +473,8 @@
   const int acts = flags & (MX_EPI_SILU | MX_EPI_GELU | MX_EPI_GELU_TANH | MX_EPI_QUICK_GELU | MX_EPI_GEGLU_TANH);
   return ((flags & MX_EPI_QKV) ? EPI_F_QKV : 0) | (acts == 0 ? 0 : acts == MX_EPI_GELU_TANH ? EPI_F_TANH : EPI_F_ACT);
 }
-template <int NI, int MI, bool GEGLU, bool VEC = true, bool VPF = true, bool STATS = true, int FEAT = EPI_F_ALL, bool EMIT = STATS, bool RSTD_LOAD = false, bool WT = false>
+template <int NI, int MI, bool GEGLU, bool VEC = true, bool VPF = true, bool STATS = true, int FEAT = EPI_F_ALL, bool EMIT = STATS, bool RSTD_LOAD = false, bool WT = false,
+          bool UP4 = false>
 __device__ __forceinline__ void gemm_epilogue_regs(const GemmArgs& p, f32x4 (&acc)[NI][MI], const int m_wave0, const int wave_n0,
                                                    const int fr, const int fq, const float (&ln_rstd_a)[MI]) {
 #pragma clang fp contract(off)
@@ -543,7 +560,14 @@
   const int mA0 = (m_wave0 + fr) & ~1;
   int row_a[MI], row_b[MI];
   int bo_walk = 0, ro_walk = 0;
-  {
+  if (UP4 && p.up == MX_CONV_UP4_VIEW) {
+#pragma unroll
+    for (int j = 0; j < MI; ++j) {
+      const int mA = mA0 + 16 * j;
+      row_a[j] = conv_up4_out_row(p, mA < p.M ? mA : p.M - 1);
+      row_b[j] = conv_up4_out_row(p, mA + 1 < p.M ? mA + 1 : p.M - 1);
+    }
+  } else {
     int bA = p.rows_per_batch > 0 ? mA0 / p.rows_per_batch : 0;
     int rA = mA0 - bA * (p.rows_per_batch > 0 ? p.rows_per_batch : 0);
 #pragma unroll
diff --git a/sduss_amd/csrc/gemm_bf16.hip b/sduss_amd/csrc/gemm_bf16.hip
--- a/sduss_amd/csrc/gemm_bf16.hip
+++ b/sduss_amd/csrc/gemm_bf16.hip
@@ -32,6 +32,7 @@
   GemmArgs p = pk;
   int tm = blockIdx.x;
   gemm_select_seg(p, pk, tm);
+  if constexpr (CONV) { if (pk.up == MX_CONV_UP4_VIEW) gemm_set_phase(p, pk, blockIdx.z); }
   const int m0 = tm * BM;
   const int n0 = blockIdx.y * BN;
   const int nk = p.K / BK;
@@ -83,9 +84,11 @@
     } else {
       const int tap = k0 / p.Cin;
       const int c0 = k0 - tap * p.Cin;
-      const int dy = tap / 3 - 1;
-      const int dx = tap - (tap / 3) * 3 - 1;
-      const int Hv = p.Hin << p.up, Wv = p.Win << p.up;
+      const bool up4 = p.up == MX_CONV_UP4_VIEW;
+      const int ush = up4 ? 0 : p.up;
+      const int dy = up4 ? (tap >> 1) + (p.phase >> 1) - 1 : tap / 3 - 1;
+      const int dx = up4 ? (tap & 1) + (p.phase & 1) - 1 : tap - (tap / 3) * 3 - 1;
+      const int Hv = p.Hin << ush, Wv = p.Win << ush;
       const int P = p.corner_patch;
 #pragma unroll
       for (int i = 0; i < 4; ++i) {
@@ -98,7 +101,7 @@
         }
         const bool ok = (cb[i] >= 0) && (iy >= -p.vhalo) && (iy < Hv + p.vhalo) && (ix >= 0) && (ix < Wv);
         if (ok) {
-          const long src = (((long)cb[i] * (p.Hin + 2 * p.vhalo) + (iy >> p.up) + p.vhalo) * p.Win + (ix >> p.up)) * p.Cin + c0 + sch * 8;
+          const long src = (((long)cb[i] * (p.Hin + 2 * p.vhalo) + (iy >> ush) + p.vhalo) * p.Win + (ix >> ush)) * p.Cin + c0 + sch * 8;
           rx[i] = *reinterpret_cast<const u32x4*>(p.a + src);
         } else {
           rx[i] = zero4;
@@ -161,7 +164,7 @@
     __syncthreads();
   }
 
-  gemm_epilogue<NI, MI, BN>(p, acc, m0 + wm * 64, n0 + wn * (BN / 2), fr, fq);
+  gemm_epilogue<NI, MI, BN, CONV>(p, acc, m0 + wm * 64, n0 + wn * (BN / 2), fr, fq);
 }
 
 int launch_v2(hipStream_t s, const GemmArgs& a, int bn, int form);
@@ -190,6 +193,21 @@
   for (int i = 0; i < d->n_segs; ++i) m += d->segs[i].M;
   return m;
 }
+static bool conv_up4_serves(const mx_gemm_desc* d) {
+  static const bool off = [] { const char* e = getenv("MX_CONV_UP4"); return e && e[0] == '0'; }();
+  if (off || !d->w_up4 || d->up != 1 || d->stride != 1 || d->corner_patch != 0 || d->vhalo != 0 || d->cin_valid != 0) return false;
+  if (d->flags != 0 || d->rowbias || d->residual || d->gate || d->out_scale != 0.f || d->gn_part_out || d->c_batch_rows > 0) return false;
+  if (d->Cin <= 0 || d->K != 9 * d->Cin) return false;
+  if (d->n_segs <= 0) return d->Hout == 2 * d->Hin && d->Wout == 2 * d->Win && (long)d->B * d->Hout * d->Wout == d->M;
+  if (d->n_segs > MX_MAX_SEGS || !d->segs) return false;
+  for (int i = 0; i < d->n_segs; ++i) {
+    const mx_gemm_seg& g = d->segs[i];
+    if (g.c_batch_rows > 0 || g.Hout != 2 * g.Hin || g.Wout != 2 * g.Win || (long)g.B * g.Hout * g.Wout != g.M) return false;
+  }
+  return true;
+}
+static int phases_of(const mx_gemm_desc* d, bool conv) { return conv && d->up == MX_CONV_UP4_VIEW ? 4 : 1; }
+
 static TileChoice pick_tile(const mx_gemm_desc* d, bool conv) {
   constexpr double v3_discount = 0.87;
   const TileChoice none = {0, 0};
@@ -226,7 +244,7 @@
     if (qkv && d->seg % 64 != 0) continue;
     if ((d->flags & MX_EPI_RMSNORM) && bn == 160) continue;
     if (qkv && bn != 256 && d->seg % (bn / 2) != 0) continue;
-    const long tiles = m_tiles_of(d, rows) * (d->N / bn);
+    const long tiles = m_tiles_of(d, rows) * (d->N / bn) * phases_of(d, conv);
     const int ncu = cu_count();
     const double cost = (double)((tiles + ncu - 1) / ncu) * (rows + bn) * (bn == 256 ? v3_discount : 1.0);
     if (best.rows == 0 || cost < best_cost) { best = cands[c]; best_cost = cost; }
@@ -364,6 +382,24 @@
   return conv ? GK_GEN64_CONV : GK_GEN64;
 }
 
+struct ConvView { mx_gemm_desc d; mx_gemm_seg segs[MX_MAX_SEGS]; };
+static bool conv_up4_carried_by(int form) {
+  return form == GK_V5_160_CONV || form == GK_V5_128_CONV || form == GK_V2_160_CONV || form == GK_V2_128_CONV || form == GK_GEN128_CONV || form == GK_GEN64_CONV;
+}
+static const mx_gemm_desc* conv_view(const mx_gemm_desc* d, bool conv, ConvView& v) {
+  if (!conv || !d || !conv_up4_serves(d)) return d;
+  v.d = *d;
+  v.d.w = d->w_up4; v.d.w_up4 = nullptr; v.d.up = MX_CONV_UP4_VIEW; v.d.K = 4 * d->Cin; v.d.splitk = 1;
+  v.d.Hout = d->Hin; v.d.Wout = d->Win; v.d.M = d->M / 4; v.d.rows_per_batch = 0;
+  for (int i = 0; i < d->n_segs; ++i) {
+    v.segs[i] = d->segs[i];
+    v.segs[i].Hout = v.segs[i].Hin; v.segs[i].Wout = v.segs[i].Win; v.segs[i].M /= 4; v.segs[i].rows_per_batch = 0;
+  }
+  if (d->n_segs > 0) v.d.segs = v.segs;
+  if (rows_of(&v.d) <= 0 || !conv_up4_carried_by(gemm_kernel_of(&v.d, true, pick_tile(&v.d, true)))) return d;
+  return &v.d;
+}
+
 static int prepare(void* stream, const mx_gemm_desc* d, bool conv, GemmArgs& a, TileChoice& tc_out) {
   MX_CHECK(d != nullptr, "gemm: null descriptor");
   MX_CHECK(d->a && d->w && (d->c || (d->flags & MX_EPI_QKV)), "gemm: null operand");
@@ -388,7 +424,8 @@
       MX_CHECK(g.M % g.rows_per_batch == 0 && g.ldvt >= MX_VT_LD(g.c_batch_rows > 0 ? g.c_batch_rows : g.rows_per_batch) && g.ldvt % 8 == 0,
                "gemm: grouped launch: QKV needs whole batches and ldvt >= MX_VT_LD(keys per batch)");
     if (conv) {
-      const int Hv = g.Hin << d->up, Wv = g.Win << d->up;
+      const int ush = d->up == MX_CONV_UP4_VIEW ? 0 : d->up;
+      const int Hv = g.Hin << ush, Wv = g.Win << ush;
       MX_CHECK(g.Hout == (Hv + d->stride - 1) / d->stride && g.Wout == (Wv + d->stride - 1) / d->stride && (long)g.B * g.Hout * g.Wout == g.M,
                "conv3x3: grouped launch: a problem's output grid does not match its input grid / stride / rows");
     }
@@ -404,7 +441,7 @@
   a.M = d->M; a.N = d->N; a.K = d->K; a.lda = d->lda; a.ldc = d->ldc; a.ldr = d->ldr; a.ldrb = d->ldrb;
   a.rows_per_batch = d->rows_per_batch; a.flags = d->flags; a.seg = d->seg; a.period = d->period; a.ldvt = d->ldvt;
   a.B = d->B; a.Hin = d->Hin; a.Win = d->Win; a.Cin = d->Cin; a.Hout = d->Hout; a.Wout = d->Wout;
-  a.stride = d->stride; a.up = d->up; a.corner_patch = d->corner_patch;
+  a.stride = d->stride; a.up = conv ? d->up : 0; a.corner_patch = d->corner_patch; a.phase = 0;
   a.a_batch_rows = d->a_batch_rows; a.a_row_off = d->a_row_off; a.c_batch_rows = d->c_batch_rows; a.c_row_off = d->c_row_off;
   a.gate = d->gate; a.ldg = d->ldg; a.out_scale = d->out_scale;
   a.rms_wq = d->rms_wq; a.rms_wk = d->rms_wk; a.rms_eps = d->rms_eps;
@@ -433,12 +470,13 @@
   } else if (!conv) {
     MX_CHECK(d->lda >= d->K && d->lda % 8 == 0, "gemm: lda must be >= K and a multiple of 8");
   } else {
-    MX_CHECK(d->Cin % BK == 0 && d->K == 9 * d->Cin, "conv3x3: Cin must be a multiple of 64 and K = 9*Cin");
+    MX_CHECK(d->Cin % BK == 0 && d->K == (d->up == MX_CONV_UP4_VIEW ? 4 : 9) * d->Cin, "conv3x3: Cin must be a multiple of 64 and K = 9*Cin (4*Cin in the collapsed upsampler view)");
     MX_CHECK(d->stride == 1 || d->stride == 2, "conv3x3: stride must be 1 or 2");
-    MX_CHECK(d->up == 0 || d->up == 1, "conv3x3: up must be 0 or 1");
+    MX_CHECK(d->up == 0 || d->up == 1 || d->up == MX_CONV_UP4_VIEW, "conv3x3: up must be 0, 1 or the collapsed upsampler view");
     MX_CHECK(!(d->up && d->stride != 1), "conv3x3: upsample only with stride 1");
     if (!grouped) {
-      const int Hv = d->Hin << d->up, Wv = d->Win << d->up;
+      const int ush = d->up == MX_CONV_UP4_VIEW ? 0 : d->up;
+      const int Hv = d->Hin << ush, Wv = d->Win << ush;
       MX_CHECK(d->Hout == (Hv + d->stride - 1) / d->stride && d->Wout == (Wv + d->stride - 1) / d->stride,
                "conv3x3: output grid does not match input grid / stride");
       MX_CHECK((long)d->B * d->Hout * d->Wout == d->M, "conv3x3: M != B*Hout*Wout");
@@ -461,7 +499,7 @@
     const long in_rows = (!conv && d->a_batch_rows > 0) ? (long)(d->M / d->rows_per_batch + 1) * d->a_batch_rows : d->M;
     MX_CHECK(in_rows * (conv ? 1 : d->lda) < 2147483647L, "gemm: operand exceeds 32-bit indexing");
   }
-  MX_CHECK((long)d->N * d->K < 2147483647L, "gemm: operand exceeds 32-bit indexing");
+  MX_CHECK((long)d->N * d->K * phases_of(d, conv) < 2147483647L, "gemm: operand exceeds 32-bit indexing");
   if (d->residual) MX_CHECK(d->ldr >= d->N && d->ldr % 4 == 0, "gemm: bad ldr");
   const bool use128 = (d->N % 128 == 0);
   const TileChoice tc = pick_tile(d, conv);
@@ -542,6 +580,12 @@
 static int launch(void* stream, const mx_gemm_desc* d, bool conv) {
   GemmArgs a;
   TileChoice tc;
+  ConvView view;
+  if (conv && d) {
+    MX_CHECK(d->up == 0 || d->up == 1, "conv3x3: up must be 0 or 1");
+    if (d->w_up4) MX_CHECK(((uintptr_t)d->w_up4 & 15) == 0, "conv3x3: w_up4 must be 16-byte aligned");
+    d = conv_view(d, true, view);
+  }
   if (int rc = prepare(stream, d, conv, a, tc)) return rc;
   const bool grouped = d->n_segs > 0;
   const bool use128 = (d->N % 128 == 0);
@@ -549,8 +593,8 @@
   dim3 block(256);
   hipStream_t s = (hipStream_t)stream;
   if (prof_enabled()) {
-    const double kk = conv ? 9.0 * d->Cin : (double)d->K;
-    const double Mt = (double)rows_of(d);
+    const double kk = (double)d->K;
+    const double Mt = (double)rows_of(d) * phases_of(d, conv);
     double in_elems = conv ? (double)d->B * d->Hin * d->Win * d->Cin : Mt * d->K;
     if (conv && grouped) { in_elems = 0; for (int i = 0; i < d->n_segs; ++i) in_elems += (double)d->segs[i].B * d->segs[i].Hin * d->segs[i].Win * d->Cin; }
     const double flops = 2.0 * Mt * (double)d->N * kk;
@@ -563,6 +607,7 @@
   const int form = gemm_kernel_of(d, conv, tc);
   MX_CHECK(form >= 0, v2bn == 256 ? "gemm: no 256 x 256 instantiation serves ln_final with this epilogue (GEGLU, QKV or plain bias only)"
                                    : "gemm: no kernel instantiation serves this descriptor");
+  if (a.up == MX_CONV_UP4_VIEW) MX_CHECK(conv_up4_carried_by(form), "conv3x3: the collapsed upsampler view reached an instantiation that does not carry it");
   if (is_small_m_form(form)) {
     MX_CHECK(launch_small_m(s, a, form) == 0, "gemm: the small-M launcher was handed a form outside its list");
   } else if (form == GK_CONV_SMALL_N) {
@@ -575,7 +620,7 @@
     if (tc.rows == 256) MX_CHECK(launch_v5(s, a, v2bn, tc.rows, form) == 0, "gemm: the 256-row launcher was handed a form outside its list");
     else MX_CHECK(launch_v2(s, a, v2bn, form) == 0, "gemm: the 128-row launcher was handed a form outside its list");
   } else {
-    const dim3 grid(mt128, use128 ? d->N / 128 : cdiv(d->N, 64));
+    const dim3 grid(mt128, use128 ? d->N / 128 : cdiv(d->N, 64), phases_of(d, conv));
     switch (form) {
 #define MX_GEN(id, k, targs) case id: hipLaunchKernelGGL((k<MX_FORM_UNPAREN targs>), grid, block, 0, s, a); break;
       MX_GEMM_GENERIC_FORMS(MX_GEN)
@@ -631,6 +676,8 @@
 extern "C" int mx_gemm_launches(const mx_gemm_desc* d) { mx_gemm_desc d1, d2; return d != nullptr && mx::tail_split(d, d1, d2) ? 2 : 1; }
 extern "C" int mx_gemm_form(const mx_gemm_desc* d, int conv) {
   if (!d || mx::rows_of(d) <= 0 || d->N <= 0 || d->K <= 0) return MX_FORM_TILE_GENERIC;
+  mx::ConvView view;
+  d = mx::conv_view(d, conv != 0, view);
   if (mx::small_m_serves(d, conv != 0)) return MX_FORM_SMALL_M;
   if (conv && mx::conv_small_n_serves(d)) return MX_FORM_CONV_SMALL_N;
   if (conv && mx::conv_small_cin_serves(d)) return MX_FORM_CONV_SMALL_CIN;
@@ -667,6 +714,8 @@
 extern "C" void mx_gemm_release_scratch(void* stream, int all) { mx::splitk_release((hipStream_t)stream, all != 0); }
 extern "C" int mx_gemm_splitk(const mx_gemm_desc* d, int conv) {
   if (!d || mx::rows_of(d) <= 0 || d->N <= 0 || d->K <= 0) return 0;
+  mx::ConvView view;
+  d = mx::conv_view(d, conv != 0, view);
   return mx::pick_tile(d, conv != 0).splitk;
 }
 
@@ -679,7 +728,8 @@
 extern "C" int mx_gemm_kernel_name(const mx_gemm_desc* d, int conv, int launch, char* buf, int cap) {
   if (!d || mx::rows_of(d) <= 0 || d->N <= 0 || d->K <= 0 || launch < 0) return -1;
   mx_gemm_desc d1, d2;
-  const mx_gemm_desc* q = d;
+  mx::ConvView view;
+  const mx_gemm_desc* q = mx::conv_view(d, conv != 0, view);
   if (!conv && mx::tail_split(d, d1, d2)) { if (launch > 1) return 0; q = launch == 0 ? &d1 : &d2; }
   else if (launch > 0) return 0;
   const int form = mx::gemm_kernel_of(q, conv != 0, mx::pick_tile(q, conv != 0));
diff --git a/sduss_amd/csrc/gemm_bf16_v2.hip b/sduss_amd/csrc/gemm_bf16_v2.hip
--- a/sduss_amd/csrc/gemm_bf16_v2.hip
+++ b/sduss_amd/csrc/gemm_bf16_v2.hip
@@ -26,10 +26,14 @@
   GemmArgs p = pk;
   int tm, tn;
   const int n_tiles = gemm_m_tiles(pk, BM2) * (pk.N / BN);
-  const int slice = pk.splitk > 1 ? (int)blockIdx.x / n_tiles : 0;
-  const int tile_id = (int)blockIdx.x - slice * n_tiles;
+  constexpr bool CONV_UP4 = conv_up4_form(CONV, FEAT, GEGLU, false);
+  const bool up4 = CONV_UP4 && pk.up == MX_CONV_UP4_VIEW;
+  const int outer = (pk.splitk > 1 || up4) ? (int)blockIdx.x / n_tiles : 0;
+  const int slice = up4 ? 0 : outer;
+  const int tile_id = (int)blockIdx.x - outer * n_tiles;
   gemm_tile_of_block(tile_id, gemm_m_tiles(pk, BM2), pk.N / BN, pk.xcd_map, tm, tn);
   gemm_select_seg(p, pk, tm);
+  if (up4) gemm_set_phase(p, pk, outer);
   const int nk_all = p.K / DMA_BK;
   const int k_first = pk.splitk > 1 ? (int)((long)nk_all * slice / pk.splitk) : 0;
   const int nk = pk.splitk > 1 ? (int)((long)nk_all * (slice + 1) / pk.splitk) - k_first : nk_all;
@@ -123,13 +127,13 @@
       if (!splitk_combine<NI, MI>(pk, acc, tile_id, slice, BM2 * BN, reinterpret_cast<volatile int*>(smem))) return;
     }
     static_assert(!GEGLU || (NI % 4 == 0 && !CONV), "the gated epilogue pairs whole 32-feature halves");
-    gemm_epilogue_regs<NI, MI, GEGLU, true, true, true, FEAT>(p, acc, m0 + wm * 16 * MI, n0 + wn * (BN / 2), fr, fq, ln_rstd);
+    gemm_epilogue_regs<NI, MI, GEGLU, true, true, true, FEAT, true, false, false, CONV_UP4>(p, acc, m0 + wm * 16 * MI, n0 + wn * (BN / 2), fr, fq, ln_rstd);
     wait_vmcnt<0>();
   }
 }
 
 int launch_v2(hipStream_t s, const GemmArgs& a, int bn, int form) {
-  const int tiles = (a.nseg > 0 ? a.mt_total : cdiv(a.M, 128)) * (a.N / bn) * (a.splitk > 1 ? a.splitk : 1);
+  const int tiles = (a.nseg > 0 ? a.mt_total : cdiv(a.M, 128)) * (a.N / bn) * (a.splitk > 1 ? a.splitk : a.up == MX_CONV_UP4_VIEW ? 4 : 1);
   dim3 grid(tiles), block(512);
   switch (form) {
 #define MX_V2(id, k, targs) case id: hipLaunchKernelGGL((k<MX_FORM_UNPAREN targs>), grid, block, 0, s, a); return 0;
diff --git a/sduss_amd/csrc/gemm_bf16_v5.hip b/sduss_amd/csrc/gemm_bf16_v5.hip
--- a/sduss_amd/csrc/gemm_bf16_v5.hip
+++ b/sduss_amd/csrc/gemm_bf16_v5.hip
@@ -13,12 +13,20 @@
   constexpr int STAGE_ELEMS = (64 * MI + BN) * DMA_BK;
   __shared__ __attribute__((aligned(16))) bf16_t smem[NSTAGE5 * STAGE_ELEMS];
   int tm, tn;
-  gemm_tile_of_block(blockIdx.x, gemm_m_tiles(pk, 64 * MI), pk.N / BN, pk.xcd_map, tm, tn);
-  gemm_v5_tile<BN, MI, CONV, FEAT, GEGLU, VEC>(pk, tm, tn, smem);
+  int tile_id = blockIdx.x, phase = 0;
+  if constexpr (conv_up4_form(CONV, FEAT, GEGLU, VEC)) {
+    if (pk.up == MX_CONV_UP4_VIEW) {
+      const int n_tiles = gemm_m_tiles(pk, 64 * MI) * (pk.N / BN);
+      phase = tile_id / n_tiles;
+      tile_id -= phase * n_tiles;
+    }
+  }
+  gemm_tile_of_block(tile_id, gemm_m_tiles(pk, 64 * MI), pk.N / BN, pk.xcd_map, tm, tn);
+  gemm_v5_tile<BN, MI, CONV, FEAT, GEGLU, VEC>(pk, tm, tn, smem, phase);
 }
 
 int launch_v5(hipStream_t s, const GemmArgs& a, int bn, int rows, int form) {
-  const int tiles = (a.nseg > 0 ? a.mt_total : cdiv(a.M, rows)) * (a.N / bn);
+  const int tiles = (a.nseg > 0 ? a.mt_total : cdiv(a.M, rows)) * (a.N / bn) * (a.up == MX_CONV_UP4_VIEW ? 4 : 1);
   dim3 grid(tiles), block(512);
   switch (form) {
 #define MX_V5(id, k, targs) case id: hipLaunchKernelGGL((k<MX_FORM_UNPAREN targs>), grid, block, 0, s, a); return 0;
diff --git a/sduss_amd/csrc/gemm_dma_loader.inc b/sduss_amd/csrc/gemm_dma_loader.inc
--- a/sduss_amd/csrc/gemm_dma_loader.inc
+++ b/sduss_amd/csrc/gemm_dma_loader.inc
@@ -13,9 +13,11 @@
   int tap_next = 0, in_tap = 0;
 
   auto conv_set_tap = [&](int tap, int cbyte = 0) __attribute__((always_inline)) {
-    const int dy = tap / 3 - 1;
-    const int dx = tap - (tap / 3) * 3 - 1;
-    const int Hv = p.Hin << p.up, Wv = p.Win << p.up;
+    const bool up4 = CONV_UP4 && p.up == MX_CONV_UP4_VIEW;
+    const int ush = up4 ? 0 : p.up;
+    const int dy = up4 ? (tap >> 1) + (p.phase >> 1) - 1 : tap / 3 - 1;
+    const int dx = up4 ? (tap & 1) + (p.phase & 1) - 1 : tap - (tap / 3) * 3 - 1;
+    const int Hv = p.Hin << ush, Wv = p.Win << ush;
     const int P = p.corner_patch;
 #pragma unroll
     for (int i = 0; i < XI; ++i) {
@@ -27,7 +29,7 @@
         if (cross_r && cross_c) iy = cy[i];
       }
       const bool ok = (cb[i] >= 0) && (iy >= -p.vhalo) && (iy < Hv + p.vhalo) && (ix >= 0) && (ix < Wv);
-      const long off = ((((long)cb[i] * (p.Hin + 2 * p.vhalo) + (iy >> p.up) + p.vhalo) * p.Win + (ix >> p.up)) * p.Cin) * 2;
+      const long off = ((((long)cb[i] * (p.Hin + 2 * p.vhalo) + (iy >> ush) + p.vhalo) * p.Win + (ix >> ush)) * p.Cin) * 2;
       xsrc[i] = (ok ? reinterpret_cast<const char*>(p.a) + off + cbyte : zero) + xchb[i];
     }
   };
diff --git a/sduss_amd/csrc/gemm_v5_body.h b/sduss_amd/csrc/gemm_v5_body.h
--- a/sduss_amd/csrc/gemm_v5_body.h
+++ b/sduss_amd/csrc/gemm_v5_body.h
@@ -17,7 +17,7 @@
 #endif
 
 template <int BN, int MI, bool CONV, int FEAT, bool GEGLU, bool VEC, bool WT = false>
-__device__ __forceinline__ void gemm_v5_tile(const GemmArgs& pk, int tm, const int tn, bf16_t* const smem) {
+__device__ __forceinline__ void gemm_v5_tile(const GemmArgs& pk, int tm, const int tn, bf16_t* const smem, const int phase = 0) {
   constexpr int BM5 = 64 * MI;
   constexpr int NI = BN / 32;
   constexpr int LOADS = DmaTile<BN, MI>::LOADS;
@@ -31,6 +31,8 @@
   MX5_STAMP(0);
   GemmArgs p = pk;
   gemm_select_seg(p, pk, tm);
+  constexpr bool CONV_UP4 = conv_up4_form(CONV, FEAT, GEGLU, VEC);
+  if constexpr (CONV_UP4) { if (pk.up == MX_CONV_UP4_VIEW) gemm_set_phase(p, pk, phase); }
   const int nk = p.K / DMA_BK;
   constexpr bool SPLIT_K = false;
   constexpr int k_first = 0;
@@ -100,7 +102,7 @@
 
   const int m0 = tm * BM5, n0 = tn * BN;
   static_assert(!GEGLU || (NI % 4 == 0 && !CONV), "the gated epilogue pairs whole 32-feature halves");
-  gemm_epilogue_regs<NI, MI, GEGLU, VEC, true, true, FEAT, true, false, WT>(p, acc, m0 + wm * 16 * MI, n0 + wn * (BN / 2), fr, fq, ln_rstd);
+  gemm_epilogue_regs<NI, MI, GEGLU, VEC, true, true, FEAT, true, false, WT, CONV_UP4>(p, acc, m0 + wm * 16 * MI, n0 + wn * (BN / 2), fr, fq, ln_rstd);
   if constexpr (!GEGLU && FEAT == 0 && MI == 4) {
     if (pk.gn_part != nullptr) gemm_gn_partials<NI, MI>(p, acc, m0 + wm * 16 * MI, n0 + wn * (BN / 2), fr, fq);
   }
diff --git a/sduss_amd/csrc/plan_base.h b/sduss_amd/csrc/plan_base.h
--- a/sduss_amd/csrc/plan_base.h
+++ b/sduss_amd/csrc/plan_base.h
@@ -79,6 +79,10 @@
   }
   const bf16_t* wb(const std::string& name, size_t elems) { return (const bf16_t*)w(name, elems * 2); }
   const float* wf(const std::string& name, size_t elems) { return (const float*)w(name, elems * 4); }
+  const bf16_t* wb_optional(const std::string& name, size_t elems) {
+    if ((dry && !lookup) || weights->table.find(name) == weights->table.end()) return nullptr;
+    return wb(name, elems);
+  }
   template <typename T> T* alloc(size_t elems) {
     T* p = (T*)ar.alloc(elems * sizeof(T));
     if (!p) fail("workspace too small");
diff --git a/sduss_amd/csrc/unet_sdxl.cpp b/sduss_amd/csrc/unet_sdxl.cpp
--- a/sduss_amd/csrc/unet_sdxl.cpp
+++ b/sduss_amd/csrc/unet_sdxl.cpp
@@ -309,6 +309,7 @@
     d.c = out; d.ldc = Cout; d.B = gB[0]; d.Hin = Hin; d.Win = Win; d.Cin = Cin;
     d.Hout = (Hv + stride - 1) / stride; d.Wout = (Wv + stride - 1) / stride; d.stride = stride; d.up = up;
     d.corner_patch = corner_patch;
+    if (up == 1 && stride == 1 && corner_patch == 0 && vhalo == 0) d.w_up4 = wb_optional(prefix + ".weight_up4", (size_t)16 * Cout * Cin);
     d.M = gB[0] * d.Hout * d.Wout; d.N = Cout; d.K = 9 * Cin;
     d.rowbias = rowbias; d.ldrb = ldrb; d.rows_per_batch = d.Hout * d.Wout;
     d.residual = residual; d.ldr = Cout;
diff --git a/sduss_amd/lib.py b/sduss_amd/lib.py
--- a/sduss_amd/lib.py
+++ b/sduss_amd/lib.py
@@ -44,6 +44,7 @@
         ("ln_stats", C.c_void_p), ("ln_colsum", C.c_void_p), ("ln_slabs", C.c_int), ("ln_eps", C.c_float), ("stats_out", C.c_void_p),
         ("segs", C.POINTER(GemmSeg)), ("n_segs", C.c_int), ("splitk", C.c_int),
         ("ln_final", C.c_void_p), ("ln_final_out", C.c_void_p), ("ln_final_cnt", C.c_void_p), ("gn_part_out", C.c_void_p), ("cin_valid", C.c_int),
+        ("w_up4", C.c_void_p),
     ]
 
 
diff --git a/sduss_amd/ops.py b/sduss_amd/ops.py
--- a/sduss_amd/ops.py
+++ b/sduss_amd/ops.py
@@ -130,10 +130,11 @@
 
 def conv3x3(x: torch.Tensor, w: torch.Tensor, bias: Optional[torch.Tensor], stride: int = 1, up: int = 0,
             corner_patch: int = 0, rowbias: Optional[torch.Tensor] = None, residual: Optional[torch.Tensor] = None, splitk: int = 0, want_gn_partials: bool = False,
-            cin_valid: int = 0):
+            cin_valid: int = 0, w_up4: Optional[torch.Tensor] = None, vhalo: int = 0):
     l = _lib.load()
     _bf16(x); _bf16(w)
     b, h, wd, cin = x.shape
+    h -= 2 * vhalo
     cout = w.shape[0]
     hv, wv = h << up, wd << up
     ho, wo = (hv + stride - 1) // stride, (wv + stride - 1) // stride
@@ -146,6 +147,11 @@
     d.B, d.Hin, d.Win, d.Cin, d.Hout, d.Wout, d.stride, d.up, d.corner_patch = b, h, wd, cin, ho, wo, stride, up, corner_patch
     d.splitk = splitk
     d.cin_valid = cin_valid
+    d.vhalo = vhalo
+    if w_up4 is not None:
+        _bf16(w_up4)
+        assert tuple(w_up4.shape) == (4, cout, 4 * cin)
+        d.w_up4 = w_up4.data_ptr()
     part = None
     if want_gn_partials and l.mx_gemm_gn_partials_supported(C.byref(d), 1):
         part = torch.full((b * ho * wo // 64, cout, 2), float("nan"), dtype=torch.float32, device=x.device)
diff --git a/sduss_amd/unet.py b/sduss_amd/unet.py
--- a/sduss_amd/unet.py
+++ b/sduss_amd/unet.py
@@ -20,7 +20,7 @@
 
 class MxUNet:
 
-    def __init__(self, cfg: UNetConfig, params: Dict[str, torch.Tensor], device="cuda:0"):
+    def __init__(self, cfg: UNetConfig, params: Dict[str, torch.Tensor], device="cuda:0", upconv_collapse: bool = True):
         self.cfg = cfg
         self.device = torch.device(device)
         self.dtype = torch.bfloat16
@@ -42,7 +42,7 @@
         self._handle = self._lib.mx_unet_create(C.byref(cc))
         if not self._handle:
             raise _lib.MxError("mx_unet_create: " + self._lib.mx_last_error().decode())
-        self.weights = PackedWeights(pack(cfg, params), self.device)
+        self.weights = PackedWeights(pack(cfg, params, up4=upconv_collapse), self.device)
         _lib.check(self._lib.mx_unet_set_weights(self._handle, self.weights.blob.data_ptr(), self.weights.blob.numel(),
                                                  self.weights.table, len(self.weights.names)), "mx_unet_set_weights")
         self.mixed_one_sequence = True
diff --git a/sduss_amd/weights.py b/sduss_amd/weights.py
--- a/sduss_amd/weights.py
+++ b/sduss_amd/weights.py
@@ -64,6 +64,29 @@
     return w.reshape(o, -1).contiguous()
 
 
+_UP4_TAPS = (((0,), (1, 2)), ((0, 1), (2,)))
+
+
+def up4_sums(w: torch.Tensor) -> torch.Tensor:
+    w = w if w.dtype == torch.float64 else w.to(torch.float32)
+    o, i = w.shape[:2]
+    out = w.new_zeros((2, 2, o, i, 2, 2))
+    for py in range(2):
+        for px in range(2):
+            for ty in range(2):
+                for tx in range(2):
+                    for ky in _UP4_TAPS[py][ty]:
+                        for kx in _UP4_TAPS[px][tx]:
+                            out[py, px, :, :, ty, tx] += w[:, :, ky, kx]
+    return out
+
+
+def pack_up4(w: torch.Tensor) -> torch.Tensor:
+    o, i = w.shape[:2]
+    s = up4_sums(w.to(torch.float32))
+    return s.permute(0, 1, 2, 4, 5, 3).reshape(4, o, 4 * i).to(torch.bfloat16).contiguous()
+
+
 def fold_layernorm(w: torch.Tensor, bias: Optional[torch.Tensor], gamma: torch.Tensor, beta: torch.Tensor):
     w32 = w.to(torch.float32)
     wf = (w32 * gamma.to(torch.float32)[None, :]).to(torch.bfloat16)
@@ -97,7 +120,7 @@
     return torch.cat([h, g], dim=1).reshape(t.shape).contiguous()
 
 
-def pack(cfg: UNetConfig, P: Dict[str, torch.Tensor]) -> List[Tuple[str, torch.Tensor]]:
+def pack(cfg: UNetConfig, P: Dict[str, torch.Tensor], up4: bool = True) -> List[Tuple[str, torch.Tensor]]:
     missing = [k for k in param_shapes(cfg) if k not in P]
     if missing:
         raise KeyError(f"state dict lacks {len(missing)} tensors, e.g. {missing[:3]}")
@@ -158,6 +181,11 @@
     if pad:
         w = torch.nn.functional.pad(w, (0, 0, 0, pad)); bias = torch.nn.functional.pad(bias, (0, pad))
     mat("conv_out.weight", w); vec("conv_out.bias", bias)
+    if up4:
+        for i in range(n - 1):
+            p = f"up_blocks.{i}.upsamplers.0.conv"
+            if P[f"{p}.weight"].shape[1] % 64 == 0:
+                mat(f"{p}.weight_up4", pack_up4(P[f"{p}.weight"]))
     return out
 
 
```

Result: faster. 1.454 images/s (median of 6 runs) (+1.3%).
